# fabioiuri/DRecPy

Measured on AMD Instinct MI355X. Metric: training samples/sec (user-item pairs), higher is better.
Workload: dtype f32; 1 GPU; CDAE hidden_factors=128 sampled-output sparse-Adagrad on synth-10m-shaped synthetic (10000000 users x 1000000 items, 199573906 positives), corruption 0.2, neg_ratio 5; batch_per_gpu=65536, global_batch=65536, touch_list=prepared ahead on a side stream, batches=fresh device-sampled batch every step (sampler running ahead on the side stream)

## Files before the change

drecpy_amd/_lib.py:

```python
import ctypes as C
import os

_HERE = os.path.dirname(os.path.abspath(__file__))
LIB_PATH = os.path.join(_HERE, 'libdrx.so')

LOSS_BCE, LOSS_MSE = 0, 1
TARGETS_REFERENCE, TARGETS_PER_ROW = 0, 1
OPT_ADAM, OPT_ADAGRAD, OPT_ROWWISE_ADAGRAD = 0, 1, 2
DENSE_AUX_CLEAN = 0x100
KEY_NONE = 0xFFFFFFFF
SHARD_SELF_BYPASS = 1
BATCH_SHARE_USERS = 1


class DrxError(RuntimeError):
    pass


DRX_REC_SIGMOID_BIAS, DRX_REC_BIAS, DRX_REC_CLIP = 0, 1, 2

KNN_METRICS = {'cosine': 0, 'adjusted_cosine': 1, 'cosine_cf': 2, 'jaccard': 3, 'msd': 4, 'pearson': 5}
KNN_USER, KNN_ITEM = 0, 1
KNN_AGGREGATIONS = {'mean': 0, 'weighted_mean': 1}

# ... 6 lines not shown
class History(C.Structure):
    _fields_ = [('indptr', C.c_void_p), ('indices', C.c_void_p), ('t_rank', C.c_void_p), ('t_nnz', C.c_int64), ('t_users', C.c_void_p),
                ('t_pos', C.c_void_p), ('t_items', C.c_void_p)]


class Batch(C.Structure):
    _fields_ = [('B', C.c_int32), ('uid', C.c_void_p), ('iid', C.c_void_p), ('y', C.c_void_p),
                ('keep_off', C.c_void_p), ('keep', C.c_void_p), ('mask_seed', C.c_uint64), ('q', C.c_float),
                ('n_touch_slots', C.c_int32), ('flags', C.c_uint32)]


class HotHead(C.Structure):
    _fields_ = [('H', C.c_int32), ('slot', C.c_void_p), ('item', C.c_void_p)]


class ListGroups(C.Structure):
    _fields_ = [('indptr', C.c_void_p), ('seq_ids', C.c_void_p), ('held_indptr', C.c_void_p), ('held', C.c_void_p),
                ('group_value', C.c_void_p), ('eligible', C.c_void_p), ('n_groups', C.c_int32), ('n_eligible', C.c_int32),
                ('n_ids', C.c_int32)]


class Shard(C.Structure):
    _fields_ = [('world', C.c_int32), ('rank', C.c_int32), ('n_items', C.c_int32), ('items_per_rank', C.c_int32),
                ('n_users_local', C.c_int32), ('flags', C.c_uint32), ('chunks', C.c_int32)]


MAX_CHUNKS = 16


class ShardExchange(C.Structure):
    _fields_ = [('send_counts', C.c_void_p), ('recv_counts', C.c_void_p), ('uniq', C.c_void_p), ('req', C.c_void_p), ('table', C.c_void_p),
                ('table_bytes', C.c_size_t), ('rows_cache', C.c_void_p), ('rows_send', C.c_void_p), ('grad_send', C.c_void_p),
                ('grad_recv', C.c_void_p), ('rows_ticket', C.c_int64 * MAX_CHUNKS), ('grad_ticket', C.c_int64 * MAX_CHUNKS)]


MAX_SEGMENTS = 24


class AdamSegments(C.Structure):
    _fields_ = [('n', C.c_int32), ('start', C.c_int32 * MAX_SEGMENTS), ('len', C.c_int32 * MAX_SEGMENTS), ('alpha', C.c_float * MAX_SEGMENTS),
                ('l2_coef', C.c_float * MAX_SEGMENTS)]


class CaserDims(C.Structure):
    _fields_ = [(n, C.c_int32) for n in ('L', 'T', 'Tp', 'd', 'ld', 'ld2', 'n_v', 'n_h', 'n_small', 'off_kv', 'off_bv')] + \
               [('off_kh', C.c_int32 * 8), ('off_bh', C.c_int32 * 8), ('off_wd', C.c_int32), ('off_bd', C.c_int32), ('act_h', C.c_int32),
                ('act_mlp', C.c_int32)]


class CaserArgs(C.Structure):
    _fields_ = [(n, C.c_void_p) for n in ('item_emb', 'user_emb', 'W1', 'b1', 'sw', 'uid', 'before', 'after', 'keep')] + \
               [('rate', C.c_float), ('B', C.c_int32)] + \
               [(n, C.c_void_p) for n in ('dE', 'dW1', 'db1', 'dPu', 'gsw_part', 'loss_part', 'cat_out')] + [('mask_seed', C.c_uint64)]


class CsrAdamTable(C.Structure):
    _fields_ = [(n, C.c_void_p) for n in ('row_ptr', 'order', 'src', 'scale')] + [(n, C.c_int32) for n in ('group', 'ld', 'n_rows')] + \
               [(n, C.c_void_p) for n in ('p', 'm', 'v', 'p_s', 'm_s', 'v_s')] + [(n, C.c_float) for n in ('alpha', 'alpha_s', 'l2_coef')]


class OptRule(C.Structure):
    _fields_ = [('kind', C.c_int32), ('lr', C.c_float), ('mu', C.c_float), ('mu2', C.c_float), ('eps', C.c_float)]


class NcfDims(C.Structure):
    _fields_ = [(n, C.c_int32) for n in ('n_users', 'n_items', 'kg', 'km', 'ldg', 'ldm', 'n_layers')] + \
               [('f', C.c_int32 * 4), ('off_w', C.c_int32 * 4), ('off_b', C.c_int32 * 4), ('off_h', C.c_int32), ('off_b0', C.c_int32),
                ('n_small', C.c_int32)]


class GruDims(C.Structure):
    _fields_ = [(n, C.c_int32) for n in ('n_items', 'k', 'h', 'ldk', 'ldh', 'off_wx', 'off_wh', 'off_bx', 'off_bhn', 'n_small')]


class VaeDims(C.Structure):
    _fields_ = [(n, C.c_int32) for n in ('n_items', 'h', 'ldh', 'latent', 'variational', 'e', 'off_we', 'off_wd', 'off_vec', 'n_small')]


class SasDims(C.Structure):
    _fields_ = [(n, C.c_int32) for n in ('n_items', 'h', 'ldh', 'L', 'blocks', 'off_pos', 'off_blk', 'off_vec', 'off_lnf', 'n_small')]


class CsrList(C.Structure):
    _fields_ = [('keys', C.c_void_p), ('T', C.c_int32), ('n_rows', C.c_int32), ('row_ptr', C.c_void_p), ('order', C.c_void_p)]


class DmfDims(C.Structure):
    _fields_ = [('n_layers', C.c_int32 * 2), ('f', (C.c_int32 * 4) * 2), ('ld0', C.c_int32 * 2),
                ('off_k', (C.c_int32 * 4) * 2), ('off_b', (C.c_int32 * 4) * 2), ('n_small', C.c_int32),
                ('l2_norm_vectors', C.c_int32), ('off_scale', C.c_int32)]


class DmfArgs(C.Structure):
    _fields_ = [(n, C.c_void_p) for n in ('K0u', 'K0i', 'sw', 'u_indptr', 'u_indices', 'u_values', 'i_indptr', 'i_indices',
                                          'i_values', 'uid', 'iid', 'y')] + [('target_mode', C.c_int32), ('y_mean', C.c_float)] + \
               [(n, C.c_void_p) for n in ('off_u', 'off_i')] + [('B', C.c_int32)] + \
               [(n, C.c_void_p) for n in ('dz0u', 'dz0i', 'tkeys_u', 'tsrc_u', 'tcoef_u', 'tkeys_i', 'tsrc_i', 'tcoef_i',
                                          'gsw_part', 'loss_part', 'pred_out', 'rep_u_out', 'rep_i_out', 'work', 'inv_u', 'inv_i',
                                          'gptr_u', 'gptr_i', 'grows_u', 'grows_i')] + [('n_du', C.c_int32), ('n_di', C.c_int32)] + \
               [(n, C.c_void_p) for n in ('map_u', 'map_i', 'rho_u', 'rho_i')] + [('stamp', C.c_uint32)] + \
               [(n, C.c_void_p) for n in ('nd_dev', 'y_mean_dev', 'work_order')] + [('n_work', C.c_int32), ('seg_len', C.c_int32)] + \
               [(n, C.c_void_p) for n in ('zseg', 'zpart', 'n_work_dev')]


class DmfK0Update(C.Structure):
    _fields_ = [(n, C.c_void_p) for n in ('K0u', 'm_u', 'v_u', 'K0i', 'm_i', 'v_i')] + [('n_items', C.c_int32), ('n_users', C.c_int32)] + \
               [(n, C.c_float) for n in ('alpha_u', 'alpha_i', 'l2_coef', 'beta1', 'beta2', 'eps')] + [('row_order', C.c_void_p), ('n_long', C.c_int32), ('opt_kind', C.c_int32)]


class Optim(C.Structure):
    _fields_ = [('kind', C.c_int32), ('lr', C.c_float), ('reg_rate', C.c_float), ('beta1', C.c_float),
                ('beta2', C.c_float), ('eps', C.c_float), ('alpha', C.c_float * 5),
                ('s1', C.c_void_p * 5), ('s2', C.c_void_p * 5)]


_lib = None

SIGNATURES = {
    'drx_version': (C.c_int, []),
    'drx_strerror': (C.c_char_p, [C.c_int]),
    'drx_hash_u32': (C.c_uint32, [C.c_uint64, C.c_uint32, C.c_uint32]),
    'drx_event_create': (C.c_void_p, []),
    'drx_event_destroy': (None, [C.c_void_p]),
    'drx_event_record': (C.c_int, [C.c_void_p, C.c_void_p]),
    'drx_stream_wait_event': (C.c_int, [C.c_void_p, C.c_void_p]),
    'drx_event_synchronize': (C.c_int, [C.c_void_p]),
    'drx_stream_create_cu_slice': (C.c_void_p, [C.c_int32]),
    'drx_stream_destroy': (None, [C.c_void_p]),
    'drx_cdae_forward': (C.c_int, [C.POINTER(CdaeParams), C.POINTER(History), C.POINTER(Batch), C.c_void_p,
                                   C.c_void_p, C.c_void_p]),
    'drx_cdae_scratch_bytes': (C.c_size_t, [C.POINTER(CdaeParams), C.c_int32, C.c_int32, C.c_int32]),
    'drx_cdae_step_dense': (C.c_int, [C.POINTER(CdaeParams), C.POINTER(Optim), C.POINTER(History), C.POINTER(Batch),
                                      C.c_int32, C.c_int32, C.c_void_p, C.c_size_t, C.c_void_p, C.c_void_p]),
    'drx_cdae_step_sparse': (C.c_int, [C.POINTER(CdaeParams), C.POINTER(Optim), C.POINTER(History), C.POINTER(Batch),
                                       C.c_int32, C.c_void_p, C.c_size_t, C.c_void_p, C.c_void_p]),
    'drx_cdae_step_sparse_timed': (C.c_int, [C.POINTER(CdaeParams), C.POINTER(Optim), C.POINTER(History),
                                             C.POINTER(Batch), C.c_int32, C.c_void_p, C.c_size_t, C.c_void_p,
                                             C.POINTER(C.c_void_p), C.c_void_p]),
    'drx_cdae_prep_bytes': (C.c_size_t, [C.POINTER(CdaeParams), C.c_int32, C.c_int32]),
    'drx_cdae_sparse_prepare': (C.c_int, [C.POINTER(CdaeParams), C.POINTER(History), C.POINTER(Batch), C.c_void_p,
                                          C.c_size_t, C.c_void_p]),
    'drx_cdae_step_sparse_prepared': (C.c_int, [C.POINTER(CdaeParams), C.POINTER(Optim), C.POINTER(History),
                                                C.POINTER(Batch), C.c_int32, C.c_void_p, C.c_size_t, C.c_void_p,
                                                C.c_size_t, C.c_void_p, C.POINTER(C.c_void_p), C.c_void_p]),
    'drx_cdae_prep_bytes_hot': (C.c_size_t, [C.POINTER(CdaeParams), C.c_int32, C.c_int32, C.c_int32]),
    'drx_cdae_scratch_bytes_hot': (C.c_size_t, [C.POINTER(CdaeParams), C.c_int32, C.c_int32, C.c_int32]),
    'drx_cdae_sparse_prepare_hot': (C.c_int, [C.POINTER(CdaeParams), C.POINTER(History), C.POINTER(Batch), C.POINTER(HotHead),
                                              C.c_void_p, C.c_size_t, C.c_void_p]),
    'drx_debug_prep_counts': (C.c_int, [C.POINTER(CdaeParams), C.POINTER(History), C.POINTER(Batch), C.POINTER(HotHead), C.c_void_p,
                                        C.c_int32, C.c_int32, C.c_int32, C.c_void_p, C.c_size_t, C.c_void_p, C.c_void_p, C.c_void_p,
                                        C.c_void_p, C.c_void_p, C.POINTER(C.c_int32), C.c_void_p]),
    'drx_debug_prep_result': (C.c_int, [C.POINTER(CdaeParams), C.c_int32, C.c_int32, C.c_int32, C.c_void_p, C.c_size_t, C.c_void_p,
                                        C.c_void_p, C.c_void_p, C.c_void_p, C.c_void_p, C.c_void_p]),
    'drx_debug_cdae_reduce': (C.c_int, [C.POINTER(CdaeParams), C.POINTER(Optim), C.POINTER(History), C.POINTER(Batch), C.POINTER(HotHead),
                                        C.c_void_p, C.c_size_t, C.c_void_p, C.c_void_p, C.c_void_p, C.c_int32, C.c_void_p, C.c_size_t,
                                        C.c_void_p]),
    'drx_debug_span_plan': (C.c_int, [C.POINTER(CdaeParams), C.c_int32, C.c_int32, C.c_int32, C.c_void_p, C.c_size_t, C.c_void_p,
                                      C.c_void_p, C.c_void_p, C.c_void_p]),
    'drx_cdae_step_sparse_hot': (C.c_int, [C.POINTER(CdaeParams), C.POINTER(Optim), C.POINTER(History), C.POINTER(Batch),
                                           C.POINTER(HotHead), C.c_int32, C.c_void_p, C.c_size_t, C.c_void_p, C.c_size_t,
                                           C.c_void_p, C.POINTER(C.c_void_p), C.c_void_p]),
    'drx_cdae_hot_rows_for': (C.c_int32, [C.POINTER(CdaeParams), C.c_int32, C.c_int32, C.c_int32, C.c_int32]),
    'drx_cdae_prep_forget': (None, [C.c_void_p]),
    'drx_point_sample_scratch_bytes': (C.c_size_t, [C.c_int32]),
    'drx_list_sample_device': (C.c_int, [C.POINTER(ListGroups), C.c_int32, C.c_int32, C.c_int32, C.c_int32, C.c_uint64, C.c_void_p, C.c_void_p,
                                         C.c_void_p, C.c_void_p]),
    'drx_point_sample': (C.c_int, [C.POINTER(History), C.c_int32, C.c_int32, C.c_int32, C.c_int32, C.c_uint64,
                                   C.c_void_p, C.c_void_p, C.c_void_p, C.c_void_p, C.c_void_p, C.c_size_t, C.c_void_p, C.c_uint32,
                                   C.c_void_p]),
    'drx_point_sample_recorded': (C.c_int, [C.POINTER(History), C.POINTER(History), C.c_int32, C.c_int32, C.c_int32, C.c_int32, C.c_uint64,
                                   C.c_void_p, C.c_void_p, C.c_void_p, C.c_void_p, C.c_void_p, C.c_size_t, C.c_void_p, C.c_uint32,
                                   C.c_void_p]),
    'drx_point_sample_by_user_scratch_bytes': (C.c_size_t, [C.c_int32, C.c_int32]),
    'drx_point_sample_by_user': (C.c_int, [C.POINTER(History), C.POINTER(History), C.c_int32, C.c_int32, C.c_int32, C.c_int32, C.c_uint64,
                                           C.c_void_p, C.c_void_p, C.c_void_p, C.c_void_p, C.c_void_p, C.c_size_t, C.c_void_p, C.c_uint32,
                                           C.c_void_p]),
    'drx_point_sample_valued': (C.c_int, [C.POINTER(History), C.POINTER(History), C.c_void_p, C.c_float, C.c_float, C.c_int32, C.c_int32,
                                          C.c_int32, C.c_int32, C.c_uint64, C.c_void_p, C.c_void_p, C.c_void_p, C.c_void_p]),
    'drx_dmf_distinct_scratch_bytes': (C.c_size_t, [C.c_int32, C.c_int32, C.c_int32]),
    'drx_dmf_batch_distinct_device': (C.c_int, [C.c_void_p, C.c_void_p, C.c_void_p, C.c_int32, C.c_int32, C.c_int32] + [C.c_void_p] * 10 +
                                      [C.c_void_p, C.c_size_t, C.c_void_p]),
    'drx_shard_prep_bytes': (C.c_size_t, [C.POINTER(CdaeParams), C.POINTER(Shard), C.c_int32, C.c_int32]),
    'drx_shard_work_bytes': (C.c_size_t, [C.POINTER(Shard)]),
    'drx_shard_prep_layout': (C.c_int, [C.POINTER(CdaeParams), C.POINTER(Shard), C.c_int32, C.c_int32, C.POINTER(C.c_size_t)]),
    'drx_shard_prepare': (C.c_int, [C.POINTER(CdaeParams), C.POINTER(Shard), C.POINTER(History), C.POINTER(Batch), C.c_void_p,
                                    C.c_size_t, C.c_void_p, C.c_size_t, C.c_void_p]),
    'drx_shard_owner_table_bytes': (C.c_size_t, [C.POINTER(Shard), C.c_int32]),
    'drx_shard_chunks': (C.c_int32, [C.POINTER(Shard)]),
    'drx_shard_unit_shift': (C.c_int32, [C.POINTER(Shard)]),
    'drx_shard_owner_index': (C.c_int, [C.POINTER(Shard), C.c_void_p, C.c_int32, C.POINTER(C.c_int32), C.c_int32, C.c_int32, C.c_void_p,
                                        C.c_size_t, C.c_void_p]),
    'drx_shard_gather_rows': (C.c_int, [C.POINTER(CdaeParams), C.POINTER(Shard), C.c_void_p, C.c_int32, C.POINTER(C.c_int32),
                                        C.c_int32, C.c_void_p, C.c_void_p]),
    'drx_shard_step_scratch_bytes': (C.c_size_t, [C.POINTER(CdaeParams), C.c_int32, C.c_int32]),
    'drx_shard_step_local': (C.c_int, [C.POINTER(CdaeParams), C.POINTER(Optim), C.POINTER(Shard), C.POINTER(History), C.POINTER(Batch),
                                       C.c_void_p, C.c_size_t, C.c_void_p, C.c_void_p, C.c_int32, C.c_int32, C.c_void_p, C.c_size_t,
                                       C.POINTER(C.c_void_p), C.c_void_p]),
    'drx_shard_apply': (C.c_int, [C.POINTER(CdaeParams), C.POINTER(Optim), C.POINTER(Shard), C.c_int32, C.c_void_p, C.c_void_p,
                                  C.c_int32, C.POINTER(C.c_int32), C.c_int32, C.c_int32, C.c_void_p, C.POINTER(C.c_void_p), C.POINTER(C.c_int64),
                                  C.c_void_p, C.c_void_p]),
    'drx_shard_exchange_sizes': (C.c_int, [C.POINTER(CdaeParams), C.POINTER(Shard), C.c_void_p, C.c_void_p, C.POINTER(C.c_int64)]),
    'drx_shard_phase_layout': (C.c_int, [C.POINTER(CdaeParams), C.POINTER(Shard), C.c_void_p, C.c_void_p, C.c_int32, C.POINTER(C.c_int64)]),
    'drx_shard_phase_keys': (C.c_int, [C.POINTER(Shard), C.c_void_p, C.POINTER(ShardExchange), C.c_void_p]),
    'drx_shard_phase_rows': (C.c_int, [C.POINTER(CdaeParams), C.POINTER(Shard), C.c_void_p, C.POINTER(ShardExchange), C.c_int32, C.c_void_p]),
    'drx_shard_phase_local': (C.c_int, [C.POINTER(CdaeParams), C.POINTER(Optim), C.POINTER(Shard), C.POINTER(History), C.POINTER(Batch),
                                        C.c_void_p, C.POINTER(ShardExchange), C.c_void_p, C.c_size_t, C.c_int32, C.c_int32, C.c_void_p,
                                        C.c_size_t, C.POINTER(C.c_void_p), C.c_void_p]),
    'drx_shard_phase_tail': (C.c_int, [C.POINTER(CdaeParams), C.POINTER(Optim), C.POINTER(Shard), C.c_void_p, C.POINTER(ShardExchange),
                                       C.POINTER(ShardExchange), C.c_int32, C.c_void_p, C.c_void_p]),
    'drx_copy_f4': (C.c_int, [C.c_void_p, C.c_void_p, C.c_size_t, C.c_void_p]),
    'drx_copy_f4_variant': (C.c_int, [C.c_void_p, C.c_void_p, C.c_size_t, C.c_int32, C.c_void_p]),
    'drx_comm_unique_id': (C.c_int, [C.c_void_p]),
    'drx_comm_create': (C.c_int, [C.c_void_p, C.c_int32, C.c_int32, C.c_uint32, C.POINTER(C.c_void_p)]),
    'drx_comm_destroy': (C.c_int, [C.c_void_p]),
    'drx_comm_stream': (C.c_void_p, [C.c_void_p]),
    'drx_comm_alltoallv': (C.c_int64, [C.c_void_p, C.c_void_p, C.POINTER(C.c_int64), C.POINTER(C.c_int64), C.c_void_p, C.POINTER(C.c_int64),
                                       C.POINTER(C.c_int64), C.c_void_p]),
    'drx_comm_wait': (C.c_int, [C.c_void_p, C.c_int64, C.c_void_p]),
    'drx_comm_last_error': (C.c_char_p, []),
    'drx_adam_dense': (C.c_int, [C.c_void_p, C.c_void_p, C.c_void_p, C.c_void_p, C.c_int64, C.c_float, C.c_float, C.c_float,
                                 C.c_float, C.c_float, C.c_void_p]),
    'drx_scatter_scratch_bytes': (C.c_size_t, [C.c_int32, C.c_int32, C.c_int32]),
    'drx_scatter_rows': (C.c_int, [C.c_void_p, C.c_int32, C.c_void_p, C.c_void_p, C.c_void_p, C.c_void_p, C.c_int32,
                                   C.c_int32, C.c_void_p, C.c_void_p, C.c_void_p, C.c_size_t, C.c_void_p]),
    'drx_batch_offsets': (C.c_int, [C.c_void_p, C.c_void_p, C.c_int32, C.c_void_p, C.c_void_p, C.c_size_t, C.c_void_p]),
    'drx_sumsq': (C.c_int, [C.c_void_p, C.c_int64, C.c_void_p, C.c_int32, C.c_void_p]),
    'drx_rows_dot': (C.c_int, [C.c_void_p, C.c_int32, C.c_void_p, C.c_int32, C.c_int32, C.c_void_p, C.c_void_p,
                               C.c_void_p]),
    'drx_adam_segments': (C.c_int, [C.c_void_p, C.c_void_p, C.c_void_p, C.c_void_p, C.POINTER(AdamSegments), C.c_float,
                                    C.c_float, C.c_float, C.c_void_p]),
    'drx_caser_grid': (C.c_int, [C.POINTER(CaserDims), C.c_int32]),
    'drx_caser_fwd_bwd': (C.c_int, [C.POINTER(CaserDims), C.POINTER(CaserArgs), C.c_void_p, C.c_void_p]),
    'drx_caser_step_small': (C.c_int, [C.POINTER(CaserDims), C.POINTER(CaserArgs), C.c_void_p, C.c_void_p, C.c_void_p, C.c_void_p,
                                       C.POINTER(AdamSegments), C.c_float, C.c_float, C.c_float, C.c_void_p]),
    'drx_caser_hidden': (C.c_int, [C.POINTER(CaserDims), C.POINTER(CaserArgs), C.c_void_p]),
    'drx_rows_csr_adam_multi': (C.c_int, [C.POINTER(CsrAdamTable), C.c_int32, C.c_float, C.c_float, C.c_float, C.c_void_p]),
    'drx_dmf_grid': (C.c_int, [C.c_int32]),
    'drx_dmf_work_bytes': (C.c_size_t, [C.c_int32]),
    'drx_dmf_fwd_bwd': (C.c_int, [C.POINTER(DmfDims), C.POINTER(DmfArgs), C.c_void_p, C.c_void_p]),
    'drx_dmf_step_small': (C.c_int, [C.POINTER(DmfDims), C.POINTER(DmfArgs), C.c_void_p, C.c_void_p, C.c_void_p, C.c_void_p,
                                     C.POINTER(AdamSegments), C.c_float, C.c_float, C.c_float, C.c_void_p]),
    'drx_dmf_predict': (C.c_int, [C.POINTER(DmfDims), C.POINTER(DmfArgs), C.c_void_p]),
    'drx_first_occurrence': (C.c_int64, [C.c_void_p, C.c_int64, C.c_int64, C.c_void_p]),
    'drx_spin_until': (C.c_int, [C.c_void_p, C.c_int64, C.c_int32]),
    'drx_batch_csr': (C.c_int, [C.c_void_p, C.c_int32, C.c_int32, C.c_void_p, C.c_void_p]),
    'drx_batch_csr_device_bytes': (C.c_size_t, [C.POINTER(CsrList), C.c_int32]),
    'drx_batch_csr_device': (C.c_int, [C.POINTER(CsrList), C.c_int32, C.c_void_p, C.c_size_t, C.c_void_p]),
    'drx_rows_csr_adam': (C.c_int, [C.c_void_p, C.c_void_p, C.c_void_p, C.c_void_p, C.c_int32, C.c_int32, C.c_void_p, C.c_void_p, C.c_void_p,
                                    C.c_void_p, C.c_void_p, C.c_void_p, C.c_float, C.c_float, C.c_float, C.c_float, C.c_float, C.c_float,
                                    C.c_void_p]),
    'drx_rows_csr_adam_outer': (C.c_int, [C.c_void_p, C.c_void_p, C.c_void_p, C.c_void_p, C.c_int32, C.c_int32, C.c_int32, C.c_void_p,
                                          C.c_void_p, C.c_void_p, C.c_void_p, C.c_void_p, C.c_void_p, C.c_float, C.c_float, C.c_float,
                                          C.c_float, C.c_float, C.c_float, C.c_void_p]),
    'drx_opt_dense': (C.c_int, [C.c_void_p, C.c_void_p, C.c_void_p, C.c_void_p, C.c_int64, C.POINTER(OptRule), C.c_float, C.c_void_p]),
    'drx_opt_segments': (C.c_int, [C.c_void_p, C.c_void_p, C.c_void_p, C.c_void_p, C.POINTER(AdamSegments), C.POINTER(OptRule), C.c_void_p]),
    'drx_rows_csr_opt': (C.c_int, [C.c_void_p, C.c_void_p, C.c_void_p, C.c_void_p, C.c_int32, C.c_int32, C.c_void_p, C.c_void_p, C.c_void_p,
                                   C.c_void_p, C.c_void_p, C.c_void_p, C.c_float, C.c_float, C.c_float, C.POINTER(OptRule), C.c_void_p]),
    'drx_rows_csr_opt_outer': (C.c_int, [C.c_void_p, C.c_void_p, C.c_void_p, C.c_void_p, C.c_int32, C.c_int32, C.c_int32, C.c_void_p,
                                         C.c_void_p, C.c_void_p, C.c_void_p, C.c_void_p, C.c_void_p, C.c_float, C.c_float, C.c_float,
                                         C.POINTER(OptRule), C.c_void_p]),
    'drx_rows_csr_opt_multi': (C.c_int, [C.POINTER(CsrAdamTable), C.c_int32, C.POINTER(OptRule), C.c_void_p]),
    'drx_bpr_sample': (C.c_int, [C.POINTER(History), C.POINTER(History), C.c_void_p, C.c_int32, C.c_int32, C.c_int32, C.c_int32, C.c_uint64,
                                 C.c_void_p, C.c_void_p, C.c_void_p, C.c_void_p]),
    'drx_bpr_gather_rows': (C.c_int, [C.c_void_p, C.c_int32, C.c_void_p, C.c_int32, C.c_void_p, C.c_void_p]),
    'drx_bpr_step_scratch_bytes': (C.c_size_t, [C.c_int32, C.c_int32, C.c_int32, C.c_int32]),
    'drx_bpr_step': (C.c_int, [C.c_void_p] * 9 + [C.c_int32, C.c_int32, C.c_int32, C.c_void_p, C.c_void_p, C.c_void_p, C.c_int32,
                               C.POINTER(OptRule), C.POINTER(C.c_float), C.c_float, C.c_void_p, C.c_void_p, C.c_size_t, C.c_void_p]),
    'drx_als_gram_scratch_bytes': (C.c_size_t, [C.c_int32, C.c_int32]),
    'drx_als_gram': (C.c_int, [C.c_void_p, C.c_int32, C.c_int32, C.c_void_p, C.c_void_p, C.c_size_t, C.c_void_p]),
    'drx_als_solve_rows_scratch_bytes': (C.c_size_t, [C.c_int32, C.c_int32, C.c_int32]),
    'drx_als_solve_rows': (C.c_int, [C.c_void_p] * 7 + [C.c_int32, C.c_int32, C.c_int32, C.c_float, C.c_void_p, C.c_void_p, C.c_size_t,
                                     C.c_void_p]),
    'drx_als_loss_scratch_bytes': (C.c_size_t, [C.c_int32, C.c_int32]),
    'drx_als_loss': (C.c_int, [C.c_void_p] * 7 + [C.c_int32, C.c_int32, C.c_int32, C.c_float, C.c_void_p, C.c_void_p, C.c_size_t, C.c_void_p]),
    'drx_fpmc_step_scratch_bytes': (C.c_size_t, [C.c_int32] * 6),
    'drx_fpmc_step': (C.c_int, [C.c_void_p] * 12 + [C.c_int32, C.c_int32, C.c_int32, C.c_void_p, C.c_void_p, C.c_void_p, C.c_int32, C.c_int32,
                                C.c_int32, C.POINTER(OptRule), C.POINTER(C.c_float), C.c_float, C.c_void_p, C.c_void_p, C.c_size_t, C.c_void_p]),
    'drx_fpmc_query_rows': (C.c_int, [C.c_void_p, C.c_void_p, C.c_int32, C.c_void_p, C.c_int32, C.c_void_p, C.c_int32, C.c_void_p, C.c_void_p]),
    'drx_ncf_grid': (C.c_int, [C.c_int32]),
    'drx_ncf_step_scratch_bytes': (C.c_size_t, [C.POINTER(NcfDims), C.c_int32]),
    'drx_ncf_step': (C.c_int, [C.POINTER(NcfDims)] + [C.c_void_p] * 12 + [C.c_int32, C.POINTER(OptRule), C.POINTER(C.c_float), C.c_float,
                               C.c_void_p, C.c_void_p, C.c_size_t, C.c_void_p]),
    'drx_ncf_half_width': (C.c_int32, [C.POINTER(NcfDims)]),
    'drx_ncf_half_rows': (C.c_int, [C.POINTER(NcfDims), C.c_void_p, C.c_void_p, C.c_void_p, C.c_int32, C.c_int32, C.c_void_p, C.c_void_p]),
    'drx_ncf_score_rows': (C.c_int, [C.POINTER(NcfDims), C.c_void_p, C.c_void_p, C.c_void_p, C.c_int32, C.c_void_p, C.c_void_p]),
    'drx_ncf_pair_scores': (C.c_int, [C.POINTER(NcfDims), C.c_void_p, C.c_void_p, C.c_void_p, C.c_void_p, C.c_void_p, C.c_int32, C.c_void_p,
                                      C.c_void_p]),
    'drx_gru_grid': (C.c_int, [C.c_int32]),
    'drx_gru_step_scratch_bytes': (C.c_size_t, [C.POINTER(GruDims), C.c_int32, C.c_int32, C.c_int32]),
    'drx_gru_step': (C.c_int, [C.POINTER(GruDims)] + [C.c_void_p] * 14 + [C.c_int32, C.c_int32, C.c_int32, C.POINTER(OptRule),
                               C.POINTER(C.c_float), C.c_float, C.c_void_p, C.c_void_p, C.c_size_t, C.c_void_p]),
    'drx_gru_query_rows': (C.c_int, [C.c_void_p, C.c_void_p, C.POINTER(GruDims), C.c_void_p, C.c_int32, C.c_void_p, C.c_int32, C.c_void_p,
                                     C.c_void_p]),
    'drx_sas_grid': (C.c_int, [C.c_int32]),
    'drx_sas_step_scratch_bytes': (C.c_size_t, [C.POINTER(SasDims), C.c_int32, C.c_int32]),
    'drx_sas_step': (C.c_int, [C.POINTER(SasDims)] + [C.c_void_p] * 14 + [C.c_int32, C.c_int32, C.POINTER(OptRule), C.POINTER(C.c_float),
                               C.c_float, C.c_void_p, C.c_void_p, C.c_size_t, C.c_void_p]),
    'drx_sas_query_rows': (C.c_int, [C.c_void_p, C.c_void_p, C.POINTER(SasDims), C.c_void_p, C.c_void_p, C.c_int32, C.c_void_p,
                                     C.c_void_p]),
    'drx_vae_step_scratch_bytes': (C.c_size_t, [C.POINTER(VaeDims), C.c_int32, C.c_int32, C.c_int32]),
    'drx_vae_step': (C.c_int, [C.POINTER(VaeDims)] + [C.c_void_p] * 12 + [C.POINTER(History), C.c_void_p, C.c_void_p, C.c_int32, C.c_int32,
                               C.c_int32, C.c_void_p, C.c_void_p, C.c_float, C.c_float, C.POINTER(OptRule), C.POINTER(C.c_float), C.c_float,
                               C.c_void_p, C.c_void_p, C.c_size_t, C.c_void_p]),
    'drx_vae_noise': (C.c_int, [C.c_uint64, C.c_void_p, C.c_int32, C.c_int32, C.c_int32, C.c_float, C.c_void_p, C.c_void_p, C.c_void_p,
                                C.c_void_p]),
    'drx_vae_query_rows': (C.c_int, [C.c_void_p, C.c_void_p, C.POINTER(VaeDims), C.POINTER(History), C.c_void_p, C.c_int32, C.c_void_p,
# ... 172 lines not shown
```

drecpy_amd/csrc/drx_cdae.hip:

```cpp
#include "drx_common.hpp"
#include "drx_rows.hpp"
#include "drx_segreduce.hpp"
#include <cstring>
#include "drx_scan.hpp"
#include "drx_prep.hpp"
#include "drx_segstream.hpp"
#include "drx_cdae_host.hpp"
#include <type_traits>
#include <mutex>
#include <unordered_map>

#ifdef DRX_STAMPS
static unsigned long long *h_stamps = nullptr;
extern "C" int drx_debug_set_stamps(unsigned long long *buf, unsigned int) { h_stamps = buf; return 0; }
#endif

namespace drx {

struct SparseBufs {
  float *dz1;
  float *g2;
  float *dz2;
  float *lossb;
  float *phead, *ptail;
  float *phs, *pts;
  float *pblock, *pbs;
  float *bpart;
  const uint8_t *solo_v, *solo_o;
  unsigned long long *stamps;
  const int32_t *order;
  const int32_t *usamp, *worder, *n_items;
  const WorkItem *witem;
  int T, n_chunks, n_bpart;
};

template <int G, int J, int KIND = -1>
__device__ __forceinline__ void sparse_apply(const DrxCdaeParams &P, const DrxOptim &opt, int B, uint32_t key, int lane,
                                             const float4 (&g)[J], float gs) {
  const uint32_t N = (uint32_t)P.n_items;
  float *const tW = P.W, *const tO = P.W2T, *const tV = P.V;
  float *const a0 = opt.s1[0], *const a1 = opt.s1[1], *const a2 = opt.s1[2];
  float *const c0 = opt.s2[0], *const c1 = opt.s2[1], *const c2 = opt.s2[2];
  const int var = key < N ? 0 : (key < 2 * N ? 1 : 2);
  const size_t row = key - (uint32_t)var * N;
  float *const tab = var == 0 ? tW : (var == 1 ? tO : tV);
  float *const s1 = var == 0 ? a0 : (var == 1 ? a1 : a2);
  float *const s2 = var == 0 ? c0 : (var == 1 ? c1 : c2);
  OptScalars o = opt_for(opt, 0, B);
  o.inv_k = 1.0f / (float)P.k;
  float4 w[J];
  load_row<G, J>(tab, row, P.ld, lane, w);
  row_update<G, J, KIND>(o, tab, s1, s2, row, P.ld, lane, w, g);
  if (var == 1 && lane == 0) {
    const int kind = KIND >= 0 ? KIND : o.kind;
    float pb = P.b2[row], m = opt.s1[4][row], v = kind == DRX_OPT_ADAM ? opt.s2[4][row] : 0.f;
    o.rb = 0.f;
    opt_update1<KIND>(o, gs, pb, m, v);
    P.b2[row] = pb; opt.s1[4][row] = m;
    if (kind == DRX_OPT_ADAM) opt.s2[4][row] = v;
  }
}

template <int G, int J>
__device__ __forceinline__ float sampled_hidden(const DrxCdaeParams &P, const DrxBatch &bt, float scale, int b, int lane,
                                                const float4 (&acc)[J], float4 (&h)[J], float4 (&w2)[J]) {
  hidden_act<G, J>(P, bt.uid[b], scale, lane, acc, h);
  load_row<G, J>(P.W2T, (size_t)bt.iid[b], P.ld, lane, w2);
  float d = 0.f;
#pragma unroll
  for (int j = 0; j < J; ++j) d += f4_dot(w2[j], h[j]);
  return group_sum<G>(d);
}

template <int G, int J, int KIND = -1>
__device__ __forceinline__ void sampled_rest(const DrxCdaeParams &P, const DrxOptim &opt, const DrxHistory &H, const DrxBatch &bt,
                                             float scale, uint32_t qthr, int loss_kind, const SparseBufs &S, int b, int lane,
                                             float d, const float4 (&h)[J], const float4 (&w2)[J],
                                             float4 (*dz1_out)[J] = nullptr) {
  const int u = bt.uid[b], i = bt.iid[b];
  const float y = bt.y[b];
  const float p = sigmoidf_(d + P.b2[i]);
  const float invB = 1.0f / (float)bt.B;
  float lval, dp;
  if (loss_kind == DRX_LOSS_BCE) { lval = bce_elem(y, p); dp = bce_grad(y, p) * invB; }
  else { lval = (p - y) * (p - y); dp = 2.0f * (p - y) * invB; }
  const float dz2 = dp * p * (1.0f - p);
  float4 dz1[J], g2[J];
#pragma unroll
  for (int j = 0; j < J; ++j) {
    dz1[j].x = dz2 * w2[j].x * h[j].x * (1.0f - h[j].x); dz1[j].y = dz2 * w2[j].y * h[j].y * (1.0f - h[j].y);
    dz1[j].z = dz2 * w2[j].z * h[j].z * (1.0f - h[j].z); dz1[j].w = dz2 * w2[j].w * h[j].w * (1.0f - h[j].w);
    g2[j].x = dz2 * h[j].x; g2[j].y = dz2 * h[j].y; g2[j].z = dz2 * h[j].z; g2[j].w = dz2 * h[j].w;
  }
  store_row<G, J>(S.dz1, (size_t)b, P.ld, lane, dz1);
  if (lane == 0) S.lossb[b] = lval;
  const uint8_t *const pv = S.solo_v, *const po = S.solo_o;
  const bool solo_v = pv && pv[b], solo_o = po && po[b];
  if (solo_o) {
    sparse_apply<G, J, KIND>(P, opt, bt.B, (uint32_t)P.n_items + (uint32_t)i, lane, g2, dz2);
  } else {
    store_row<G, J>(S.g2, (size_t)b, P.ld, lane, g2);
    if (lane == 0) S.dz2[b] = dz2;
  }
  if (solo_v) sparse_apply<G, J, KIND>(P, opt, bt.B, 2u * (uint32_t)P.n_items + (uint32_t)u, lane, dz1, 0.f);
  if (dz1_out) {
#pragma unroll
    for (int j = 0; j < J; ++j) (*dz1_out)[j] = dz1[j];
  }
}

template <int G, int J, int KIND = -1>
__device__ __forceinline__ void sampled_finish(const DrxCdaeParams &P, const DrxOptim &opt, const DrxHistory &H, const DrxBatch &bt,
                                               float scale, uint32_t qthr, int loss_kind, const SparseBufs &S, int b, int lane,
                                               const float4 (&acc)[J]) {
  float4 h[J], w2[J];
#ifdef DRX_STAMPS
  if (acc[0].x == acc[0].x) DRX_STAMP(S.stamps, b, 5, lane);
#endif
  const float d = sampled_hidden<G, J>(P, bt, scale, b, lane, acc, h, w2);
#ifdef DRX_STAMPS
  if (d == d) DRX_STAMP(S.stamps, b, 6, lane);
#endif
  sampled_rest<G, J, KIND>(P, opt, H, bt, scale, qthr, loss_kind, S, b, lane, d, h, w2);
  DRX_STAMP(S.stamps, b, 7, lane);
}

template <int G, int J>
__global__ __launch_bounds__(kBlock) void k_kshard_fwd(DrxCdaeParams P, DrxHistory H, DrxBatch bt, float scale, uint32_t qthr,
                                                       float *__restrict__ h_out, float *__restrict__ dot_out,
                                                       const int32_t *__restrict__ order) {
  const int lane = threadIdx.x % G;
  const int slot = blockIdx.x * (kBlock / G) + threadIdx.x / G;
  if (slot >= bt.B) return;
  const int b = order ? order[slot] : slot;
  float4 acc[J], h[J], w2[J];
  DenseAux none{};
  gather_bag<G, J, 0>(P, H, bt, qthr, b, lane, acc, none, nullptr, nullptr, 0);
  const float d = sampled_hidden<G, J>(P, bt, scale, b, lane, acc, h, w2);
  store_row<G, J>(h_out, (size_t)b, P.ld, lane, h);
  if (lane == 0) dot_out[b] = d;
}

template <int G, int J>
__global__ __launch_bounds__(kBlock) void k_kshard_fwd_wg(DrxCdaeParams P, DrxHistory H, DrxBatch bt, float scale, uint32_t qthr,
                                                          float *__restrict__ h_out, float *__restrict__ dot_out) {
  extern __shared__ __align__(16) float lds[];
  constexpr int R = kBlock / G;
  const int lane = threadIdx.x % G, r = threadIdx.x / G;
  const int b = blockIdx.x;
  float4 acc[J], h[J], w2[J];
  DenseAux none{};
  gather_bag<G, J, 0>(P, H, bt, qthr, b, lane, acc, none, nullptr, nullptr, 0, r, R);
  store_row<G, J>(lds, (size_t)r, P.ld, lane, acc);
  __syncthreads();
  if (r != 0) return;
#pragma unroll
  for (int j = 0; j < J; ++j) acc[j] = f4_zero();
#pragma unroll 8
  for (int rr = 0; rr < R; ++rr) {
    float4 v[J];
    load_row<G, J>(lds, (size_t)rr, P.ld, lane, v);
#pragma unroll
    for (int j = 0; j < J; ++j) f4_add(acc[j], v[j]);
  }
  const float d = sampled_hidden<G, J>(P, bt, scale, b, lane, acc, h, w2);
  store_row<G, J>(h_out, (size_t)b, P.ld, lane, h);
  if (lane == 0) dot_out[b] = d;
}

template <int G, int J>
__global__ __launch_bounds__(kBlock) void k_kshard_rest(DrxCdaeParams P, DrxOptim opt, DrxHistory H, DrxBatch bt, float scale,
                                                        uint32_t qthr, int loss_kind, SparseBufs S,
                                                        const float *__restrict__ h_in, const float *__restrict__ dot_total) {
  const int lane = threadIdx.x % G;
  const int b = blockIdx.x * (kBlock / G) + threadIdx.x / G;
  if (b >= bt.B) return;
  float4 h[J], w2[J];
  load_row<G, J>(h_in, (size_t)b, P.ld, lane, h);
  load_row<G, J>(P.W2T, (size_t)bt.iid[b], P.ld, lane, w2);
  sampled_rest<G, J>(P, opt, H, bt, scale, qthr, loss_kind, S, b, lane, dot_total[b], h, w2);
}

template <int G, int J, int KIND = -1>
__global__ __launch_bounds__(kBlock) void k_sampled_fwd_bwd(DrxCdaeParams P, DrxOptim opt, DrxHistory H, DrxBatch bt, float scale,
                                                            uint32_t qthr, int loss_kind, SparseBufs S) {
  const int lane = threadIdx.x % G;
  const int slot = blockIdx.x * (kBlock / G) + threadIdx.x / G;
#ifdef DRX_STAMPS
  const unsigned long long t_in = wall_clock64();
#endif
  if (slot >= bt.B) return;
  const int32_t *const ord = S.order;
  const int b = ord ? ord[slot] : slot;
  float4 acc[J];
  DenseAux none{};
#ifdef DRX_STAMPS
  if (lane == 0 && S.stamps && (unsigned)b < 110000u) S.stamps[(size_t)b * 16] = t_in;
  if (bt.uid[b] >= 0) DRX_STAMP(S.stamps, b, 1, lane);
#endif
  gather_bag<G, J, 0>(P, H, bt, qthr, b, lane, acc, none, nullptr, nullptr, 0, 0, 1, S.stamps);
  sampled_finish<G, J, KIND>(P, opt, H, bt, scale, qthr, loss_kind, S, b, lane, acc);
}

template <int G, int J, int KIND = -1>
__global__ __launch_bounds__(kItemThreads, (4 * G * J <= 128 ? 5 : 1)) void k_items_fwd_bwd(DrxCdaeParams P, DrxOptim opt, DrxHistory H, DrxBatch bt, float scale,
                                                          uint32_t qthr, int loss_kind, SparseBufs S) {
  extern __shared__ __align__(16) float lds[];
  constexpr int R = kItemThreads / G, NWV = kItemThreads / 64, RT = kShareTriples;
  constexpr int NH = 4 * G * J / 64;
  static_assert(NH >= 1 && NH <= 8 && RT == 16, "rows of 64 .. 512 floats; the 16 x 16 x 4 matrix instruction");
  constexpr int NF = NH <= 2 ? 16 : (NH == 4 ? 8 : 4);
  constexpr int TPG = (RT + R - 1) / R;
  if ((int)blockIdx.x >= S.n_items[0]) return;
  const int w = S.worder[blockIdx.x];
  const WorkItem wi = S.witem[w];
  const int p0 = wi.p0, n = wi.n, u = wi.user;
  const int64_t s = wi.hist_start, e = s + wi.deg;
  const int lane = threadIdx.x % G, r = threadIdx.x / G;
  int *lb = (int *)(lds + (size_t)NWV * RT * P.ld);
  if ((int)threadIdx.x < RT) lb[threadIdx.x] = (int)threadIdx.x < n ? S.usamp[p0 + threadIdx.x] : 0;
  float4 vrow[J];
  load_row<G, J>(P.V, (size_t)u, P.ld, lane, vrow);
  const int n_waves = (int)min((int64_t)NWV, (e - s + NF - 1) / NF);
  {
    typedef float f4v __attribute__((ext_vector_type(4)));
    const int wl = threadIdx.x & 63, wv = threadIdx.x >> 6;
    const int kr = wl >> 4, nc = wl & 15;
    f4v acc[NH][4];
#pragma unroll
    for (int h = 0; h < NH; ++h)
#pragma unroll
      for (int j = 0; j < 4; ++j) acc[h][j] = f4v{0.f, 0.f, 0.f, 0.f};
    const int64_t c0 = s + (int64_t)wv * NF;
    int ridx[NF / 4];
#pragma unroll
    for (int g = 0; g < NF / 4; ++g) ridx[g] = c0 + 4 * g + kr < e ? H.indices[c0 + 4 * g + kr] : 0;
    __syncthreads();
    const int bmine = lb[nc];
    for (int64_t c = c0; c < e; c += (int64_t)NWV * NF) {
      const int64_t cn = c + (int64_t)NWV * NF;
      int ridx_n[NF / 4];
#pragma unroll
      for (int g = 0; g < NF / 4; ++g) ridx_n[g] = cn + 4 * g + kr < e ? H.indices[cn + 4 * g + kr] : 0;
      float4 bv[NF / 4][NH];
#pragma unroll
      for (int g = 0; g < NF / 4; ++g)
#pragma unroll
        for (int h = 0; h < NH; ++h) {
          bv[g][h] = f4_zero();
          if (c + 4 * g + kr < e && 64 * h + 4 * nc < P.ld)
            bv[g][h] = *reinterpret_cast<const float4 *>(P.W + (size_t)ridx[g] * P.ld + 64 * h + 4 * nc);
        }
#pragma unroll
      for (int g = 0; g < NF / 4; ++g) {
        const int64_t row = c + 4 * g + kr;
        bool kf = false;
        if (nc < n && row < e) {
          const uint32_t jj = (uint32_t)(row - s);
          kf = bt.keep ? (bt.keep[bt.keep_off[bmine] + jj] != 0) : (hash_u32(bt.mask_seed, (uint32_t)bmine, jj) >= qthr);
        }
        const float a = kf ? 1.0f : 0.0f;
#pragma unroll
        for (int h = 0; h < NH; ++h) {
          acc[h][0] = __builtin_amdgcn_mfma_f32_16x16x4f32(a, bv[g][h].x, acc[h][0], 0, 0, 0);
          acc[h][1] = __builtin_amdgcn_mfma_f32_16x16x4f32(a, bv[g][h].y, acc[h][1], 0, 0, 0);
          acc[h][2] = __builtin_amdgcn_mfma_f32_16x16x4f32(a, bv[g][h].z, acc[h][2], 0, 0, 0);
          acc[h][3] = __builtin_amdgcn_mfma_f32_16x16x4f32(a, bv[g][h].w, acc[h][3], 0, 0, 0);
        }
      }
#pragma unroll
      for (int g = 0; g < NF / 4; ++g) ridx[g] = ridx_n[g];
    }
    if (wv < n_waves) {
#pragma unroll
      for (int i = 0; i < 4; ++i) {
        const int t = 4 * kr + i;
        if (t < n) {
#pragma unroll
          for (int h = 0; h < NH; ++h)
            if (64 * h + 4 * nc < P.ld)
              *reinterpret_cast<float4 *>(lds + (size_t)(wv * RT + t) * P.ld + 64 * h + 4 * nc) =
                  make_float4(acc[h][0][i], acc[h][1][i], acc[h][2][i], acc[h][3][i]);
        }
      }
    }
  }
  __syncthreads();
  float4 dsum[J];
#pragma unroll
  for (int j = 0; j < J; ++j) dsum[j] = f4_zero();
#pragma unroll
  for (int kt = 0; kt < TPG; ++kt) {
    const int t = r + kt * R;
    if (t < n) {
      const int b = lb[t];
      float4 acc[J], h[J], w2[J], dz1[J];
#pragma unroll
      for (int j = 0; j < J; ++j) acc[j] = f4_zero();
      for (int wv = 0; wv < n_waves; ++wv) {
        float4 x[J];
        load_row<G, J>(lds, (size_t)(wv * RT + t), P.ld, lane, x);
#pragma unroll
        for (int j = 0; j < J; ++j) f4_add(acc[j], x[j]);
      }
      float4 brow[J];
      load_row<G, J>(P.b, 0, P.ld, lane, brow);
      hidden_act_rows<G, J>(P, scale, lane, acc, vrow, brow, h);
      load_row<G, J>(P.W2T, (size_t)bt.iid[b], P.ld, lane, w2);
      float d = 0.f;
#pragma unroll
      for (int j = 0; j < J; ++j) d += f4_dot(w2[j], h[j]);
      d = group_sum<G>(d);
      sampled_rest<G, J, KIND>(P, opt, H, bt, scale, qthr, loss_kind, S, b, lane, d, h, w2, &dz1);
#pragma unroll
      for (int j = 0; j < J; ++j) f4_add(dsum[j], dz1[j]);
    }
  }
  __syncthreads();
  if (r < n) store_row<G, J>(lds, (size_t)r, P.ld, lane, dsum);
  __syncthreads();
  if (r == 0) {
    float4 t[J];
#pragma unroll
    for (int j = 0; j < J; ++j) t[j] = f4_zero();
    for (int rr = 0; rr < min(n, R); ++rr) {
      float4 x[J];
      load_row<G, J>(lds, (size_t)rr, P.ld, lane, x);
#pragma unroll
      for (int j = 0; j < J; ++j) f4_add(t[j], x[j]);
    }
    store_row<G, J>(S.dz1, (size_t)bt.B + w, P.ld, lane, t);
  }
}

template <int G, int J>
__global__ __launch_bounds__(kBlock) void k_sampled_fwd_bwd_wg(DrxCdaeParams P, DrxOptim opt, DrxHistory H, DrxBatch bt, float scale,
                                                               uint32_t qthr, int loss_kind, SparseBufs S) {
  extern __shared__ __align__(16) float lds[];
  constexpr int R = kBlock / G;
  const int lane = threadIdx.x % G, r = threadIdx.x / G;
  const int b = blockIdx.x;
  float4 acc[J];
  DenseAux none{};
  gather_bag<G, J, 0>(P, H, bt, qthr, b, lane, acc, none, nullptr, nullptr, 0, r, R);
// ... 153 lines not shown
    const uint32_t mlane = (uint32_t)c * (uint32_t)A.Bw, xlane = (uint32_t)(8 * kq * LD + c);
    hot_f32x4 acc[4];
#pragma unroll
    for (int t = 0; t < 4; ++t) acc[t] = hot_f32x4{0.f, 0.f, 0.f, 0.f};
    uint32_t seen = 0u;
    float bsum = 0.f;
    for (int b0 = b_begin; b0 < b_end; b0 += 32) {
      float x[8];
      uint32_t w[4];
      {
        const float *const rows = slice + (size_t)(b0 - b_begin) * LD;
        const uint32_t *const words = mgrp + (b0 >> 5);
        const int left = A.B - b0 - 8 * kq;
        if (left >= 8) {
#pragma unroll
          for (int j = 0; j < 8; ++j) x[j] = rows[xlane + (uint32_t)(j * LD)];
        } else {
#pragma unroll
          for (int j = 0; j < 8; ++j) x[j] = j < left ? rows[xlane + (uint32_t)(j * LD)] : 0.f;
        }
#pragma unroll
        for (int t = 0; t < 4; ++t) w[t] = (words + (size_t)(16 * min(t, nt - 1)) * A.Bw)[mlane] & (t < nt ? ~0u : 0u);
      }
      hot_u32x4 bh, bm, bl;
#pragma unroll
      for (int i = 0; i < 4; ++i) {
        uint32_t hv[2], mv[2], lv[2];
#pragma unroll
        for (int e = 0; e < 2; ++e) {
          const float v = x[2 * i + e];
          bsum += v;
          hv[e] = __float_as_uint(v) & 0xFFFF0000u;
          const float r1 = v - __uint_as_float(hv[e]);
          mv[e] = __float_as_uint(r1) & 0xFFFF0000u;
          lv[e] = __float_as_uint(r1 - __uint_as_float(mv[e])) & 0xFFFF0000u;
        }
        bh[i] = (hv[0] >> 16) | hv[1];
        bm[i] = (mv[0] >> 16) | mv[1];
        bl[i] = (lv[0] >> 16) | lv[1];
      }
#pragma unroll
      for (int t = 0; t < 4; ++t) {
        seen |= (w[t] != 0u ? 1u : 0u) << t;
        const uint32_t bits = (w[t] >> (8 * kq)) & 0xFFu;
        hot_u32x4 a;
#pragma unroll
        for (int i = 0; i < 4; ++i) a[i] = ((bits >> (2 * i)) & 1u) * 0x3F80u | ((bits >> (2 * i + 1)) & 1u) * 0x3F800000u;
        const hot_bf16x8 av = __builtin_bit_cast(hot_bf16x8, a);
        acc[t] = __builtin_amdgcn_mfma_f32_16x16x32_bf16(av, __builtin_bit_cast(hot_bf16x8, bh), acc[t], 0, 0, 0);
        acc[t] = __builtin_amdgcn_mfma_f32_16x16x32_bf16(av, __builtin_bit_cast(hot_bf16x8, bm), acc[t], 0, 0, 0);
        acc[t] = __builtin_amdgcn_mfma_f32_16x16x32_bf16(av, __builtin_bit_cast(hot_bf16x8, bl), acc[t], 0, 0, 0);
      }
    }
    float *const out = A.part + ((size_t)s * A.H + rg * kHotGroup) * LD + cs * 16 + c;
#pragma unroll
    for (int t = 0; t < 4; ++t)
      if (t < nt) {
#pragma unroll
        for (int i = 0; i < 4; ++i) out[(size_t)(16 * t + 4 * kq + i) * LD] = acc[t][i];
      }
    if (cs == 0) {
      uint32_t rows[4];
#pragma unroll
      for (int t = 0; t < 4; ++t) rows[t] = (uint32_t)__ballot((seen >> t) & 1u) & 0xFFFFu;
      if (lane == 0) {
        uint32_t *const any = A.any + (size_t)s * (A.H / 32) + rg * (kHotGroup / 32);
        any[0] = rows[0] | (rows[1] << 16);
        if (nt > 2) any[1] = rows[2] | (rows[3] << 16);
      }
    }
    if (rg == 0) {
      const float g1 = __shfl(bsum, c + 16, 64), g2 = __shfl(bsum, c + 32, 64), g3 = __shfl(bsum, c + 48, 64);
      if (kq == 0) A.bpart[(size_t)s * LD + cs * 16 + c] = ((bsum + g1) + g2) + g3;
      if (cs == 0 && A.lossb) {
        float l = 0.f;
        for (int b = b_begin + lane; b < b_end; b += 64) l += A.lossb[b];
#pragma unroll
        for (int o = 32; o > 0; o >>= 1) l += __shfl_xor(l, o, 64);
        if (lane == 0) A.bpart[(size_t)A.S * LD + s] = l;
      }
    }
  }
};

template <int LD, class Policy>
struct HotFinishExtra {
  HotArgs A;
  Policy pol;
  __device__ __forceinline__ void operator()(float *lds) const {
    constexpr int NT = kFixBlock, NQ = NT / LD;
    static_assert(NQ >= 1 && NT % LD == 0, "a row per workgroup");
    const int h = (int)blockIdx.x - A.first;
    if (h >= A.H) return;
    const uint32_t bit = 1u << (h & 31);
    bool touched = false;
    for (int s = (int)threadIdx.x; s < A.S; s += NT) touched |= (A.any[(size_t)s * (A.H / 32) + (h >> 5)] & bit) != 0u;
    if (!__syncthreads_or(touched)) return;
    const int c = (int)threadIdx.x % LD, q = (int)threadIdx.x / LD;
    const int per = (A.S + NQ - 1) / NQ, s0 = q * per, s1 = min(A.S, s0 + per);
    float sum = 0.f;
#pragma unroll 8
    for (int s = s0; s < s1; ++s) sum += A.part[((size_t)s * A.H + h) * LD + c];
    lds[q * LD + c] = sum;
    __syncthreads();
    if (q == 0) {
      float t = lds[c];
#pragma unroll
      for (int k = 1; k < NQ; ++k) t += lds[k * LD + c];
      const StreamArrays SA = pol.stream_arrays();
      const size_t off = (size_t)A.item[h] * LD + c;
      float pv = SA.table[0][off], av = SA.slot[0][off];
      pol.stream_update(fmaf(pol.stream_decay(), pv, A.scale * t), pv, av);
      SA.table[0][off] = pv;
      SA.slot[0][off] = av;
    }
  }
};

template <class E1, class E2>
struct ExtraPair {
  E1 e1;
  int n1;
  E2 e2;
  __device__ __forceinline__ void operator()(float *lds) const {
    if ((int)blockIdx.x < n1) e1(lds);
    else e2(lds);
  }
};

static SparseBufs sparse_layout(Carver &cv, const DrxCdaeParams &P, int B, int n_touch_slots) {
  SparseBufs S{};
  S.T = n_touch_slots + 2 * B;
  const int chunk = seg_chunk(long_segments(S.T, P));
  S.n_chunks = (S.T + chunk - 1) / chunk;
  S.n_bpart = 1024;
  S.dz1 = cv.take<float>((size_t)2 * B * P.ld);
  S.g2 = cv.take<float>((size_t)B * P.ld);
  S.dz2 = cv.take<float>(B);
  S.lossb = cv.take<float>(B);
  S.phead = cv.take<float>((size_t)S.n_chunks * P.ld);
  S.ptail = cv.take<float>((size_t)S.n_chunks * P.ld);
  S.phs = cv.take<float>(S.n_chunks);
  S.pts = cv.take<float>(S.n_chunks);
  {
    const int cpb = kSegBlock / pick_geom(P.ld).G;
    const int n_blocks = (S.n_chunks + cpb - 1) / cpb;
    S.pblock = cv.take<float>((size_t)n_blocks * P.ld);
    S.pbs = cv.take<float>(n_blocks);
  }
  S.bpart = cv.take<float>((size_t)S.n_bpart * (P.ld + 1));
  return S;
}

static std::mutex g_hot_mu;
static std::unordered_map<const void *, int> g_hot_of;
static void hot_record(const void *prepared, int H) {
  std::lock_guard<std::mutex> lk(g_hot_mu);
  if (H > 0) g_hot_of[prepared] = H;
  else g_hot_of.erase(prepared);
}
static int hot_recorded(const void *prepared) {
  std::lock_guard<std::mutex> lk(g_hot_mu);
  const auto it = g_hot_of.find(prepared);
  return it == g_hot_of.end() ? 0 : it->second;
}

struct HotBufs { float *part; uint32_t *any; float *bpart; };
static HotBufs hot_layout(Carver &cv, const DrxCdaeParams &P, int B, int H) {
  HotBufs HB{nullptr, nullptr, nullptr};
  if (H <= 0) return HB;
  HB.part = cv.take<float>((size_t)hot_slices(B) * H * P.ld);
  HB.any = cv.take<uint32_t>((size_t)hot_slices(B) * (H / 32));
  HB.bpart = cv.take<float>((size_t)hot_slices(B) * (P.ld + 1));
  return HB;
}

template <int G, int J>
static void launch_forward(ForwardForm form, const DrxCdaeParams &P, const DrxOptim &opt, const DrxHistory &hist, const DrxBatch &bt,
                           float scale, uint32_t qthr, int32_t loss_kind, const SparseBufs &S, const float *ks_h, const float *ks_dot,
                           hipStream_t st) {
  constexpr int gpb = kBlock / G;
  const dim3 groups((bt.B + gpb - 1) / gpb);
  const bool adagrad = opt.kind == DRX_OPT_ADAGRAD;
  switch (form) {
  case ForwardForm::ColumnShard:
    hipLaunchKernelGGL((k_kshard_rest<G, J>), groups, dim3(kBlock), 0, st, P, opt, hist, bt, scale, qthr, loss_kind, S, ks_h, ks_dot);
    break;
  case ForwardForm::SharedUsers:
    if constexpr (G >= 16 && J <= 2) {
      const long long wmax = (long long)(P.n_users < bt.B ? P.n_users : bt.B) + bt.B / share_item_triples(P.ld) + 1;
      hipLaunchKernelGGL((adagrad ? k_items_fwd_bwd<G, J, DRX_OPT_ADAGRAD> : k_items_fwd_bwd<G, J>), dim3((unsigned)(wmax < bt.B ? wmax : bt.B)),
                         dim3(kItemThreads), share_item_lds_bytes(P.ld), st, P, opt, hist, bt, scale, qthr, loss_kind, S);
    }
    break;
  case ForwardForm::PerWorkgroup:
    hipLaunchKernelGGL((k_sampled_fwd_bwd_wg<G, J>), dim3(bt.B), dim3(kBlock), (size_t)gpb * P.ld * 4, st, P, opt, hist, bt, scale, qthr,
                       loss_kind, S);
    break;
  case ForwardForm::PerGroup:
    hipLaunchKernelGGL((adagrad ? k_sampled_fwd_bwd<G, J, DRX_OPT_ADAGRAD> : k_sampled_fwd_bwd<G, J>), groups, dim3(kBlock), 0, st, P, opt, hist,
                       bt, scale, qthr, loss_kind, S);
    break;
  }
}

template <int G, int J, class Policy>
static int reduce_and_finish(ReduceForm form, const DrxCdaeParams &P, const DrxOptim &opt, const SparseBufs &S, const SegBufs &SB,
                             const PlanBufs &PB, const SpanPlan &plan, const BiasArgs &BA, const HotArgs &HA, void *const *events,
                             hipStream_t st) {
  const Policy pol{P, opt, BA.B, HA.scale, S.dz1, (long long)(S.g2 - S.dz1), S.dz2};
  const BiasFinalExtra<G, J> bias{P, opt, BA};
  int rc = DRX_EINVAL;
  if (HA.H == 0) rc = launch_reduce<G, J>(form, SB, PB, plan, pol, BA, st);
  else if constexpr (kHotBuilt<G, J, Policy>) {
    constexpr int NT = kStreamThreads<G>;
    HotArgs part = HA;
    part.first = 0;
    const int n_hot = (HA.S * hot_groups(HA.H) * (G / 4) + NT / 64 - 1) / (NT / 64);
    rc = launch_reduce_streamed<G, J>(SB, PB, plan, pol, n_hot, HotPartialExtra<4 * G, NT>{part}, st);
  }
  if (rc) return rc;
  DRX_HIP(phase_event(events, 3, st));
  rc = DRX_EINVAL;
  if (HA.H == 0) rc = launch_spans<G, J>(SB, PB, plan, pol, 1, bias, st);
  else if constexpr (kHotBuilt<G, J, Policy>) {
    HotArgs fin = HA;
    fin.first = kSpanBlocks + 1;
    using Finish = ExtraPair<BiasFinalExtra<G, J>, HotFinishExtra<4 * G, Policy>>;
    rc = launch_spans<G, J>(SB, PB, plan, pol, 1 + HA.H, Finish{bias, fin.first, {fin, pol}}, st);
  }
  if (rc) return rc;
  DRX_HIP(phase_event(events, 4, st));
  DRX_HIP(phase_event(events, 5, st));
  return DRX_OK;
}

}

using namespace drx;

extern "C" {

size_t drx_cdae_scratch_bytes(const DrxCdaeParams *p, int32_t B, int32_t n_touch_slots, int32_t dense_mode) {
  if (!p || B < 1 || n_touch_slots < 0) return 0;
  Carver c(nullptr, 0);
  if (dense_mode) {
    c.off = dense_layout_bytes(*p, B);
  } else {
    (void)sparse_layout(c, *p, B, n_touch_slots);
    (void)prep_layout(c, *p, B, n_touch_slots);
  }
  return align_up(c.off, 256) + 256;
}

struct GivenGradients { const float *dz1, *g2, *dz2; int32_t form; };

static int step_sparse_impl(const DrxCdaeParams *p, const DrxOptim *opt, const DrxHistory *hist, const DrxBatch *bt,
                            int32_t loss_kind, const void *prepared, size_t prepared_bytes, void *scratch, size_t scratch_bytes,
                            float *loss_out, void *const *events, void *stream, const float *ks_h = nullptr,
                            const float *ks_dot = nullptr, const DrxHotHead *hot = nullptr, const GivenGradients *given = nullptr) {
  int rc = check_params(p);
  if (rc) return rc;
  rc = check_batch(hist, bt);
  if (rc || !opt || !scratch || !bt->iid || (!bt->y && !given) || !bt->keep_off) return DRX_EINVAL;
  if (opt->kind != DRX_OPT_ADAM && opt->kind != DRX_OPT_ADAGRAD && opt->kind != DRX_OPT_ROWWISE_ADAGRAD) return DRX_EINVAL;
  for (int i = 0; i < 5; ++i)
    if (!opt->s1[i] || (opt->kind == DRX_OPT_ADAM && !opt->s2[i])) return DRX_EINVAL;
  if ((uint64_t)2 * p->n_items + p->n_users + 1 >= 0xFFFFFFFFull) return DRX_EINVAL;
  hipStream_t st = (hipStream_t)stream;
  const int H = hot ? hot->H : 0;
  if (prepared && hot_recorded(prepared) != H) return DRX_EINVAL;
  Carver cv(scratch, scratch_bytes);
  SparseBufs S = sparse_layout(cv, *p, bt->B, bt->n_touch_slots);
  const HotBufs HB = hot_layout(cv, *p, bt->B, H);
  PrepBufs R{};
  if (prepared) {
    Carver cp(const_cast<void *>(prepared), prepared_bytes);
    R = prep_layout(cp, *p, bt->B, bt->n_touch_slots, H);
    if (!cp.ok()) return DRX_ESCRATCH;
  } else {
    R = prep_layout(cv, *p, bt->B, bt->n_touch_slots, H);
  }
  if (!cv.ok()) return DRX_ESCRATCH;
  const float scale = 1.0f / (1.0f - bt->q);
  const uint32_t qthr = q_threshold(bt->q);
  const int rows_per_block = (bt->B + S.n_bpart - 1) / S.n_bpart;
  const int n_bpart = (bt->B + rows_per_block - 1) / rows_per_block;
  S.solo_v = prepared ? R.solo_v : nullptr;
  S.solo_o = prepared ? R.solo_o : nullptr;
  S.order = prepared ? R.order : nullptr;
  SegBufs SB{R.keys_s, R.vals_s, S.phead, S.ptail, S.phs, S.pts, nullptr, nullptr, nullptr, nullptr, S.T, S.n_chunks, p->ld, nullptr};
#ifdef DRX_STAMPS
  S.stamps = SB.stamps = h_stamps;
#endif
  PlanBufs PB{S.pblock, S.pbs};
  if (prepared && ks_h && share_users(p, hist, bt, R)) return DRX_EINVAL;
  const bool share = prepared && !ks_h && share_users(p, hist, bt, R);
  S.usamp = share ? R.usamp : nullptr;
  S.witem = share ? R.witem : nullptr;
  S.worder = share ? R.worder : nullptr;
  S.n_items = share ? R.n_du : nullptr;
  ReduceForm form = reduce_form(opt->kind, bt->B, S.T, *p);
  const ForwardForm fwd = forward_form(ks_h != nullptr, share, bt->B, bt->n_touch_slots);
  if (H > 0 && !hot_head_fits(form, p->ld, share, ks_h != nullptr)) return DRX_EINVAL;
  if (given) {
    if (share || (given->form == 1 && (H > 0 || form == ReduceForm::PlannedLong))) return DRX_EINVAL;
    if (given->form == 1) form = ReduceForm::PlannedShort;
  }
  const HotArgs HA{S.dz1, R.hmask, HB.part, HB.any, hot ? hot->item : nullptr, scale, bt->B, H, R.Bw, hot_slices(bt->B), 0, HB.bpart,
                   loss_out ? S.lossb : nullptr};
  const BiasArgs BA = H > 0 ? BiasArgs{S.dz1, HB.bpart, S.lossb, loss_out, bt->B, hot_slices(bt->B), kHotSlice}
                            : BiasArgs{S.dz1, S.bpart, S.lossb, loss_out, bt->B, n_bpart, rows_per_block};
  DRX_HIP(phase_event(events, 0, st));
  if (given) {
    const size_t row_bytes = (size_t)bt->B * p->ld * sizeof(float);
    DRX_HIP(hipMemcpyAsync(S.dz1, given->dz1, row_bytes, hipMemcpyDeviceToDevice, st));
    DRX_HIP(hipMemcpyAsync(S.g2, given->g2, row_bytes, hipMemcpyDeviceToDevice, st));
    DRX_HIP(hipMemcpyAsync(S.dz2, given->dz2, (size_t)bt->B * sizeof(float), hipMemcpyDeviceToDevice, st));
    DRX_HIP(hipMemsetAsync(S.lossb, 0, (size_t)bt->B * sizeof(float), st));
  } else {
    (void)dispatch_geom(p->ld, [&](auto g) -> int {
      launch_forward<decltype(g)::G, decltype(g)::J>(fwd, *p, *opt, *hist, *bt, scale, qthr, loss_kind, S, ks_h, ks_dot, st);
      return DRX_OK;
    });
  }
  DRX_HIP(phase_event(events, 1, st));
  if (!prepared) {
    rc = prepare_impl(p, hist, bt, R, st, false, TouchPresence{nullptr, WireGeo{1, 0, 1}}, hot ? hot->slot : nullptr,
                      hot ? hot->item : nullptr);
    if (rc) return rc;
  }
  DRX_HIP(phase_event(events, 2, st));
  rc = dispatch_geom(p->ld, [&](auto g) -> int {
    constexpr int G = decltype(g)::G, J = decltype(g)::J;
    return opt->kind == DRX_OPT_ADAGRAD
        ? reduce_and_finish<G, J, DirectPolicyAdagrad>(form, *p, *opt, S, SB, PB, R.plan, BA, HA, events, st)
        : reduce_and_finish<G, J, DirectPolicy>(form, *p, *opt, S, SB, PB, R.plan, BA, HA, events, st);
  });
  if (rc) return rc;
  DRX_LAUNCH_CHECK();
  return DRX_OK;
}

size_t drx_cdae_prep_bytes(const DrxCdaeParams *p, int32_t B, int32_t n_touch_slots) {
  if (!p || B < 1 || n_touch_slots < 0) return 0;
  Carver c(nullptr, 0);
  (void)prep_layout(c, *p, B, n_touch_slots);
  return align_up(c.off, 256) + 256;
}

int drx_cdae_sparse_prepare(const DrxCdaeParams *p, const DrxHistory *hist, const DrxBatch *bt, void *prepared,
                            size_t prepared_bytes, void *stream) {
  int rc = check_params(p);
  if (rc) return rc;
  rc = check_batch(hist, bt);
  if (rc || !prepared || !bt->iid || !bt->keep_off) return DRX_EINVAL;
  Carver cp(prepared, prepared_bytes);
  PrepBufs R = prep_layout(cp, *p, bt->B, bt->n_touch_slots);
  if (!cp.ok()) return DRX_ESCRATCH;
  hot_record(prepared, 0);
  rc = prepare_impl(p, hist, bt, R, (hipStream_t)stream, true);
  if (rc) return rc;
  if (p->ld <= 16) order_by_degree(bt, R, (hipStream_t)stream, true);
  DRX_LAUNCH_CHECK();
  return DRX_OK;
}

size_t drx_cdae_prep_result_bytes(const DrxCdaeParams *p, int32_t B, int32_t n_touch_slots) {
  if (!p || B < 1 || n_touch_slots < 0) return 0;
  Carver c(nullptr, 0);
  return prep_layout(c, *p, B, n_touch_slots).result_bytes;
}

int drx_cdae_step_sparse_prepared(const DrxCdaeParams *p, const DrxOptim *opt, const DrxHistory *hist, const DrxBatch *bt,
                                  int32_t loss_kind, const void *prepared, size_t prepared_bytes, void *scratch,
                                  size_t scratch_bytes, float *loss_out, void *const *events, void *stream) {
  if (!prepared) return DRX_EINVAL;
  return step_sparse_impl(p, opt, hist, bt, loss_kind, prepared, prepared_bytes, scratch, scratch_bytes, loss_out, events, stream);
}

int drx_cdae_kshard_forward(const DrxCdaeParams *p, const DrxHistory *hist, const DrxBatch *bt, float *h_out, float *dot_partial,
                            void *stream) {
  return drx_cdae_kshard_forward_prepared(p, hist, bt, nullptr, 0, h_out, dot_partial, stream);
}

int drx_cdae_kshard_forward_prepared(const DrxCdaeParams *p, const DrxHistory *hist, const DrxBatch *bt, const void *prepared,
                                     size_t prepared_bytes, float *h_out, float *dot_partial, void *stream) {
  int rc = check_params(p);
  if (rc) return rc;
  rc = check_batch(hist, bt);
  if (rc || !bt->iid || !bt->keep_off || !h_out || !dot_partial) return DRX_EINVAL;
  const int32_t *order = nullptr;
  if (prepared) {
    Carver cp(const_cast<void *>(prepared), prepared_bytes);
    const PrepBufs R = prep_layout(cp, *p, bt->B, bt->n_touch_slots);
    if (!cp.ok()) return DRX_ESCRATCH;
    order = R.order;
  }
  hipStream_t st = (hipStream_t)stream;
  const float scale = 1.0f / (1.0f - bt->q);
  const uint32_t qthr = q_threshold(bt->q);
  const bool per_wg = forward_per_workgroup(bt->B, bt->n_touch_slots);
  return dispatch_geom(p->ld, [&](auto g) -> int {
    constexpr int G = decltype(g)::G, J = decltype(g)::J;
    constexpr int gpb = kBlock / G;
    if (per_wg)
      hipLaunchKernelGGL((k_kshard_fwd_wg<G, J>), dim3(bt->B), dim3(kBlock), (size_t)gpb * p->ld * 4, st, *p, *hist, *bt, scale, qthr,
                         h_out, dot_partial);
    else
      hipLaunchKernelGGL((k_kshard_fwd<G, J>), dim3((bt->B + gpb - 1) / gpb), dim3(kBlock), 0, st, *p, *hist, *bt, scale, qthr, h_out,
                         dot_partial, order);
    DRX_LAUNCH_CHECK();
    return DRX_OK;
  });
}

int drx_cdae_kshard_step(const DrxCdaeParams *p, const DrxOptim *opt, const DrxHistory *hist, const DrxBatch *bt, int32_t loss_kind,
                         const float *h, const float *dot_total, const void *prepared, size_t prepared_bytes, void *scratch,
                         size_t scratch_bytes, float *loss_out, void *const *events, void *stream) {
  if (!h || !dot_total) return DRX_EINVAL;
  if (opt && opt->kind == DRX_OPT_ROWWISE_ADAGRAD) return DRX_EINVAL;
  return step_sparse_impl(p, opt, hist, bt, loss_kind, prepared, prepared_bytes, scratch, scratch_bytes, loss_out, events, stream,
                          h, dot_total);
}

int drx_cdae_step_sparse(const DrxCdaeParams *p, const DrxOptim *opt, const DrxHistory *hist, const DrxBatch *bt,
                         int32_t loss_kind, void *scratch, size_t scratch_bytes, float *loss_out, void *stream) {
  return step_sparse_impl(p, opt, hist, bt, loss_kind, nullptr, 0, scratch, scratch_bytes, loss_out, nullptr, stream);
}

int drx_cdae_step_sparse_timed(const DrxCdaeParams *p, const DrxOptim *opt, const DrxHistory *hist, const DrxBatch *bt,
                               int32_t loss_kind, void *scratch, size_t scratch_bytes, float *loss_out, void *const *events,
                               void *stream) {
  if (!events) return DRX_EINVAL;
  return step_sparse_impl(p, opt, hist, bt, loss_kind, nullptr, 0, scratch, scratch_bytes, loss_out, events, stream);
}

static int hot_rows(const DrxCdaeParams *p, int32_t H) {
  if (!p || H < 0 || H > DRX_MAX_HOT || H % 32 || H > p->n_items) return -1;
  return H;
}

static bool hot_ok(const DrxCdaeParams *p, const DrxHotHead *hot) {
  return hot && hot_rows(p, hot->H) >= 0 && (hot->H == 0 || (hot->slot && hot->item && p->ld <= 4 * kHotMaxG));
}

size_t drx_cdae_prep_bytes_hot(const DrxCdaeParams *p, int32_t B, int32_t n_touch_slots, int32_t H) {
  if (!p || B < 1 || n_touch_slots < 0 || hot_rows(p, H) < 0) return 0;
  Carver c(nullptr, 0);
  (void)prep_layout(c, *p, B, n_touch_slots, H);
  return align_up(c.off, 256) + 256;
}

size_t drx_cdae_scratch_bytes_hot(const DrxCdaeParams *p, int32_t B, int32_t n_touch_slots, int32_t H) {
  if (!p || B < 1 || n_touch_slots < 0 || hot_rows(p, H) < 0) return 0;
  Carver c(nullptr, 0);
  (void)sparse_layout(c, *p, B, n_touch_slots);
  (void)hot_layout(c, *p, B, H);
  (void)prep_layout(c, *p, B, n_touch_slots, H);
  return align_up(c.off, 256) + 256;
}

int drx_cdae_sparse_prepare_hot(const DrxCdaeParams *p, const DrxHistory *hist, const DrxBatch *bt, const DrxHotHead *hot,
                                void *prepared, size_t prepared_bytes, void *stream) {
  int rc = check_params(p);
  if (rc) return rc;
  rc = check_batch(hist, bt);
  if (rc || !prepared || !bt->iid || !bt->keep_off || !hot_ok(p, hot)) return DRX_EINVAL;
  Carver cp(prepared, prepared_bytes);
  PrepBufs R = prep_layout(cp, *p, bt->B, bt->n_touch_slots, hot->H);
  if (!cp.ok()) return DRX_ESCRATCH;
  hot_record(prepared, 0);
  rc = prepare_impl(p, hist, bt, R, (hipStream_t)stream, true, TouchPresence{nullptr, WireGeo{1, 0, 1}}, hot->slot, hot->item);
  if (rc) return rc;
  hot_record(prepared, hot->H);
  if (p->ld <= 16) order_by_degree(bt, R, (hipStream_t)stream, true);
  DRX_LAUNCH_CHECK();
  return DRX_OK;
}

int drx_debug_prep_counts(const DrxCdaeParams *p, const DrxHistory *hist, const DrxBatch *bt, const DrxHotHead *hot, uint8_t *present,
                          int32_t ipr, int32_t cshift, int32_t world, void *prepared, size_t prepared_bytes, uint32_t *hist_out,
                          uint32_t *buckets_out, uint32_t *keys_out, uint32_t *vals_out, uint32_t *mask_out, int32_t *info_out,
                          void *stream) {
  int rc = check_params(p);
  if (rc) return rc;
  rc = check_batch(hist, bt);
  if (rc || !prepared || !bt->iid || !bt->keep_off || !hist_out || !buckets_out || !keys_out || !vals_out || !info_out) return DRX_EINVAL;
  if ((uint64_t)2 * p->n_items + p->n_users + 1 >= 0xFFFFFFFFull) return DRX_EINVAL;
  if (hot && !hot_ok(p, hot)) return DRX_EINVAL;
  if (present && (ipr < 1 || cshift < 0 || cshift > 30 || world < 1)) return DRX_EINVAL;
  const int H = hot ? hot->H : 0;
  if (H > 0 && !mask_out) return DRX_EINVAL;
  Carver cp(prepared, prepared_bytes);
  const PrepBufs R = prep_layout(cp, *p, bt->B, bt->n_touch_slots, H);
  if (!cp.ok()) return DRX_ESCRATCH;
  if (H > 0 && !hot_list_fits(R.T, *p, present != nullptr)) return DRX_EINVAL;
  hipStream_t st = (hipStream_t)stream;
  hot_record(prepared, 0);
  launch_touches(p, hist, bt, R, st, TouchPresence{present, WireGeo{present ? ipr : 1, present ? cshift : 0, present ? world : 1}},
                 H > 0 ? hot->slot : nullptr, H > 0 ? hot->item : nullptr);
  const SortRider rider{bt->keep_off, bt->B, R.order_work, R.partials, R.partial_rows};
  const uint32_t *h = nullptr;
  rc = sort_first_counts(R.sort_temp, R.sort_bytes, R.keys, (size_t)R.T, R.bits, true, st, rider, &h);
  if (rc) return rc;
  const int dbits = sort_first_digit_bits(R.bits);
  DRX_HIP(hipMemcpyAsync(hist_out, h, sizeof(uint32_t) << dbits, hipMemcpyDeviceToDevice, st));
  DRX_HIP(hipMemcpyAsync(buckets_out, R.order_work, 256 * sizeof(uint32_t), hipMemcpyDeviceToDevice, st));
  DRX_HIP(hipMemcpyAsync(keys_out, R.keys, (size_t)R.T * sizeof(uint32_t), hipMemcpyDeviceToDevice, st));
  DRX_HIP(hipMemcpyAsync(vals_out, R.vals, (size_t)R.T * sizeof(uint32_t), hipMemcpyDeviceToDevice, st));
  if (H > 0) DRX_HIP(hipMemcpyAsync(mask_out, R.hmask, (size_t)H * R.Bw * sizeof(uint32_t), hipMemcpyDeviceToDevice, st));
  info_out[0] = dbits;
  info_out[1] = R.partials ? R.partial_rows : 0;
  info_out[2] = R.T;
  info_out[3] = DRX_PREP_ROUNDS ? touch_grid(bt->B) : (bt->B + 15) / 16;
  DRX_LAUNCH_CHECK();
  return DRX_OK;
}

int drx_debug_prep_result(const DrxCdaeParams *p, int32_t B, int32_t n_touch_slots, int32_t H, const void *prepared, size_t prepared_bytes,
                          uint32_t *keys_s_out, uint32_t *vals_s_out, uint8_t *solo_v_out, uint8_t *solo_o_out, int32_t *order_out,
                          void *stream) {
  int rc = check_params(p);
  if (rc) return rc;
  if (B < 1 || n_touch_slots < 0 || hot_rows(p, H) < 0 || !prepared || !keys_s_out || !vals_s_out || !solo_v_out || !solo_o_out || !order_out)
    return DRX_EINVAL;
  Carver cp(const_cast<void *>(prepared), prepared_bytes);
  const PrepBufs R = prep_layout(cp, *p, B, n_touch_slots, H);
  if (!cp.ok()) return DRX_ESCRATCH;
  hipStream_t st = (hipStream_t)stream;
  DRX_HIP(hipMemcpyAsync(keys_s_out, R.keys_s, (size_t)R.T * sizeof(uint32_t), hipMemcpyDeviceToDevice, st));
  DRX_HIP(hipMemcpyAsync(vals_s_out, R.vals_s, (size_t)R.T * sizeof(uint32_t), hipMemcpyDeviceToDevice, st));
  DRX_HIP(hipMemcpyAsync(solo_v_out, R.solo_v, (size_t)B, hipMemcpyDeviceToDevice, st));
  DRX_HIP(hipMemcpyAsync(solo_o_out, R.solo_o, (size_t)B, hipMemcpyDeviceToDevice, st));
  DRX_HIP(hipMemcpyAsync(order_out, R.order, (size_t)B * sizeof(int32_t), hipMemcpyDeviceToDevice, st));
  return DRX_OK;
}

int drx_debug_cdae_reduce(const DrxCdaeParams *p, const DrxOptim *opt, const DrxHistory *hist, const DrxBatch *bt, const DrxHotHead *hot,
                          const void *prepared, size_t prepared_bytes, const float *dz1_in, const float *g2_in, const float *dz2_in,
                          int32_t form, void *scratch, size_t scratch_bytes, void *stream) {
  if (!dz1_in || !g2_in || !dz2_in || (form != 0 && form != 1) || (hot && !hot_ok(p, hot))) return DRX_EINVAL;
  const GivenGradients given{dz1_in, g2_in, dz2_in, form};
  return step_sparse_impl(p, opt, hist, bt, DRX_LOSS_BCE, prepared, prepared_bytes, scratch, scratch_bytes, nullptr, nullptr, stream,
                          nullptr, nullptr, hot && hot->H > 0 ? hot : nullptr, &given);
}

int drx_debug_span_plan(const DrxCdaeParams *p, int32_t B, int32_t n_touch_slots, int32_t H, const void *prepared, size_t prepared_bytes,
                        uint8_t *ext_out, uint32_t *desc_out, uint32_t *cnt_out, void *stream) {
  int rc = check_params(p);
  if (rc) return rc;
  if (B < 1 || n_touch_slots < 0 || hot_rows(p, H) < 0 || !prepared || !ext_out || !desc_out || !cnt_out) return DRX_EINVAL;
  Carver cp(const_cast<void *>(prepared), prepared_bytes);
  const PrepBufs R = prep_layout(cp, *p, B, n_touch_slots, H);
  if (!cp.ok()) return DRX_ESCRATCH;
  hipStream_t st = (hipStream_t)stream;
  DRX_HIP(hipMemcpyAsync(ext_out, R.plan.ext, (size_t)R.n_chunks, hipMemcpyDeviceToDevice, st));
  DRX_HIP(hipMemcpyAsync(desc_out, R.plan.desc, (size_t)R.n_chunks * sizeof(uint2), hipMemcpyDeviceToDevice, st));
  DRX_HIP(hipMemcpyAsync(cnt_out, R.plan.cnt, 2 * sizeof(uint32_t), hipMemcpyDeviceToDevice, st));
  return DRX_OK;
}

int drx_cdae_step_sparse_hot(const DrxCdaeParams *p, const DrxOptim *opt, const DrxHistory *hist, const DrxBatch *bt,
                             const DrxHotHead *hot, int32_t loss_kind, const void *prepared, size_t prepared_bytes, void *scratch,
                             size_t scratch_bytes, float *loss_out, void *const *events, void *stream) {
  if (!hot_ok(p, hot)) return DRX_EINVAL;
  return step_sparse_impl(p, opt, hist, bt, loss_kind, prepared, prepared_bytes, scratch, scratch_bytes, loss_out, events, stream,
                          nullptr, nullptr, hot);
}

int32_t drx_cdae_hot_rows_for(const DrxCdaeParams *p, int32_t opt_kind, int32_t B, int32_t n_touch_slots, int32_t H) {
  if (B < 1 || n_touch_slots < 0 || hot_rows(p, H) <= 0) return 0;
  return hot_head_fits(reduce_form(opt_kind, B, n_touch_slots + 2 * B, *p), p->ld, false, false) ? H : 0;
}

void drx_cdae_prep_forget(const void *prepared) {
  if (prepared) hot_record(prepared, 0);
}

}
```

drecpy_amd/csrc/drx_prep.hpp:

```cpp
#pragma once
#include <algorithm>
#include "drx_common.hpp"
#include "drx_rows.hpp"
#include "drx_segreduce.hpp"
#include "drx_scan.hpp"

namespace drx {

struct WireGeo {
  int ipr, cshift, world;
  __host__ __device__ __forceinline__ uint32_t wire(int item, int is_out) const {
    const int o = item / ipr;
    const uint32_t l = 2u * (uint32_t)(item - o * ipr) + (uint32_t)(is_out ? 1 : 0);
    return (((l >> cshift) * (uint32_t)world + (uint32_t)o) << cshift) | (l & ((1u << cshift) - 1u));
  }
  __host__ __device__ __forceinline__ uint32_t local(uint32_t w) const {
    return (((w >> cshift) / (uint32_t)world) << cshift) | (w & ((1u << cshift) - 1u));
  }
  __host__ __device__ __forceinline__ uint32_t unit(uint32_t w) const { return w >> cshift; }
};

struct TouchPresence {
  uint8_t *present;
  WireGeo G;
  __device__ __forceinline__ uint32_t wire(int item, int is_out) const { return G.wire(item, is_out); }
};

#ifndef DRX_HOT_LDS_LOOKUP
#define DRX_HOT_LDS_LOOKUP 1
#endif
struct HotMark {
  const int16_t *slot;
  uint32_t *mask;
  int H, Bw;
  const int32_t *item;
  int tbits;
};
static inline int hot_table_bits(int H) {
  int b = 0;
  while ((1 << b) < 4 * H) ++b;
  return b;
}
static inline size_t hot_table_lds_bytes(int H) { return H > 0 && DRX_HOT_LDS_LOOKUP ? ((size_t)6 << hot_table_bits(H)) : 0; }
__device__ __forceinline__ uint32_t hot_table_home(int item, int tbits) { return ((uint32_t)item * 2654435761u) >> (32 - tbits); }

static __global__ __launch_bounds__(kBlock) void k_sparse_touches(int n_items, DrxHistory H, DrxBatch bt, uint32_t qthr, uint32_t *keys,
                                                           uint32_t *vals, int T, uint8_t *solo, uint32_t *zero_a,
                                                           int n_zero_a, uint32_t *zero_b, int n_zero_b, uint32_t *zero_c, int n_zero_c,
                                                           TouchPresence pres, HotMark hot) {
  constexpr int G = 16;
  const int lane = threadIdx.x % G;
  const int b = blockIdx.x * (kBlock / G) + threadIdx.x / G;
  for (int w = blockIdx.x * kBlock + threadIdx.x; w < n_zero_a; w += gridDim.x * kBlock) zero_a[w] = 0u;
  for (int w = blockIdx.x * kBlock + threadIdx.x; w < n_zero_b; w += gridDim.x * kBlock) zero_b[w] = 0u;
  for (int w = blockIdx.x * kBlock + threadIdx.x; w < n_zero_c; w += gridDim.x * kBlock) zero_c[w] = 0u;
  __shared__ uint32_t hm[DRX_MAX_HOT];
  extern __shared__ __align__(16) int hot_table[];
  const uint32_t tmask = (1u << hot.tbits) - 1u;
  uint16_t *const hot_slot_of = reinterpret_cast<uint16_t *>(hot_table + tmask + 1);
  if (hot.slot) {
    for (int i = threadIdx.x; i < hot.H; i += kBlock) hm[i] = 0u;
    if (DRX_HOT_LDS_LOOKUP) {
      for (int i = threadIdx.x; i <= (int)tmask; i += kBlock) hot_table[i] = -1;
      __syncthreads();
      for (int i = threadIdx.x; i < hot.H; i += kBlock) {
        const int it = hot.item[i];
        uint32_t at = hot_table_home(it, hot.tbits);
        while (atomicCAS(&hot_table[at], -1, it) != -1) at = (at + 1u) & tmask;
        hot_slot_of[at] = (uint16_t)i;
      }
    }
    __syncthreads();
  }
  if (b < bt.B) {
  if (solo && lane == 0) { solo[b] = 0; solo[bt.B + b] = 0; }
  if (b == bt.B - 1)
    for (int j = bt.keep_off[bt.B] + 2 * bt.B + lane; j < T; j += G) { keys[j] = DRX_KEY_NONE; vals[j] = 0; }
  const int u = bt.uid[b];
  const int64_t s = H.indptr[u], e = H.indptr[u + 1];
  const int base = bt.keep_off[b] + 2 * b;
  const uint8_t *kp = bt.keep ? bt.keep + bt.keep_off[b] : nullptr;
  for (int64_t j = s + lane; j < e; j += G) {
    const uint32_t jj = (uint32_t)(j - s);
    const bool kf = kp ? (kp[jj] != 0) : (hash_u32(bt.mask_seed, (uint32_t)b, jj) >= qthr);
    const int item = H.indices[j];
    int hs = -1;
    if (hot.slot && kf) {
      if (DRX_HOT_LDS_LOOKUP) {
        for (uint32_t at = hot_table_home(item, hot.tbits);; at = (at + 1u) & tmask) {
          const int k = hot_table[at];
          if (k == item) hs = (int)hot_slot_of[at];
          if (k == item || k == -1) break;
        }
      } else hs = (int)hot.slot[item];
    }
    keys[base + jj] = kf && hs < 0 ? (uint32_t)item : DRX_KEY_NONE;
    vals[base + jj] = (uint32_t)b;
    if (hs >= 0) atomicOr(&hm[hs], 1u << (b & 15));
    if (pres.present && kf) pres.present[pres.wire(item, 0)] = 1;
  }
  if (lane == 0) {
    const int deg = (int)(e - s);
    keys[base + deg] = (uint32_t)(n_items + bt.iid[b]);       vals[base + deg] = (uint32_t)b;
    if (pres.present) pres.present[pres.wire(bt.iid[b], 1)] = 1;
    keys[base + deg + 1] = (uint32_t)(2 * n_items) + (uint32_t)u;       vals[base + deg + 1] = (uint32_t)b;
  }
  }
  if (hot.slot) {
    __syncthreads();
    uint16_t *const m16 = reinterpret_cast<uint16_t *>(hot.mask);
    const size_t row = 2 * (size_t)hot.Bw;
    const bool tail = blockIdx.x + 1 == gridDim.x && blockIdx.x + 1 < row;
    for (int i = threadIdx.x; i < hot.H; i += kBlock) {
      m16[(size_t)i * row + blockIdx.x] = (uint16_t)hm[i];
      if (tail) m16[(size_t)i * row + blockIdx.x + 1] = 0;
    }
  }
}

#ifndef DRX_PREP_ROUNDS
#define DRX_PREP_ROUNDS 1
#endif
#ifndef DRX_TOUCH_GRID
#define DRX_TOUCH_GRID 1024
#endif
static inline int touch_grid(int B) {
  const int rounds = (B + kBlock / 16 - 1) / (kBlock / 16);
  return rounds < DRX_TOUCH_GRID ? rounds : DRX_TOUCH_GRID;
}

static __global__ __launch_bounds__(kBlock) void k_sparse_touches_rounds(int n_items, DrxHistory H, DrxBatch bt, uint32_t qthr, uint32_t *keys,
                                                                  uint32_t *vals, int T, uint8_t *solo, uint32_t *zero_a,
                                                                  int n_zero_a, uint32_t *zero_b, int n_zero_b, uint32_t *zero_c,
                                                                  int n_zero_c, TouchPresence pres, HotMark hot, uint32_t *part) {
  constexpr int G = 16, SPR = kBlock / G;
  const int lane = threadIdx.x % G, grp = threadIdx.x / G;
  const int B = bt.B, n_rounds = (B + SPR - 1) / SPR, stride = (int)gridDim.x;
  for (int w = blockIdx.x * kBlock + threadIdx.x; w < n_zero_a; w += gridDim.x * kBlock) zero_a[w] = 0u;
  for (int w = blockIdx.x * kBlock + threadIdx.x; w < n_zero_b; w += gridDim.x * kBlock) zero_b[w] = 0u;
  for (int w = blockIdx.x * kBlock + threadIdx.x; w < n_zero_c; w += gridDim.x * kBlock) zero_c[w] = 0u;
  __shared__ uint32_t hm[DRX_MAX_HOT];
  __shared__ uint32_t dh[2048];
  __shared__ uint32_t bh[256];
  extern __shared__ __align__(16) int hot_table[];
  const uint32_t tmask = (1u << hot.tbits) - 1u;
  uint16_t *const hot_slot_of = reinterpret_cast<uint16_t *>(hot_table + tmask + 1);
  if (part) {
    for (int i = threadIdx.x; i < 2048; i += kBlock) dh[i] = 0u;
    for (int i = threadIdx.x; i < 256; i += kBlock) bh[i] = 0u;
  }
  if (hot.slot) {
    for (int i = threadIdx.x; i < hot.H; i += kBlock) hm[i] = 0u;
    if (DRX_HOT_LDS_LOOKUP) {
      for (int i = threadIdx.x; i <= (int)tmask; i += kBlock) hot_table[i] = -1;
      __syncthreads();
      for (int i = threadIdx.x; i < hot.H; i += kBlock) {
        const int it = hot.item[i];
        uint32_t at = hot_table_home(it, hot.tbits);
        while (atomicCAS(&hot_table[at], -1, it) != -1) at = (at + 1u) & tmask;
        hot_slot_of[at] = (uint16_t)i;
      }
    }
  }
  __syncthreads();
  const uint32_t rep = threadIdx.x & 7u;
  constexpr int kPre = 2;
  struct Stage { int u, ko0, ko1, iid; int64_t s, e; };
  const int S = stride * SPR;
  int r = (int)blockIdx.x;
  int b = r * SPR + grp;
  Stage c{0, 0, 0, 0, 0, 0}, n1 = c;
  int it[kPre], u2 = 0;
  if (b < B) { c.u = bt.uid[b]; c.ko0 = bt.keep_off[b]; c.ko1 = bt.keep_off[b + 1]; c.iid = bt.iid[b]; c.s = H.indptr[c.u]; c.e = H.indptr[c.u + 1]; }
  if (b + S < B) {
    n1.u = bt.uid[b + S]; n1.ko0 = bt.keep_off[b + S]; n1.ko1 = bt.keep_off[b + S + 1]; n1.iid = bt.iid[b + S];
    n1.s = H.indptr[n1.u]; n1.e = H.indptr[n1.u + 1];
  }
  if (b + 2 * S < B) u2 = bt.uid[b + 2 * S];
#pragma unroll
  for (int k = 0; k < kPre; ++k) it[k] = c.s + lane + k * G < c.e ? H.indices[c.s + lane + k * G] : 0;
  for (; r < n_rounds; r += stride, b += S) {
    int itn[kPre], u3 = 0;
    Stage n2{u2, 0, 0, 0, 0, 0};
#pragma unroll
    for (int k = 0; k < kPre; ++k) itn[k] = n1.s + lane + k * G < n1.e ? H.indices[n1.s + lane + k * G] : 0;
    if (b + 2 * S < B) {
      n2.ko0 = bt.keep_off[b + 2 * S]; n2.ko1 = bt.keep_off[b + 2 * S + 1]; n2.iid = bt.iid[b + 2 * S];
      n2.s = H.indptr[u2]; n2.e = H.indptr[u2 + 1];
    }
    if (b + 3 * S < B) u3 = bt.uid[b + 3 * S];
    if (b < B) {
      const int u = c.u, ko0 = c.ko0, ko1 = c.ko1;
      const int64_t s = c.s, e = c.e;
      if (solo && lane == 0) { solo[b] = 0; solo[B + b] = 0; }
      if (b == B - 1)
        for (int j = ko1 + 2 * B + lane; j < T; j += G) { keys[j] = DRX_KEY_NONE; vals[j] = 0; }
      const int base = ko0 + 2 * b;
      const uint8_t *kp = bt.keep ? bt.keep + ko0 : nullptr;
      auto touch = [&](uint32_t jj, int item) {
        const bool kf = kp ? (kp[jj] != 0) : (hash_u32(bt.mask_seed, (uint32_t)b, jj) >= qthr);
        int hs = -1;
        if (hot.slot && kf) {
          if (DRX_HOT_LDS_LOOKUP) {
            for (uint32_t at = hot_table_home(item, hot.tbits);; at = (at + 1u) & tmask) {
              const int k = hot_table[at];
              if (k == item) hs = (int)hot_slot_of[at];
              if (k == item || k == -1) break;
            }
          } else hs = (int)hot.slot[item];
        }
        const bool listed = kf && hs < 0;
        keys[base + jj] = listed ? (uint32_t)item : DRX_KEY_NONE;
        vals[base + jj] = (uint32_t)b;
        if (part && listed) atomicAdd(&dh[(((uint32_t)item & 255u) << 3) + rep], 1u);
        if (hs >= 0) atomicOr(&hm[hs], 1u << (b & 15));
        if (pres.present && kf) pres.present[pres.wire(item, 0)] = 1;
      };
#pragma unroll
      for (int k = 0; k < kPre; ++k)
        if (s + lane + k * G < e) touch((uint32_t)(lane + k * G), it[k]);
      for (int64_t j = s + lane + kPre * G; j < e; j += G) touch((uint32_t)(j - s), H.indices[j]);
      if (lane == 0) {
        const int deg = (int)(e - s);
        const uint32_t k_out = (uint32_t)(n_items + c.iid), k_usr = (uint32_t)(2 * n_items) + (uint32_t)u;
        keys[base + deg] = k_out;       vals[base + deg] = (uint32_t)b;
        if (pres.present) pres.present[pres.wire(c.iid, 1)] = 1;
        keys[base + deg + 1] = k_usr;       vals[base + deg + 1] = (uint32_t)b;
        if (part) {
          atomicAdd(&dh[((k_out & 255u) << 3) + rep], 1u);
          atomicAdd(&dh[((k_usr & 255u) << 3) + rep], 1u);
          const int d = (ko1 - ko0) >> 2;
          atomicAdd(&bh[255 - (d > 255 ? 255 : d)], 1u);
        }
      }
    }
    if (hot.slot) {
      __syncthreads();
      uint16_t *const m16 = reinterpret_cast<uint16_t *>(hot.mask);
      const size_t row = 2 * (size_t)hot.Bw;
      const bool tail = r + 1 == n_rounds && (size_t)r + 1 < row;
      for (int i = threadIdx.x; i < hot.H; i += kBlock) {
        m16[(size_t)i * row + r] = (uint16_t)hm[i];
        if (tail) m16[(size_t)i * row + r + 1] = 0;
        hm[i] = 0u;
      }
      __syncthreads();
    }
    c = n1; n1 = n2; u2 = u3;
#pragma unroll
    for (int k = 0; k < kPre; ++k) it[k] = itn[k];
  }
  if (part) {
    __syncthreads();
    uint32_t *const mine = part + (size_t)blockIdx.x * kPartialWords;
    for (int d = threadIdx.x; d < 256; d += kBlock) {
      uint32_t c = 0;
#pragma unroll
      for (int q = 0; q < 8; ++q) c += dh[(d << 3) + q];
      mine[d] = c;
      mine[256 + d] = bh[d];
    }
  }
}

static __global__ __launch_bounds__(1024) void k_degree_counts(const int32_t *__restrict__ keep_off, int B, unsigned int *__restrict__ work) {
  __shared__ unsigned int cnt[256];
  degree_counts_body<1024>(keep_off, B, work, (int)blockIdx.x, cnt);
}

template <int NT>
__device__ __forceinline__ void degree_scatter_body(const int32_t *__restrict__ keep_off, int B, unsigned int *__restrict__ work,
                                                    int32_t *__restrict__ order, int block_id, unsigned int *lds ) {
  unsigned int *start = lds, *cnt = lds + 256, *base = lds + 512;
  for (int i = threadIdx.x; i < 256; i += NT) cnt[i] = 0;
  if (threadIdx.x < 64) {
    unsigned int c[4], sum = 0;
#pragma unroll
    for (int q = 0; q < 4; ++q) { c[q] = work[threadIdx.x * 4 + q]; sum += c[q]; }
    unsigned int inc = sum;
#pragma unroll
    for (int o = 1; o < 64; o <<= 1) { const unsigned int t = __shfl_up(inc, o); if ((int)threadIdx.x >= o) inc += t; }
    unsigned int run = inc - sum;
#pragma unroll
    for (int q = 0; q < 4; ++q) { start[threadIdx.x * 4 + q] = run; run += c[q]; }
  }
  __syncthreads();
  const int b = block_id * NT + (int)threadIdx.x, lane = threadIdx.x & 63;
  const bool valid = b < B;
  const int d = valid ? degree_bucket(keep_off, b) : 0;
  const unsigned long long m = same_bucket_lanes(valid, d);
  const int leader = valid ? __ffsll((long long)m) - 1 : lane;
  unsigned int at = 0;
  if (valid && lane == leader) at = atomicAdd(&cnt[d], (unsigned int)__popcll(m));
  at = __shfl(at, leader);
  __syncthreads();
  for (int i = threadIdx.x; i < 256; i += NT) base[i] = cnt[i] ? atomicAdd(&work[256 + i], cnt[i]) : 0u;
  __syncthreads();
  if (valid) order[start[d] + base[d] + at + __popcll(m & ((1ull << lane) - 1ull))] = b;
}

static __global__ __launch_bounds__(1024) void k_degree_scatter(const int32_t *__restrict__ keep_off, int B, unsigned int *__restrict__ work,
                                                         int32_t *__restrict__ order) {
  __shared__ unsigned int lds[768];
  degree_scatter_body<1024>(keep_off, B, work, order, (int)blockIdx.x, lds);
}

static __global__ void k_mark_solo(uint32_t *keys_s, const uint32_t *__restrict__ vals_s, int T, uint32_t n_items, int B, uint8_t *solo_v,
                            uint8_t *solo_o) {
  for (int j = blockIdx.x * blockDim.x + threadIdx.x; j < T; j += gridDim.x * blockDim.x) {
    const uint32_t k = keys_s[j];
    if (k == DRX_KEY_NONE || k < n_items) continue;
    const uint32_t prev = j > 0 ? keys_s[j - 1] : DRX_KEY_NONE, next = j + 1 < T ? keys_s[j + 1] : DRX_KEY_NONE;
    if (k == prev || k == next) continue;
    const uint32_t b = vals_s[j];
    if (k < 2 * n_items) solo_o[b] = 1;
    else solo_v[b] = 1;
    keys_s[j] = DRX_KEY_NONE;
  }
}

static __global__ __launch_bounds__(256) void k_plan_and_mark(uint32_t *keys_s, const uint32_t *__restrict__ vals_s, int T, int n_chunks, int cpb,
                                                       SpanPlan P, uint32_t n_items, int B, uint8_t *solo_v, uint8_t *solo_o,
                                                       int order_blocks, const int32_t *keep_off, unsigned int *order_work,
                                                       int32_t *order) {
  const int plan_blocks = (int)gridDim.x - order_blocks;
  if ((int)blockIdx.x >= plan_blocks) {
    __shared__ unsigned int lds[768];
    degree_scatter_body<256>(keep_off, B, order_work, order, (int)blockIdx.x - plan_blocks, lds);
    return;
  }
  const int tid = blockIdx.x * blockDim.x + threadIdx.x;
  const int real = P.xrank ? (int)P.cnt[20] : 0;
  if (tid < n_chunks && (real == 0 || (long long)tid * P.chunk < (long long)real)) plan_chunk(keys_s, T, n_chunks, cpb, P, tid);
  const int nb = (n_chunks + cpb - 1) / cpb;
  if (P.xrank && (tid & ~63) < nb) place_block(keys_s, vals_s, T, cpb, B, P, tid, tid < nb);
  const int j_lo = real != 0 ? max(0, real - 2 * B) : 0, j_hi = real != 0 ? min(T, real) : T;
  for (int j = j_lo + tid; j < j_hi; j += plan_blocks * blockDim.x) {
    const uint32_t k = keys_s[j];
    if (k == DRX_KEY_NONE || k < n_items) continue;
    const uint32_t prev = j > 0 ? keys_s[j - 1] : DRX_KEY_NONE, next = j + 1 < T ? keys_s[j + 1] : DRX_KEY_NONE;
    if (k == prev || k == next) continue;
    const uint32_t b = vals_s[j];
    if (k < 2 * n_items) solo_o[b] = 1;
    else solo_v[b] = 1;
    keys_s[j] = DRX_KEY_NONE;
  }
}

struct BiasArgs {
  const float *dz1;
  float *part;
  const float *lossb;
  float *loss_out;
  int B, n_part, rows_per_block;
};

template <int G, int J, int NT>
__device__ __forceinline__ void bias_partial_body(int ld, const BiasArgs &A, int block_id, float *lds , float *red) {
  constexpr int R = (NT < kSegBlock ? NT : kSegBlock) / G;
  const int lane = threadIdx.x % G, r = threadIdx.x / G;
  const int b0 = block_id * A.rows_per_block, b1 = r < R ? min(A.B, b0 + A.rows_per_block) : 0;
  float4 acc[J];
#pragma unroll
  for (int j = 0; j < J; ++j) acc[j] = f4_zero();
  constexpr int NB = J == 1 ? 8 : 2;
  for (int b = b0 + r; b < b1; b += NB * R) {
    float4 v[NB][J];
#pragma unroll
    for (int q = 0; q < NB; ++q) {
#pragma unroll
      for (int j = 0; j < J; ++j) v[q][j] = f4_zero();
      if (b + q * R < b1) load_row<G, J>(A.dz1, (size_t)(b + q * R), ld, lane, v[q]);
    }
#pragma unroll
    for (int q = 0; q < NB; ++q)
#pragma unroll
      for (int j = 0; j < J; ++j) f4_add(acc[j], v[q][j]);
  }
  if (r < R) store_row<G, J>(lds, (size_t)r, ld, lane, acc);
  __syncthreads();
  if (r == 0) {
    float4 t[J];
#pragma unroll
    for (int j = 0; j < J; ++j) t[j] = f4_zero();
#pragma unroll 8
    for (int rr = 0; rr < R; ++rr) {
      float4 v[J];
      load_row<G, J>(lds, (size_t)rr, ld, lane, v);
#pragma unroll
      for (int j = 0; j < J; ++j) f4_add(t[j], v[j]);
    }
    store_row<G, J>(A.part, (size_t)block_id, ld, lane, t);
  }
  if (A.loss_out) {
    const int b1 = min(A.B, b0 + A.rows_per_block);
    float a = 0.f;
    for (int b = b0 + (int)threadIdx.x; b < b1; b += NT) a += A.lossb[b];
    const float tl = block_sum(a, red);
    if (threadIdx.x == 0) A.part[(size_t)A.n_part * ld + block_id] = tl;
  }
}

template <int G, int J, int NT = kSegBlock>
struct BiasPartialExtra {
  int ld;
  BiasArgs A;
  __device__ __forceinline__ void operator()(float *lds) const {
    __shared__ float red[NT / 64 > 0 ? NT / 64 : 1];
    bias_partial_body<G, J, NT>(ld, A, (int)blockIdx.x, lds, red);
  }
};

constexpr int kLongBlocks = 256, kShortBlocks = 1024;

struct __attribute__((aligned(32))) WorkItem { int32_t p0, n, user, deg; long long hist_start, pad_; };

struct PrepBufs {
  uint32_t *keys_s, *vals_s, *keys, *vals;
  void *sort_temp;
  size_t sort_bytes;
  uint8_t *solo_v, *solo_o;
  SpanPlan plan;
  int32_t *order;
  int32_t *usamp;
  int32_t *pitem;
  WorkItem *witem;
  int32_t *worder;
  int32_t *n_du;
  unsigned int *order_work;
  int n_chunks;
  size_t result_bytes;
  int T, bits;
  uint32_t *hmask;
  int H, Bw;
  uint32_t *partials;
  int partial_rows;
};

static inline bool long_segments(int T, const DrxCdaeParams &P) { return (int64_t)T > 8 * ((int64_t)2 * P.n_items + P.n_users); }

#ifndef DRX_STREAM_DEPTH
#define DRX_STREAM_DEPTH 4
#endif
constexpr int kStreamDepth = DRX_STREAM_DEPTH;
constexpr int kStreamIndexBits = 28;
constexpr int kHotMaxG = 32;

enum class ReduceForm { Streamed, PlannedLong, PlannedShort };

template <class Policy> struct PolicyKind;
template <template <int> class PolicyT, int KIND> struct PolicyKind<PolicyT<KIND>> { static constexpr int value = KIND; };
template <int G, int J, class Policy>
constexpr bool kStreamBuilt = kStreamDepth > 0 && J == 1 && G >= 16 && PolicyKind<Policy>::value == DRX_OPT_ADAGRAD;
template <int G, int J, class Policy>
constexpr bool kHotBuilt = kStreamBuilt<G, J, Policy> && G <= kHotMaxG;

static inline ReduceForm reduce_form(int opt_kind, int B, int T, const DrxCdaeParams &K) {
  if (long_segments(T, K)) return ReduceForm::PlannedLong;
  const Geom gm = pick_geom(K.ld);
  const bool streamed = kStreamDepth > 0 && gm.J == 1 && gm.G >= 16 && K.ld == 4 * gm.G && opt_kind == DRX_OPT_ADAGRAD &&
                        B < (1 << kStreamIndexBits) && K.n_items < (1 << kStreamIndexBits) && K.n_users < (1 << kStreamIndexBits);
  return streamed ? ReduceForm::Streamed : ReduceForm::PlannedShort;
}

static inline bool hot_list_fits(int T, const DrxCdaeParams &K, bool presence) { return !presence && !long_segments(T, K); }
static inline bool hot_head_fits(ReduceForm form, int ld, bool share, bool kshard) {
  return form == ReduceForm::Streamed && pick_geom(ld).G <= kHotMaxG && !share && !kshard;
}

static inline bool forward_per_workgroup(int B, int n_touch_slots) {
  const long long mean_hist = n_touch_slots / (long long)B;
  return mean_hist > 64 || (B <= 8192 && mean_hist > 16);
}
enum class ForwardForm { ColumnShard, SharedUsers, PerWorkgroup, PerGroup };
static inline ForwardForm forward_form(bool kshard, bool share, int B, int n_touch_slots) {
  if (kshard) return ForwardForm::ColumnShard;
  if (share) return ForwardForm::SharedUsers;
  return forward_per_workgroup(B, n_touch_slots) ? ForwardForm::PerWorkgroup : ForwardForm::PerGroup;
}

static inline hipError_t phase_event(void *const *events, int i, hipStream_t st) {
  return events ? hipEventRecord((hipEvent_t)events[i], st) : hipSuccess;
}

static PrepBufs prep_layout(Carver &cv, const DrxCdaeParams &P, int B, int n_touch_slots, int H = 0) {
  PrepBufs R{};
  R.T = n_touch_slots + 2 * B;
  R.bits = bits_for((uint64_t)2 * P.n_items + P.n_users + 1);
  R.keys_s = cv.take<uint32_t>(R.T);
  R.vals_s = cv.take<uint32_t>(R.T);
  R.solo_v = cv.take<uint8_t>((size_t)2 * B);
  R.solo_o = R.solo_v ? R.solo_v + B : nullptr;
  R.plan.chunk = seg_chunk(long_segments(R.T, P));
  R.n_chunks = (R.T + R.plan.chunk - 1) / R.plan.chunk;
  R.plan.desc = cv.take<uint2>(R.n_chunks);
  R.plan.cnt = cv.take<uint32_t>(128);
  R.plan.ext = cv.take<uint8_t>(R.n_chunks);
  {
    R.plan.xstride = (R.n_chunks + 1) / 2;
    const bool placed = long_segments(R.T, P);
    const bool placed_any = placed || DRX_STREAM_PLACED != 0;
    R.plan.xrank = placed_any ? cv.take<uint32_t>((size_t)R.plan.xstride) : nullptr;
    R.plan.xperm = placed_any ? cv.take<uint32_t>((size_t)R.plan.xstride) : nullptr;
    R.usamp = placed ? cv.take<int32_t>(B) : nullptr;
    R.pitem = placed ? cv.take<int32_t>(B) : nullptr;
    R.witem = placed ? cv.take<WorkItem>((size_t)B) : nullptr;
    R.worder = placed ? cv.take<int32_t>(B) : nullptr;
    R.n_du = placed ? cv.take<int32_t>(128) : nullptr;
  }
  R.order = cv.take<int32_t>(B);
  R.result_bytes = align_up(cv.off, 256);
  R.keys = cv.take<uint32_t>(R.T);
  R.vals = cv.take<uint32_t>(R.T);
  R.sort_bytes = sort_pairs_temp_bytes(R.T, R.bits);
  R.sort_temp = cv.take<char>(R.sort_bytes);
  R.order_work = cv.take<unsigned int>(512);
  R.H = H;
  R.Bw = (B + 31) / 32;
  R.hmask = H > 0 ? cv.take<uint32_t>((size_t)H * R.Bw) : nullptr;
  R.partial_rows = DRX_PREP_ROUNDS && sort_first_digit_bits(R.bits) == 8 ? touch_grid(B) : 0;
  R.partials = R.partial_rows > 0 ? cv.take<uint32_t>((size_t)R.partial_rows * kPartialWords) : nullptr;
  return R;
}

static int plan_zero_words(const PrepBufs &R) { return (int)(((const char *)R.plan.ext + R.n_chunks - (const char *)R.plan.cnt + 3) / 4); }

static int plan_spans(const DrxCdaeParams *p, const DrxBatch *bt, const PrepBufs &R0, hipStream_t st, bool cleared) {
  const PrepBufs &R = R0;
  if (!cleared) DRX_HIP(hipMemsetAsync(R.plan.cnt, 0, (size_t)plan_zero_words(R) * 4, st));
  hipLaunchKernelGGL(k_plan_spans<0>, dim3((R.n_chunks + 255) / 256), dim3(256), 0, st, R.keys_s, R.vals_s, R.T, R.n_chunks,
                     kSegBlock / pick_geom(p->ld).G, bt->B, R.plan);
  if (R.plan.xrank) hipLaunchKernelGGL(k_place_blocks, dim3(256), dim3(256), 0, st, R.plan, R.n_chunks);
  return DRX_OK;
}

static void order_by_degree(const DrxBatch *bt, const PrepBufs &R, hipStream_t st, bool cleared) {
  if (!cleared) (void)hipMemsetAsync(R.order_work, 0, 512 * sizeof(unsigned int), st);
  const int blocks = (bt->B + 1023) / 1024;
  hipLaunchKernelGGL(k_degree_counts, dim3(blocks), dim3(1024), 0, st, bt->keep_off, bt->B, R.order_work);
  hipLaunchKernelGGL(k_degree_scatter, dim3(blocks), dim3(1024), 0, st, bt->keep_off, bt->B, R.order_work, R.order);
}

constexpr int kTpFallback = 0x7fff0001;

static __global__ __launch_bounds__(256) void k_tp_begin(DrxBatch bt, int n_users, uint32_t *__restrict__ k2, uint32_t *__restrict__ v2,
                                                         int32_t *__restrict__ se, int n_se, uint8_t *solo, uint32_t *zero_a, int n_zero_a,
                                                         uint32_t *zero_b, int n_zero_b) {
  const int tid = blockIdx.x * blockDim.x + threadIdx.x, nt = gridDim.x * blockDim.x;
  for (int j = tid; j < 2 * bt.B; j += nt) {
    k2[j] = j < bt.B ? (uint32_t)bt.uid[j] : (uint32_t)n_users + (uint32_t)bt.iid[j - bt.B];
    v2[j] = (uint32_t)j;
  }
  for (int j = tid; j < n_se; j += nt) se[j] = 0;
  for (int j = tid; j < 2 * bt.B; j += nt) solo[j] = 0;
  for (int j = tid; j < n_zero_a; j += nt) zero_a[j] = 0u;
  for (int j = tid; j < n_zero_b; j += nt) zero_b[j] = 0u;
}

static __global__ __launch_bounds__(256) void k_tp_runs(const uint32_t *__restrict__ ks, int n, int32_t *__restrict__ start, int32_t *__restrict__ end) {
  for (int p = blockIdx.x * blockDim.x + threadIdx.x; p < n; p += gridDim.x * blockDim.x) {
    const uint32_t k = ks[p];
    if (p == 0 || ks[p - 1] != k) start[k] = p;
    if (p == n - 1 || ks[p + 1] != k) end[k] = p + 1;
  }
}

#ifndef DRX_ITEM_THREADS
#define DRX_ITEM_THREADS 256
#endif
constexpr int kShareTriples = 16;
static inline int share_item_triples(int) { return kShareTriples; }
constexpr int kItemThreads = DRX_ITEM_THREADS;
static inline size_t share_item_lds_bytes(int ld) { return ((size_t)(kItemThreads / 64) * kShareTriples * ld + kShareTriples) * 4; }
static inline bool share_geometry_ok(int ld) {
  const Geom g = pick_geom(ld);
  return g.G >= 16 && g.J <= 2 && share_item_lds_bytes(ld) <= 64 * 1024;
}

static __global__ __launch_bounds__(256) void k_tp_item_flags(const uint32_t *__restrict__ ks, int B, int rt, const int32_t *__restrict__ start,
                                                              int32_t *__restrict__ pitem, int32_t *n_du) {
  const int p = blockIdx.x * blockDim.x + threadIdx.x;
  if (blockIdx.x == 0 && threadIdx.x < 128) n_du[threadIdx.x] = 0;
  if (p < B) pitem[p] = ((p - start[ks[p]]) % rt == 0) ? 1 : 0;
}
__device__ __forceinline__ int tp_bucket_of(const int64_t *__restrict__ indptr, uint32_t u) {
  const long long d = (long long)(indptr[u + 1] - indptr[u]);
  return __clz((int)min(d, 0x7FFFFFFFll) | 1);
}
static __global__ __launch_bounds__(256) void k_tp_item_finish(const uint32_t *__restrict__ ks, const uint32_t *__restrict__ vs, int B, int rt,
                                                               const int32_t *__restrict__ start, const int32_t *__restrict__ end,
                                                               const int64_t *__restrict__ indptr, int32_t *__restrict__ usamp,
                                                               int32_t *__restrict__ pitem, WorkItem *__restrict__ witem, int32_t *n_du,
                                                               uint32_t *plan_cnt) {
  __shared__ int lcnt[32];
  if (threadIdx.x < 32) lcnt[threadIdx.x] = 0;
  __syncthreads();
  const int p = blockIdx.x * blockDim.x + threadIdx.x;
  if (p < B) {
    const int item = pitem[p] - 1;
    pitem[p] = item;
    usamp[p] = (int32_t)vs[p];
    const uint32_t u = ks[p];
    if ((p - start[u]) % rt == 0) {
      const long long hs = indptr[u], he = indptr[u + 1];
      witem[item] = WorkItem{p, min(rt, end[u] - p), (int32_t)u, (int32_t)min(he - hs, 0x7FFFFFFFll), hs, 0};
      atomicAdd(&lcnt[tp_bucket_of(indptr, u)], 1);
    }
    if (p == B - 1) { n_du[0] = item + 1; plan_cnt[21] = (uint32_t)(item + 1); }
  }
  __syncthreads();
  if (threadIdx.x < 32 && lcnt[threadIdx.x]) atomicAdd(&n_du[32 + threadIdx.x], lcnt[threadIdx.x]);
}
static __global__ __launch_bounds__(256) void k_tp_item_order(const uint32_t *__restrict__ ks, int B, int rt, const int32_t *__restrict__ start,
                                                              const int64_t *__restrict__ indptr, const int32_t *__restrict__ pitem,
                                                              int32_t *__restrict__ worder, int32_t *n_du) {
  __shared__ int lcnt[32], lbase[32];
  if (threadIdx.x < 32) lcnt[threadIdx.x] = 0;
  __syncthreads();
  const int p = blockIdx.x * blockDim.x + threadIdx.x;
  const bool head = p < B && (p - start[ks[p]]) % rt == 0;
  int b = 0, local = 0;
  if (head) { b = tp_bucket_of(indptr, ks[p]); local = atomicAdd(&lcnt[b], 1); }
  __syncthreads();
  if (threadIdx.x < 32) {
    const int t = threadIdx.x;
    int base = 0;
    for (int x = 0; x < t; ++x) base += n_du[32 + x];
    lbase[t] = lcnt[t] ? base + atomicAdd(&n_du[64 + t], lcnt[t]) : 0;
  }
  __syncthreads();
  if (head) worder[lbase[b] + local] = pitem[p];
}

template <bool SHARE>
static __global__ __launch_bounds__(256) void k_tp_count(DrxHistory H, DrxBatch bt, uint32_t qthr, int n_users, const int32_t *__restrict__ start,
                                                         const int32_t *__restrict__ end, const uint32_t *__restrict__ vs,
                                                         int *__restrict__ cnt, unsigned long long *__restrict__ km, int rt) {
  const int lane = threadIdx.x & 63, wv = threadIdx.x >> 6, nwv = blockDim.x >> 6;
  for (int u = blockIdx.x; u < n_users; u += gridDim.x) {
    const int s0 = start[u], c = end[u] - s0;
    const int64_t hs = H.indptr[u];
    const int deg = (int)(H.indptr[u + 1] - hs);
    if (c <= 0) {
      for (int j = wv * 64 + lane; j < deg; j += nwv * 64) cnt[H.t_rank[hs + j]] = 0;
      continue;
    }
    for (int j = wv * 64 + lane; j < deg; j += nwv * 64) {
      const int e = H.t_rank[hs + j];
      unsigned long long bits = 0ull;
      int kept = 0;
      for (int q0 = 0; q0 < c; q0 += rt) {
        const int nq = min(c - q0, rt);
        uint32_t m = 0;
        for (int q = 0; q < nq; ++q) {
          const uint32_t b = vs[s0 + q0 + q];
          m |= ((bt.keep ? (bt.keep[bt.keep_off[b] + j] != 0) : (hash_u32(bt.mask_seed, b, (uint32_t)j) >= qthr)) ? 1u : 0u) << q;
        }
        if (q0 < 64) bits |= (unsigned long long)m << q0;
        const int k = __popc(m);
        kept += (SHARE && nq > 1 && 1 + (nq - k) < k) ? 1 + (nq - k) : k;
      }
      cnt[e] = kept;
      km[e] = bits;
    }
  }
}

template <bool SHARE>
static __global__ __launch_bounds__(256) void k_tp_write(DrxHistory H, DrxBatch bt, uint32_t qthr, const int32_t *__restrict__ start,
                                                         const int32_t *__restrict__ end, const uint32_t *__restrict__ vs,
                                                         const int *__restrict__ cnt, const unsigned long long *__restrict__ km,
                                                         uint32_t *__restrict__ keys_s, uint32_t *__restrict__ vals_s,
                                                         const int32_t *__restrict__ pitem, int rt, int32_t *__restrict__ row_end) {
  const int64_t nnz = H.t_nnz;
  for (int64_t e = (int64_t)blockIdx.x * blockDim.x + threadIdx.x; e < nnz; e += (int64_t)gridDim.x * blockDim.x) {
    const int u = H.t_users[e];
    const int s0 = start[u], c = end[u] - s0;
    const uint32_t n = (uint32_t)H.t_items[e];
    const bool last_of_item = e + 1 == nnz || (uint32_t)H.t_items[e + 1] != n;
    if (last_of_item && e + 1 < nnz) row_end[n] = cnt[e + 1];
    if (c <= 0) {
      if (last_of_item && e + 1 == nnz) row_end[n] = cnt[e];
      continue;
    }
    const unsigned long long bits = km[e];
    int at = cnt[e];
    for (int q0 = 0; q0 < c; q0 += rt) {
      const int nq = min(c - q0, rt);
      uint32_t m;
      if (q0 + nq <= 64) m = (uint32_t)(bits >> q0) & (nq >= 32 ? 0xFFFFFFFFu : ((1u << nq) - 1u));
      else {
        const int j = H.t_pos[e];
        m = 0;
        for (int q = 0; q < nq; ++q) {
          const uint32_t b = vs[s0 + q0 + q];
          m |= ((bt.keep ? (bt.keep[bt.keep_off[b] + j] != 0) : (hash_u32(bt.mask_seed, b, (uint32_t)j) >= qthr)) ? 1u : 0u) << q;
        }
      }
      const int k = __popc(m);
      const bool shared = SHARE && nq > 1 && 1 + (nq - k) < k;
      if (shared) { keys_s[at] = n; vals_s[at] = (uint32_t)bt.B + (uint32_t)pitem[s0 + q0]; ++at; }
      uint32_t em = shared ? (~m & (nq >= 32 ? 0xFFFFFFFFu : ((1u << nq) - 1u))) : m;
      while (em) {
        const int q = __ffs((int)em) - 1;
        em &= em - 1u;
        const uint32_t b = vs[s0 + q0 + q];
        keys_s[at] = n; vals_s[at] = shared ? (b | 0x80000000u) : b; ++at;
      }
    }
    if (last_of_item && e + 1 == nnz) row_end[n] = at;
  }
}

static __global__ __launch_bounds__(256) void k_tp_tail(const uint32_t *__restrict__ ks, const uint32_t *__restrict__ vs, int B, int n_users,
                                                        int n_items, const int *__restrict__ off_last, const int *__restrict__ cnt_last, int T,
                                                        uint32_t *__restrict__ keys_s, uint32_t *__restrict__ vals_s, uint32_t *plan_cnt) {
  const int Tw = off_last[0] + cnt_last[0];
  if (blockIdx.x == 0 && threadIdx.x == 0) plan_cnt[20] = (uint32_t)(Tw + 2 * B);
  const int n_tail = min(T - Tw, 2 * B + (kSegBlock / 4 + 1) * kChunkLong);
  for (int p = blockIdx.x * blockDim.x + threadIdx.x; p < n_tail; p += gridDim.x * blockDim.x) {
    uint32_t k = DRX_KEY_NONE, v = 0;
    if (p < B) { k = (uint32_t)n_items + (ks[B + p] - (uint32_t)n_users); v = vs[B + p] - (uint32_t)B; }
    else if (p < 2 * B) { k = 2u * (uint32_t)n_items + ks[p - B]; v = vs[p - B]; }
    keys_s[Tw + p] = k; vals_s[Tw + p] = v;
  }
}

static int plan_zero_words(const PrepBufs &R);
static void order_by_degree(const DrxBatch *bt, const PrepBufs &R, hipStream_t st, bool cleared);

static bool transposed_applies(const DrxCdaeParams *p, const DrxHistory *hist, const DrxBatch *bt, const PrepBufs &R) {
  if (!hist->t_rank || !hist->t_users || !hist->t_pos || !hist->t_items || !long_segments(R.T, *p)) return false;
  const int B = bt->B, U = p->n_users, N = p->n_items;
  const int64_t nnz = hist->t_nnz;
  if (nnz < 1 || nnz > (int64_t)R.T || nnz >= (1ll << 30) || (int64_t)U + N >= 0x7FFFFFFFll) return false;
  Carver cw(nullptr, R.sort_bytes);
  for (int i = 0; i < 4; ++i) (void)cw.take<uint32_t>((size_t)2 * B);
  (void)cw.take<int32_t>((size_t)U + N); (void)cw.take<int32_t>((size_t)U + N);
  (void)cw.take<char>(sort_pairs_temp_bytes((size_t)2 * B, bits_for((uint64_t)U + (uint64_t)N + 1)));
  (void)cw.take<char>(scan_i32_temp_bytes((size_t)nnz));
  (void)cw.take<char>(scan_i32_temp_bytes((size_t)B));
  (void)cw.take<unsigned long long>((size_t)nnz);
  (void)cw.take<int32_t>((size_t)N);
  return cw.ok();
}
static bool share_users(const DrxCdaeParams *p, const DrxHistory *hist, const DrxBatch *bt, const PrepBufs &R) {
  return (bt->flags & DRX_BATCH_SHARE_USERS) != 0 && R.pitem != nullptr && share_geometry_ok(p->ld) &&
         transposed_applies(p, hist, bt, R);
}

static int prepare_transposed(const DrxCdaeParams *p, const DrxHistory *hist, const DrxBatch *bt, const PrepBufs &R, hipStream_t st,
                              bool allow_share, const int32_t **row_end_out) {
  const int B = bt->B, U = p->n_users, N = p->n_items;
  if (!transposed_applies(p, hist, bt, R)) return kTpFallback;
  const bool share = allow_share && share_users(p, hist, bt, R);
  const int64_t nnz = hist->t_nnz;
  if (nnz < 1 || nnz > (int64_t)R.T || nnz >= (1ll << 30) || (int64_t)U + N >= 0x7FFFFFFFll) return kTpFallback;
  int *cnt = (int *)R.keys;
  Carver cw(R.sort_temp, R.sort_bytes);
  const int bits2 = bits_for((uint64_t)U + (uint64_t)N + 1);
  uint32_t *k2 = cw.take<uint32_t>((size_t)2 * B), *v2 = cw.take<uint32_t>((size_t)2 * B);
  uint32_t *ks = cw.take<uint32_t>((size_t)2 * B), *vs = cw.take<uint32_t>((size_t)2 * B);
  int32_t *start = cw.take<int32_t>((size_t)U + N), *end = start + ((size_t)U + N);
  (void)cw.take<int32_t>((size_t)U + N);
  const size_t sb = sort_pairs_temp_bytes((size_t)2 * B, bits2);
  void *stemp = cw.take<char>(sb);
  const size_t scb = scan_i32_temp_bytes((size_t)nnz);
  void *sctemp = cw.take<char>(scb);
  const size_t scb2 = scan_i32_temp_bytes((size_t)B);
  void *sctemp2 = cw.take<char>(scb2);
  unsigned long long *km = cw.take<unsigned long long>((size_t)nnz);
  int32_t *row_end = cw.take<int32_t>((size_t)N);
  if (!cw.ok()) return kTpFallback;
  *row_end_out = row_end;
  const uint32_t qthr = q_threshold(bt->q);
  hipLaunchKernelGGL(k_tp_begin, dim3(512), dim3(256), 0, st, *bt, U, k2, v2, start, 2 * (U + N), R.solo_v, R.plan.cnt, plan_zero_words(R),
                     R.order_work, 512);
  int rc = sort_pairs(stemp, sb, k2, ks, v2, vs, (size_t)2 * B, bits2, st);
  if (rc) return rc;
  hipLaunchKernelGGL(k_tp_runs, dim3((2 * B + 255) / 256 < 1024 ? (2 * B + 255) / 256 : 1024), dim3(256), 0, st, ks, 2 * B, start, end);
  const int egrid = U < (1 << 20) ? U : (1 << 20);
  const int wgrid = (int)((nnz + 255) / 256 < 16384 ? (nnz + 255) / 256 : 16384);
  const int rt = share_item_triples(p->ld);
  if (share) {
    const int ig = (B + 255) / 256;
    hipLaunchKernelGGL(k_tp_item_flags, dim3(ig), dim3(256), 0, st, ks, B, rt, start, R.pitem, R.n_du);
    rc = scan_i32(sctemp2, scb2, R.pitem, R.pitem, (size_t)B, true, st);
    if (rc) return rc;
    hipLaunchKernelGGL(k_tp_item_finish, dim3(ig), dim3(256), 0, st, ks, vs, B, rt, start, end, hist->indptr, R.usamp, R.pitem, R.witem,
                       R.n_du, R.plan.cnt);
    hipLaunchKernelGGL(k_tp_item_order, dim3(ig), dim3(256), 0, st, ks, B, rt, start, hist->indptr, R.pitem, R.worder, R.n_du);
    hipLaunchKernelGGL((k_tp_count<true>), dim3(egrid), dim3(256), 0, st, *hist, *bt, qthr, U, start, end, vs, cnt, km, rt);
  } else
    hipLaunchKernelGGL((k_tp_count<false>), dim3(egrid), dim3(256), 0, st, *hist, *bt, qthr, U, start, end, vs, cnt, km, rt);
  int *cnt_last = (int *)R.vals;
  DRX_HIP(hipMemcpyAsync(cnt_last, cnt + (nnz - 1), sizeof(int), hipMemcpyDeviceToDevice, st));
  rc = scan_i32(sctemp, scb, cnt, cnt, (size_t)nnz, false, st);
  if (rc) return rc;
  if (share)
    hipLaunchKernelGGL((k_tp_write<true>), dim3(wgrid), dim3(256), 0, st, *hist, *bt, qthr, start, end, vs, cnt, km, R.keys_s, R.vals_s, R.pitem, rt, row_end);
  else
    hipLaunchKernelGGL((k_tp_write<false>), dim3(wgrid), dim3(256), 0, st, *hist, *bt, qthr, start, end, vs, cnt, km, R.keys_s, R.vals_s, R.pitem, rt, row_end);
  hipLaunchKernelGGL(k_tp_tail, dim3(2048), dim3(256), 0, st, ks, vs, B, U, N, cnt + (nnz - 1), cnt_last, R.T, R.keys_s, R.vals_s, R.plan.cnt);
  return DRX_OK;
}

static void launch_touches(const DrxCdaeParams *p, const DrxHistory *hist, const DrxBatch *bt, const PrepBufs &R, hipStream_t st,
                           TouchPresence pres, const int16_t *hot_slot, const int32_t *hot_item) {
  const int gpb = kBlock / 16;
  (void)gpb;
  uint32_t *sort_zero = nullptr;
  size_t sort_zero_words = 0;
  sort_pairs_zero_region(R.sort_temp, (size_t)R.T, R.bits, &sort_zero, &sort_zero_words);
  const HotMark hm{R.H > 0 ? hot_slot : nullptr, R.hmask, R.H, R.Bw, hot_item, hot_table_bits(R.H)};
#if DRX_PREP_ROUNDS
  hipLaunchKernelGGL(k_sparse_touches_rounds, dim3(touch_grid(bt->B)), dim3(kBlock), hot_table_lds_bytes(R.H), st, p->n_items, *hist, *bt,
                     q_threshold(bt->q), R.keys, R.vals, R.T, R.solo_v, R.plan.cnt, plan_zero_words(R), R.order_work, 512,
                     sort_zero, (int)sort_zero_words, pres, hm, R.partials);
#else
  hipLaunchKernelGGL(k_sparse_touches, dim3((bt->B + gpb - 1) / gpb), dim3(kBlock), hot_table_lds_bytes(R.H), st, p->n_items, *hist, *bt,
                     q_threshold(bt->q), R.keys, R.vals, R.T, R.solo_v, R.plan.cnt, plan_zero_words(R), R.order_work, 512,
                     sort_zero, (int)sort_zero_words, pres, hm);
#endif
}

static int prepare_impl(const DrxCdaeParams *p, const DrxHistory *hist, const DrxBatch *bt, const PrepBufs &R, hipStream_t st,
                        bool with_marks = false, TouchPresence pres = TouchPresence{nullptr, WireGeo{1, 0, 1}},
                        const int16_t *hot_slot = nullptr, const int32_t *hot_item = nullptr) {
  if (R.H > 0 && (!hot_slot || !hot_item || !hot_list_fits(R.T, *p, pres.present != nullptr))) return DRX_EINVAL;
  if (hist->t_rank && hist->t_users && hist->t_pos && hist->t_items && !pres.present && long_segments(R.T, *p)) {
    const int32_t *row_end = nullptr;
    const int rc = prepare_transposed(p, hist, bt, R, st, with_marks, &row_end);
    if (rc == DRX_OK) {
      PrepBufs Rb = R;
      Rb.plan.row_end = row_end;
      Rb.plan.row_end_keys = (uint32_t)p->n_items;
      if (with_marks && p->ld > 16) {
        if (!share_users(p, hist, bt, R)) order_by_degree(bt, R, st, true);
        const int blocks = std::max(2048, (R.n_chunks + 255) / 256);
        hipLaunchKernelGGL(k_plan_and_mark, dim3(blocks), dim3(256), 0, st, R.keys_s, R.vals_s, R.T, R.n_chunks,
                           kSegBlock / pick_geom(p->ld).G, Rb.plan, (uint32_t)p->n_items, bt->B, R.solo_v, R.solo_o, 0, bt->keep_off,
                           R.order_work, R.order);
        if (R.plan.xrank) hipLaunchKernelGGL(k_place_blocks, dim3(256), dim3(256), 0, st, Rb.plan, R.n_chunks);
        return DRX_OK;
      }
      return plan_spans(p, bt, Rb, st, true);
    }
    if (rc != kTpFallback) return rc;
  }
  launch_touches(p, hist, bt, R, st, pres, hot_slot, hot_item);
  const bool fused_order = with_marks && p->ld > 16;
  const SortRider rider{fused_order ? bt->keep_off : nullptr, bt->B, R.order_work, R.partials, R.partial_rows};
  const int rc = sort_pairs_ex(R.sort_temp, R.sort_bytes, R.keys, R.keys_s, R.vals, R.vals_s, (size_t)R.T, R.bits, true, st, true, rider);
  if (rc) return rc;
  if (with_marks && p->ld > 16) {
    const int blocks = std::max(2048, (R.n_chunks + 255) / 256);
    const int order_blocks = (bt->B + 255) / 256;
    hipLaunchKernelGGL(k_plan_and_mark, dim3(blocks + order_blocks), dim3(256), 0, st, R.keys_s, R.vals_s, R.T, R.n_chunks,
                       kSegBlock / pick_geom(p->ld).G, R.plan, (uint32_t)p->n_items, bt->B, R.solo_v, R.solo_o,
                       order_blocks, bt->keep_off, R.order_work, R.order);
    if (R.plan.xrank) hipLaunchKernelGGL(k_place_blocks, dim3(256), dim3(256), 0, st, R.plan, R.n_chunks);
    return DRX_OK;
  }
  return plan_spans(p, bt, R, st, true);
}

static int mark_solo(const DrxCdaeParams *p, const DrxBatch *bt, const PrepBufs &R, hipStream_t st, bool cleared) {
  if (!cleared) {
    DRX_HIP(hipMemsetAsync(R.solo_v, 0, (size_t)bt->B * 2, st));
  }
  if (p->ld <= 16) return DRX_OK;
  hipLaunchKernelGGL(k_mark_solo, dim3(2048), dim3(256), 0, st, R.keys_s, R.vals_s, R.T, (uint32_t)p->n_items, bt->B, R.solo_v,
                     R.solo_o);
  return DRX_OK;
}


}
```

drecpy_amd/engine.py:

```python
import ctypes as C
import math

import os
import time
import weakref

import numpy as np
import torch

from . import _lib
from ._lib import Batch, CdaeParams, History, Optim, check, lib, ptr, stream_ptr
from .engine_rows import ADAM_B1, ADAM_B2, ADAM_EPS, RowsRecommender, _round_up, pack_mask_bits

VAR_ORDER = ('W', 'W2T', 'V', 'b', 'b2')
ADAGRAD_INIT, ADAGRAD_EPS = 0.1, 1e-7


def _forget_prepared(addr):
    try:
        lib().drx_cdae_prep_forget(addr)
    except Exception:
        pass


# ... 252 lines not shown
            st['host'][k] = torch.empty(int(total * 1.25) + 4096, dtype=torch.uint8, pin_memory=True)
            st['ev'][k] = torch.cuda.Event()
            st['busy'][k] = False
            st['views'][k] = None
        if st['busy'][k]:
            st['ev'][k].synchronize()
            st['busy'][k] = False
        v = st['views'][k]
        if v is None or v[0] != (B, int(keep_capacity)):
            hv = st['host'][k].numpy()
            extra = (np.empty(B, np.int32), np.empty(B, np.float64), np.empty(B, np.uint8))
            uid_v, ko_v, kp_v = hv[:4 * B].view(np.int32), hv[off_ko:off_ko + 4 * (B + 1)].view(np.int32), hv[off_kp:off_kp + max(int(keep_capacity), 1)]
            ptrs = (uid_v.ctypes.data, extra[0].ctypes.data, extra[1].ctypes.data, extra[2].ctypes.data, ko_v.ctypes.data, kp_v.ctypes.data,
                    len(kp_v))
            v = st['views'][k] = ((B, int(keep_capacity)), (k, off_ko, off_kp), uid_v, ko_v, kp_v, extra, ptrs)
        return v[1], v[2], v[3], v[4]

    def stage_extra(self, slot):
        return self._slots['views'][slot[0]][5]

    def stage_pointers(self, slot):
        return self._slots['views'][slot[0]][6]

    def batch_in_slot(self, slot, B, n_keep, q):
        k, off_ko, off_kp = slot
        base = self._slots['host'][k].data_ptr()
        return Batch(B, base, None, None, base + off_ko, base + off_kp, 0, float(q), int(n_keep))

    def stage_release(self, slot):
        st = self._slots
        st['ev'][slot[0]].record(torch.cuda.current_stream(self.device))
        st['busy'][slot[0]] = True

    def _batch_flags(self, n_touch_slots):
        return _lib.BATCH_SHARE_USERS if (self.share_users and getattr(self, '_hist_t', None) is not None) else 0

    def make_batch(self, uid, iid=None, y=None, keep_off=None, keep=None, q=0.0, mask_seed=0, n_touch_slots=None):
        if (keep_off is not None and n_touch_slots is not None and self.device.type == 'cuda'
                and not any(torch.is_tensor(a) for a in (uid, iid, y, keep_off, keep))):
            return self._make_batch_staged(uid, iid, y, keep_off, keep, q, mask_seed, n_touch_slots)
        uid = self._dev(uid, torch.int32)
        B = int(uid.numel())
        if keep_off is None:
            keep_off = _lib.batch_offsets(self.hist_indptr, uid)
        else:
            keep_off = self._dev(keep_off, torch.int32)
        if n_touch_slots is None:
            n_touch_slots = int(keep_off[-1].item())
        iid = self._dev(iid, torch.int32)
        y = self._dev(y, torch.float32)
        keep = self._dev(keep, torch.uint8)
        if keep is not None and keep.numel() == 0:
            keep = torch.zeros(1, dtype=torch.uint8, device=self.device)
        bt = Batch(B, ptr(uid), ptr(iid), ptr(y), ptr(keep_off), ptr(keep), int(mask_seed) & (2 ** 64 - 1), float(q),
                   int(n_touch_slots), self._batch_flags(n_touch_slots))
        return bt, (uid, iid, y, keep_off, keep)

    def _ensure_scratch(self, B, n_touch_slots, dense=False, hot=0):
        if dense:
            return self._ensure_dense_scratch(B)
        need = lib().drx_cdae_scratch_bytes_hot(C.byref(self._params), B, n_touch_slots, hot) if hot else \
            lib().drx_cdae_scratch_bytes(C.byref(self._params), B, n_touch_slots, 0)
        if self._scratch is None or self._scratch.numel() < need:
            self._scratch = None
            self._scratch = torch.empty(int(need * 1.1) + 1024, dtype=torch.uint8, device=self.device)
        return self._scratch

    def _ensure_dense_scratch(self, B):
        pool = self.__dict__.setdefault('_dense_pool', {})
        ent = pool.get(B)
        if ent is None:
            if len(pool) >= 4:
                pool.pop(next(iter(pool)))
            need = lib().drx_cdae_scratch_bytes(C.byref(self._params), B, 0, 1)
            ent = pool[B] = [torch.zeros(int(need) + 1024, dtype=torch.uint8, device=self.device), True]
        elif not ent[1]:
            ent[0].zero_()
            ent[1] = True
        self._dense_scratch, self._dense_scratch_B, self._dense_clean = ent[0], B, True
        self._dense_ent = ent
        return ent[0]

    def dense_fault(self):
        for ent in self.__dict__.get('_dense_pool', {}).values():
            ent[1] = False

    def forward(self, uid, keep_off=None, keep=None, q=0.0, mask_seed=0, want_pred=True):
        bt, alive = self.make_batch(uid, keep_off=keep_off, keep=keep, q=q, mask_seed=mask_seed, n_touch_slots=0)
        h = torch.empty(bt.B, self.ld, dtype=torch.float32, device=self.device)
        pred = torch.empty(bt.B, self.n_items, dtype=torch.float32, device=self.device) if want_pred else None
        check(lib().drx_cdae_forward(C.byref(self._params), C.byref(self._hist), C.byref(bt), ptr(h), ptr(pred),
                                     stream_ptr(self.device)), 'drx_cdae_forward')
        return h[:, :self.k], pred

    def step_dense(self, step, bt, loss='bce', targets='reference', want_loss=False):
        o = self._optim(self._dense_alphas(step))
        sc = self._ensure_dense_scratch(bt.B)
        self._dense_clean = self._dense_ent[1] = False
        check(lib().drx_cdae_step_dense(
            C.byref(self._params), C.byref(o), C.byref(self._hist), C.byref(bt),
            _lib.LOSS_BCE if loss == 'bce' else _lib.LOSS_MSE,
            (_lib.TARGETS_REFERENCE if targets == 'reference' else _lib.TARGETS_PER_ROW) | _lib.DENSE_AUX_CLEAN,
            ptr(sc), sc.numel(), ptr(self._loss) if want_loss else None, stream_ptr(self.device)),
            'drx_cdae_step_dense')
        self._dense_clean = self._dense_ent[1] = True
        return self._loss if want_loss else None

    _FIT_SLOTS = 16

    def fit_dense(self, drawahead, cursor, B, q, keep_capacity, first_step, n_steps, loss='bce', targets='reference'):
        L = lib()
        need = int(L.drx_cdae_fit_slot_bytes(B, int(keep_capacity)))
        slots = getattr(self, '_fit_slots', None)
        if slots is None or slots[0] < need:
            slots = self._fit_slots = (need, torch.empty(need * self._FIT_SLOTS, dtype=torch.uint8, pin_memory=True),
                                       torch.empty(2 * need, dtype=torch.uint8, device=self.device))
        o = self._optim([0.0] * 5)
        sc = self._ensure_dense_scratch(B)
        alphas = self._alpha_table(first_step, n_steps)
        self._dense_clean = self._dense_ent[1] = False
        check(L.drx_cdae_fit_dense(
            C.byref(self._params), C.byref(o), C.byref(self._hist), drawahead, cursor.ctypes.data, B, float(q), int(keep_capacity),
            _lib.LOSS_BCE if loss == 'bce' else _lib.LOSS_MSE, _lib.TARGETS_REFERENCE if targets == 'reference' else _lib.TARGETS_PER_ROW,
            n_steps, alphas.ctypes.data, slots[1].data_ptr(), slots[0], self._FIT_SLOTS, ptr(slots[2]), slots[2].numel(), ptr(sc),
            sc.numel(), stream_ptr(self.device)),
            'drx_cdae_fit_dense')
        self._dense_clean = self._dense_ent[1] = True

    def _retire(self, t):
        t.record_stream(torch.cuda.default_stream(self.device))
        t.record_stream(torch.cuda.current_stream(self.device))

    def prep_buffer(self, bt, out=None, hot=0):
        need = lib().drx_cdae_prep_bytes_hot(C.byref(self._params), bt.B, bt.n_touch_slots, hot) if hot else \
            lib().drx_cdae_prep_bytes(C.byref(self._params), bt.B, bt.n_touch_slots)
        if out is None or out.numel() < need:
            out = None
            out = torch.empty(int(need * 1.03) + 4096, dtype=torch.uint8, device=self.device)
        return out

    def prep_result_bytes(self, bt):
        return int(lib().drx_cdae_prep_result_bytes(C.byref(self._params), bt.B, bt.n_touch_slots))

    def prepare_sparse(self, bt, out=None, hot=False):
        H = self._hot_for(bt) if hot else 0
        out = self.prep_buffer(bt, out, H)
        if H:
            check(lib().drx_cdae_sparse_prepare_hot(C.byref(self._params), C.byref(self._hist), C.byref(bt), C.byref(self._hot_head(H)),
                                                    ptr(out), out.numel(), stream_ptr(self.device)), 'drx_cdae_sparse_prepare_hot')
        else:
            check(lib().drx_cdae_sparse_prepare(C.byref(self._params), C.byref(self._hist), C.byref(bt), ptr(out), out.numel(),
                                                stream_ptr(self.device)), 'drx_cdae_sparse_prepare')
        out._drx_hot = H
        if H and not getattr(out, '_drx_forget', None):
            out._drx_forget = weakref.finalize(out, _forget_prepared, out.data_ptr())
        return out

    def prepare_part(self, bt, part, parts, slot=None):
        P = C.byref(self._params)
        nb = int(lib().drx_cdae_prep_part_out_bytes(P, bt.B, bt.n_touch_slots, parts))
        if slot is None:
            out = torch.empty(nb, dtype=torch.uint8, device=self.device)
        else:
            bufs = self.__dict__.setdefault('_part_bufs', {})
            if slot not in bufs or bufs[slot].numel() < nb:
                if bufs.get(slot) is not None:
                    self._retire(bufs[slot])
                bufs[slot] = None
                bufs[slot] = torch.empty(int(nb * 1.05) + 4096, dtype=torch.uint8, device=self.device)
            out = bufs[slot][:nb]
        need = lib().drx_cdae_prep_part_bytes(P, bt.B, bt.n_touch_slots, parts)
        if getattr(self, '_pscratch', None) is None or self._pscratch.numel() < need:
            if getattr(self, '_pscratch', None) is not None:
                self._retire(self._pscratch)
            self._pscratch = None
            self._pscratch = torch.empty(int(need * 1.1) + 1024, dtype=torch.uint8, device=self.device)
        check(lib().drx_cdae_sparse_prepare_part(P, C.byref(self._hist), C.byref(bt), part, parts, ptr(out), out.numel(),
                                                 ptr(self._pscratch), self._pscratch.numel(), stream_ptr(self.device)),
              'drx_cdae_sparse_prepare_part')
        return out

    def prepare_assemble(self, bt, all_parts, parts, out=None, overflow=None):
        need = lib().drx_cdae_prep_bytes(C.byref(self._params), bt.B, bt.n_touch_slots)
        if out is None or out.numel() < need:
            out = torch.empty(int(need), dtype=torch.uint8, device=self.device)
        if overflow is None:
            overflow = torch.zeros(1, dtype=torch.int32, device=self.device)
        check(lib().drx_cdae_sparse_prepare_assemble(C.byref(self._params), C.byref(bt), ptr(all_parts), parts, ptr(out), out.numel(),
                                                     ptr(overflow), stream_ptr(self.device)), 'drx_cdae_sparse_prepare_assemble')
        return out, overflow

    def kshard_forward(self, bt, prepared=None):
        h = torch.empty(bt.B, self.ld, dtype=torch.float32, device=self.device)
        d = torch.empty(bt.B, dtype=torch.float32, device=self.device)
        check(lib().drx_cdae_kshard_forward_prepared(C.byref(self._params), C.byref(self._hist), C.byref(bt), ptr(prepared),
                                                     prepared.numel() if prepared is not None else 0, ptr(h), ptr(d),
                                                     stream_ptr(self.device)), 'drx_cdae_kshard_forward_prepared')
        return h, d

    def step_sparse(self, step, bt, loss='bce', want_loss=False, events=None, prepared=None, kshard=None, hot=False):
        a = self.adam_alpha(self.lr, step + 1, self.beta1, self.beta2)
        o = self._optim([a] * 5)
        H = int(getattr(prepared, '_drx_hot', 0)) if prepared is not None else (self._hot_for(bt) if hot else 0)
        sc = self._ensure_scratch(bt.B, bt.n_touch_slots, hot=H)
        lk = _lib.LOSS_BCE if loss == 'bce' else _lib.LOSS_MSE
        lo = ptr(self._loss) if want_loss else None
        arr = (C.c_void_p * len(events))(*[e.cuda_event for e in events]) if events is not None else None
        if H:
            if kshard is not None:
                raise _lib.DrxError('the column-sharded step takes no hot head')
            check(lib().drx_cdae_step_sparse_hot(C.byref(self._params), C.byref(o), C.byref(self._hist), C.byref(bt),
                                                 C.byref(self._hot_head(H)), lk, ptr(prepared) if prepared is not None else None,
                                                 prepared.numel() if prepared is not None else 0, ptr(sc), sc.numel(), lo, arr,
                                                 stream_ptr(self.device)), 'drx_cdae_step_sparse_hot')
            return self._loss if want_loss else None
        if kshard is not None:
            h, dot_total = kshard
            check(lib().drx_cdae_kshard_step(C.byref(self._params), C.byref(o), C.byref(self._hist), C.byref(bt), lk, ptr(h),
                                             ptr(dot_total), ptr(prepared) if prepared is not None else None,
                                             prepared.numel() if prepared is not None else 0, ptr(sc), sc.numel(), lo, arr,
                                             stream_ptr(self.device)), 'drx_cdae_kshard_step')
            return self._loss if want_loss else None
        if prepared is not None:
            check(lib().drx_cdae_step_sparse_prepared(C.byref(self._params), C.byref(o), C.byref(self._hist), C.byref(bt),
                                                      lk, ptr(prepared), prepared.numel(), ptr(sc), sc.numel(), lo, arr,
                                                      stream_ptr(self.device)), 'drx_cdae_step_sparse_prepared')
        elif events is None:
            check(lib().drx_cdae_step_sparse(C.byref(self._params), C.byref(o), C.byref(self._hist), C.byref(bt), lk,
                                             ptr(sc), sc.numel(), lo, stream_ptr(self.device)), 'drx_cdae_step_sparse')
        else:
            check(lib().drx_cdae_step_sparse_timed(C.byref(self._params), C.byref(o), C.byref(self._hist), C.byref(bt),
                                                   lk, ptr(sc), sc.numel(), lo, arr, stream_ptr(self.device)),
                  'drx_cdae_step_sparse_timed')
        return self._loss if want_loss else None

    def sample_device(self, B, neg_ratio, seed, n_items=None, out=None, mailbox=None, tag=0):
        if out is None:
            out = (torch.empty(B, dtype=torch.int32, device=self.device), torch.empty(B, dtype=torch.int32, device=self.device),
                   torch.empty(B, dtype=torch.float32, device=self.device), torch.empty(B + 1, dtype=torch.int32, device=self.device))
        uid, iid, y, keep_off = out
        by_user = getattr(self, '_hist_t', None) is not None and self.sample_by_user
        need = lib().drx_point_sample_by_user_scratch_bytes(B, self.n_users) if by_user else lib().drx_point_sample_scratch_bytes(B)
        pool = self.__dict__.setdefault('_sscratch', {})
        key = torch.cuda.current_stream(self.device).cuda_stream
        if pool.get(key) is None or pool[key].numel() < need:
            pool[key] = torch.empty(need, dtype=torch.uint8, device=self.device)
        scratch = pool[key]
        rec = getattr(self, '_recorded', None)
        fn = lib().drx_point_sample_by_user if by_user else lib().drx_point_sample_recorded
        check(fn(C.byref(self._hist), C.byref(rec[0]) if rec is not None else None, self.n_users,
                 n_items or self.n_items, B, neg_ratio, int(seed) & (2 ** 64 - 1), ptr(uid), ptr(iid), ptr(y),
                 ptr(keep_off), ptr(scratch), scratch.numel(), ptr(mailbox), int(tag) & 0xFFFFFFFF,
                 stream_ptr(self.device)),
              'drx_point_sample_by_user' if by_user else 'drx_point_sample_recorded')
        return out

    RECOMMEND_FALLBACK_BYTES = 1 << 30
    RECOMMEND_MIN_FUSED_USERS = 1

    def _hidden_rows(self, uid):
        bt, alive = self.make_batch(uid, n_touch_slots=0)
        h = torch.empty(bt.B, self.ld, dtype=torch.float32, device=self.device)
        check(lib().drx_cdae_forward(C.byref(self._params), C.byref(self._hist), C.byref(bt), ptr(h), None, stream_ptr(self.device)),
              'drx_cdae_forward')
        return h

    EPILOGUE = _lib.DRX_REC_SIGMOID_BIAS
    _query_rows = _hidden_rows

    def rank_ld(self):
        return self.ld

    def _score_table(self, items=None):
        return self.W2T, self.b2

    def _recommend_fused(self, R, n):
        return R >= self.RECOMMEND_MIN_FUSED_USERS and self.recommend_is_fused(self.ld, n)

    def _recommend_by_matrix(self, uid, n, excl, out_idx, out_val):
        R = int(uid.numel())
        chunk = self.matrix_chunk_users(self.n_items, self.RECOMMEND_FALLBACK_BYTES)
        host_uid = uid.cpu().numpy()
        k = min(n, self.n_items)
        for lo in range(0, R, chunk):
            u = uid[lo:lo + chunk]
            r = int(u.numel())
            _, pred = self.forward(u)
            idx, val = self.topk(pred, k) if excl is None else self.masked_topk(pred, self._exclusion_mask(host_uid[lo:lo + r]), k)
            out_idx[lo:lo + r, :k] = idx
            out_val[lo:lo + r, :k] = val
            if k < n:
                out_idx[lo:lo + r, k:] = -1
                out_val[lo:lo + r, k:] = float('-inf')
        return out_idx, out_val


class DeviceBatchSource:

    AHEAD = 2

    def __init__(self, eng, batch_size, neg_ratio, q, sample_seed_of, mask_seed_of, n_items=None, slots=8, stream_slot=2):
        self.eng, self.B, self.neg_ratio, self.q = eng, int(batch_size), int(neg_ratio), float(q)
        self.sample_seed_of, self.mask_seed_of, self.n_items = sample_seed_of, mask_seed_of, n_items
        self.stream = run_ahead_stream(eng.device, int(stream_slot))
        self.stream.wait_stream(torch.cuda.current_stream(eng.device))
        self.n_slots = slots
        self.ring = [None] * slots
# ... 258 lines not shown
```

include/drx.h:

```cpp
#ifndef DRX_H_
#define DRX_H_

#include <stddef.h>
#include <stdint.h>

#ifdef __cplusplus
extern "C" {
#endif

#define DRX_VERSION 100

enum {
  DRX_OK = 0,
  DRX_EINVAL = -1,
  DRX_ESCRATCH = -2,
  DRX_ENOTIMPL = -3,
  DRX_ERETRY = -4,
  DRX_ECOMM = -5
};

#define DRX_MAX_K 1024
#define DRX_KEY_NONE 0xFFFFFFFFu

enum { DRX_LOSS_BCE = 0, DRX_LOSS_MSE = 1 };
enum { DRX_TARGETS_REFERENCE = 0, DRX_TARGETS_PER_ROW = 1 };
#define DRX_DENSE_AUX_CLEAN 0x100
enum { DRX_OPT_ADAM = 0, DRX_OPT_ADAGRAD = 1,
       DRX_OPT_ROWWISE_ADAGRAD = 2,
       DRX_OPT_SGD = 3,
       DRX_OPT_MOMENTUM = 4,
       DRX_OPT_NESTEROV = 5,
       DRX_OPT_RMSPROP = 6,
       DRX_OPT_RMSPROP_MOMENTUM = 7   };

typedef struct DrxOptRule {
  int32_t kind;
  float lr, mu, mu2, eps;
} DrxOptRule;

typedef struct DrxCdaeParams {
  int32_t n_users, n_items, k, ld;
  float *W;
  float *W2T;
  float *V;
  float *b;
  float *b2;
} DrxCdaeParams;

typedef struct DrxHistory {
  const int64_t *indptr;
  const int32_t *indices;
  const int32_t *t_rank;
  int64_t t_nnz;
  const int32_t *t_users;
  const int32_t *t_pos;
  const int32_t *t_items;
} DrxHistory;

typedef struct DrxBatch {
  int32_t B;
  const int32_t *uid;
  const int32_t *iid;
  const float   *y;
  const int32_t *keep_off;
  const uint8_t *keep;
  uint64_t mask_seed;
  float q;
  int32_t n_touch_slots;
  uint32_t flags;
} DrxBatch;
#define DRX_BATCH_SHARE_USERS 1u

typedef struct DrxOptim {
  int32_t kind;
  float lr, reg_rate;
  float beta1, beta2, eps;
  float alpha[5];
  float *s1[5];
  float *s2[5];
} DrxOptim;

int drx_version(void);
const char *drx_strerror(int code);

void *drx_event_create(void);
void drx_event_destroy(void *ev);
int drx_event_record(void *ev, void *stream);
int drx_stream_wait_event(void *stream, void *ev);
int drx_event_synchronize(void *ev);

void *drx_stream_create_cu_slice(int32_t cus_per_xcd);
void drx_stream_destroy(void *stream);

uint32_t drx_hash_u32(uint64_t seed, uint32_t a, uint32_t b);

int drx_cdae_forward(const DrxCdaeParams *p, const DrxHistory *hist, const DrxBatch *bt,
                     float *h, float *pred, void *stream);

size_t drx_cdae_scratch_bytes(const DrxCdaeParams *p, int32_t B, int32_t n_touch_slots, int32_t dense_mode);

int drx_cdae_step_dense(const DrxCdaeParams *p, const DrxOptim *opt, const DrxHistory *hist,
                        const DrxBatch *bt, int32_t loss_kind, int32_t targets_kind,
                        void *scratch, size_t scratch_bytes, float *loss_out, void *stream);

int drx_cdae_step_sparse(const DrxCdaeParams *p, const DrxOptim *opt, const DrxHistory *hist,
                         const DrxBatch *bt, int32_t loss_kind,
                         void *scratch, size_t scratch_bytes, float *loss_out, void *stream);

#define DRX_SPARSE_PHASES 5
int drx_cdae_step_sparse_timed(const DrxCdaeParams *p, const DrxOptim *opt, const DrxHistory *hist,
                               const DrxBatch *bt, int32_t loss_kind, void *scratch, size_t scratch_bytes,
                               float *loss_out, void *const *events, void *stream);

size_t drx_cdae_prep_bytes(const DrxCdaeParams *p, int32_t B, int32_t n_touch_slots);
int drx_cdae_sparse_prepare(const DrxCdaeParams *p, const DrxHistory *hist, const DrxBatch *bt, void *prepared,
                            size_t prepared_bytes, void *stream);
int drx_cdae_step_sparse_prepared(const DrxCdaeParams *p, const DrxOptim *opt, const DrxHistory *hist, const DrxBatch *bt,
                                  int32_t loss_kind, const void *prepared, size_t prepared_bytes, void *scratch,
                                  size_t scratch_bytes, float *loss_out, void *const *events, void *stream);

typedef struct DrxHotHead {
  int32_t H;
  const int16_t *slot;
  const int32_t *item;
} DrxHotHead;
#define DRX_MAX_HOT 1024
size_t drx_cdae_prep_bytes_hot(const DrxCdaeParams *p, int32_t B, int32_t n_touch_slots, int32_t H);
size_t drx_cdae_scratch_bytes_hot(const DrxCdaeParams *p, int32_t B, int32_t n_touch_slots, int32_t H);
int drx_cdae_sparse_prepare_hot(const DrxCdaeParams *p, const DrxHistory *hist, const DrxBatch *bt, const DrxHotHead *hot,
                                void *prepared, size_t prepared_bytes, void *stream);
int drx_cdae_step_sparse_hot(const DrxCdaeParams *p, const DrxOptim *opt, const DrxHistory *hist, const DrxBatch *bt,
                             const DrxHotHead *hot, int32_t loss_kind, const void *prepared, size_t prepared_bytes, void *scratch,
                             size_t scratch_bytes, float *loss_out, void *const *events, void *stream);
int32_t drx_cdae_hot_rows_for(const DrxCdaeParams *p, int32_t opt_kind, int32_t B, int32_t n_touch_slots, int32_t H);
void drx_cdae_prep_forget(const void *prepared);

int drx_debug_prep_counts(const DrxCdaeParams *p, const DrxHistory *hist, const DrxBatch *bt, const DrxHotHead *hot, uint8_t *present,
                          int32_t ipr, int32_t cshift, int32_t world, void *prepared, size_t prepared_bytes, uint32_t *hist_out,
                          uint32_t *buckets_out, uint32_t *keys_out, uint32_t *vals_out, uint32_t *mask_out, int32_t *info_out,
                          void *stream);

int drx_debug_prep_result(const DrxCdaeParams *p, int32_t B, int32_t n_touch_slots, int32_t H, const void *prepared, size_t prepared_bytes,
                          uint32_t *keys_s_out, uint32_t *vals_s_out, uint8_t *solo_v_out, uint8_t *solo_o_out, int32_t *order_out,
                          void *stream);

int drx_debug_cdae_reduce(const DrxCdaeParams *p, const DrxOptim *opt, const DrxHistory *hist, const DrxBatch *bt, const DrxHotHead *hot,
                          const void *prepared, size_t prepared_bytes, const float *dz1_in, const float *g2_in, const float *dz2_in,
                          int32_t form, void *scratch, size_t scratch_bytes, void *stream);

int drx_debug_span_plan(const DrxCdaeParams *p, int32_t B, int32_t n_touch_slots, int32_t H, const void *prepared, size_t prepared_bytes,
                        uint8_t *ext_out, uint32_t *desc_out, uint32_t *cnt_out, void *stream);

int drx_batch_offsets(const int64_t *indptr, const int32_t *ids, int32_t B, int32_t *off, void *scratch, size_t scratch_bytes, void *stream);

size_t drx_point_sample_scratch_bytes(int32_t B);
int drx_point_sample(const DrxHistory *hist, int32_t n_users, int32_t n_items, int32_t B, int32_t neg_ratio,
                     uint64_t seed, int32_t *uid, int32_t *iid, float *y, int32_t *keep_off,
                     void *scratch, size_t scratch_bytes, uint64_t *host_mailbox, uint32_t tag, void *stream);
int drx_point_sample_recorded(const DrxHistory *hist, const DrxHistory *recorded, int32_t n_users, int32_t n_items, int32_t B,
                              int32_t neg_ratio, uint64_t seed, int32_t *uid, int32_t *iid, float *y, int32_t *keep_off,
                              void *scratch, size_t scratch_bytes, uint64_t *host_mailbox, uint32_t tag, void *stream);

size_t drx_point_sample_by_user_scratch_bytes(int32_t B, int32_t n_users);
int drx_point_sample_by_user(const DrxHistory *hist, const DrxHistory *recorded, int32_t n_users, int32_t n_items, int32_t B,
                             int32_t neg_ratio, uint64_t seed, int32_t *uid, int32_t *iid, float *y, int32_t *keep_off, void *scratch,
                             size_t scratch_bytes, uint64_t *host_mailbox, uint32_t tag, void *stream);

int drx_point_sample_valued(const DrxHistory *hist, const DrxHistory *recorded, const float *pos_values, float vmin, float vrange,
                            int32_t n_users, int32_t n_items, int32_t B, int32_t neg_ratio, uint64_t seed, int32_t *uid, int32_t *iid,
                            float *y, void *stream);

typedef struct DrxListGroups {
  const int64_t *indptr;
  const int32_t *seq_ids;
  const int64_t *held_indptr;
  const int32_t *held;
  const int32_t *group_value;
  const int32_t *eligible;
  int32_t n_groups, n_eligible, n_ids;
} DrxListGroups;
int drx_list_sample_device(const DrxListGroups *g, int32_t B, int32_t n_inputs, int32_t n_targets, int32_t neg_ratio, uint64_t seed,
                           int32_t *group_out, int32_t *before, int32_t *after, void *stream);

int drx_cdae_kshard_forward(const DrxCdaeParams *p, const DrxHistory *hist, const DrxBatch *bt, float *h_out ,
                            float *dot_partial , void *stream);
int drx_cdae_kshard_forward_prepared(const DrxCdaeParams *p, const DrxHistory *hist, const DrxBatch *bt, const void *prepared,
                                     size_t prepared_bytes, float *h_out , float *dot_partial , void *stream);
int drx_cdae_kshard_step(const DrxCdaeParams *p, const DrxOptim *opt, const DrxHistory *hist, const DrxBatch *bt, int32_t loss_kind,
                         const float *h, const float *dot_total, const void *prepared, size_t prepared_bytes, void *scratch,
                         size_t scratch_bytes, float *loss_out, void *const *events, void *stream);

size_t drx_cdae_prep_result_bytes(const DrxCdaeParams *p, int32_t B, int32_t n_touch_slots);

size_t drx_cdae_prep_part_out_bytes(const DrxCdaeParams *p, int32_t B, int32_t n_touch_slots, int32_t parts);
int drx_cdae_prep_part_layout(const DrxCdaeParams *p, int32_t B, int32_t n_touch_slots, int32_t parts, size_t *out4);
size_t drx_cdae_prep_part_bytes(const DrxCdaeParams *p, int32_t B, int32_t n_touch_slots, int32_t parts);
int drx_cdae_sparse_prepare_part(const DrxCdaeParams *p, const DrxHistory *hist, const DrxBatch *bt, int32_t part, int32_t parts,
                                 void *part_out, size_t part_out_bytes, void *scratch, size_t scratch_bytes, void *stream);
int drx_cdae_sparse_prepare_assemble(const DrxCdaeParams *p, const DrxBatch *bt, const void *all_parts, int32_t parts, void *prepared,
                                     size_t prepared_bytes, int32_t *overflow_out, void *stream);

#define DRX_MAX_WORLD 64
#define DRX_MAX_MICRO 4
#define DRX_MAX_CHUNKS 16
typedef struct DrxShard {
  int32_t world, rank;
  int32_t n_items;
  int32_t items_per_rank;
  int32_t n_users_local;
  uint32_t flags;
  int32_t chunks;
} DrxShard;
int32_t drx_shard_chunks(const DrxShard *sh);
int32_t drx_shard_unit_shift(const DrxShard *sh);
#define DRX_SHARD_SELF_BYPASS 1u

size_t drx_shard_prep_bytes(const DrxCdaeParams *p, const DrxShard *sh, int32_t B, int32_t n_touch_slots);
size_t drx_shard_work_bytes(const DrxShard *sh);
int drx_shard_prep_layout(const DrxCdaeParams *p, const DrxShard *sh, int32_t B, int32_t n_touch_slots, size_t *out4);
int drx_shard_prepare(const DrxCdaeParams *p, const DrxShard *sh, const DrxHistory *hist, const DrxBatch *bt, void *prepared,
                      size_t prepared_bytes, void *work, size_t work_bytes, void *stream);
size_t drx_shard_owner_table_bytes(const DrxShard *sh, int32_t n_segments);
int drx_shard_owner_index(const DrxShard *sh, const uint32_t *recv_keys, int32_t n, const int32_t *recv_counts, int32_t n_segments,
                          int32_t chunk, void *table, size_t table_bytes, void *stream);
int drx_shard_gather_rows(const DrxCdaeParams *p, const DrxShard *sh, const uint32_t *recv_keys, int32_t n, const int32_t *recv_counts,
                          int32_t n_segments, float *out, void *stream);
size_t drx_shard_step_scratch_bytes(const DrxCdaeParams *p, int32_t B, int32_t n_touch_slots);
int drx_shard_step_local(const DrxCdaeParams *p, const DrxOptim *opt, const DrxShard *sh, const DrxHistory *hist, const DrxBatch *bt,
                         const void *prepared, size_t prepared_bytes, const float *rows_cache, float *grad_send, int32_t b_norm,
                         int32_t loss_kind, void *scratch, size_t scratch_bytes, void *const *events, void *stream);
int drx_shard_apply(const DrxCdaeParams *p, const DrxOptim *opt, const DrxShard *sh, int32_t b_norm, const uint32_t *recv_keys,
                    const float *grad_recv, int32_t n, const int32_t *recv_counts, int32_t n_segments, int32_t chunk, const void *table,
                    const float *const *own_grad, const int64_t *own_off, float *loss_out, void *stream);

#define DRX_COMM_ID_BYTES 128
#define DRX_COMM_THREAD 1u
typedef struct DrxComm DrxComm;
int drx_comm_unique_id(void *id128);
int drx_comm_create(const void *id128, int32_t world, int32_t rank, uint32_t flags, DrxComm **out);
int drx_comm_destroy(DrxComm *c);
void *drx_comm_stream(DrxComm *c);
int64_t drx_comm_alltoallv(DrxComm *c, const void *send, const int64_t *send_off, const int64_t *send_bytes, void *recv,
                           const int64_t *recv_off, const int64_t *recv_bytes, void *after_stream);
int drx_comm_wait(DrxComm *c, int64_t ticket, void *stream);
const char *drx_comm_last_error(void);

typedef struct DrxShardExchange {
  const int64_t *send_counts;
  const int64_t *recv_counts;
  const uint32_t *uniq;
  uint32_t *req;
  void *table;
  size_t table_bytes;
  float *rows_cache;
  float *rows_send;
  float *grad_send;
  float *grad_recv;
  int64_t rows_ticket[DRX_MAX_CHUNKS];
  int64_t grad_ticket[DRX_MAX_CHUNKS];
} DrxShardExchange;
int drx_shard_exchange_sizes(const DrxCdaeParams *p, const DrxShard *sh, const int64_t *send_counts, const int64_t *recv_counts,
                             int64_t *sizes4);
int drx_shard_phase_layout(const DrxCdaeParams *p, const DrxShard *sh, const int64_t *send_counts, const int64_t *recv_counts, int32_t chunk,
                           int64_t *out);
int drx_shard_phase_keys(const DrxShard *sh, DrxComm *comm, DrxShardExchange *x, void *stream);
int drx_shard_phase_rows(const DrxCdaeParams *p, const DrxShard *sh, DrxComm *comm, DrxShardExchange *x, int32_t chunk, void *stream);
int drx_shard_phase_local(const DrxCdaeParams *p, const DrxOptim *opt, const DrxShard *sh, const DrxHistory *hist, const DrxBatch *bt,
                          DrxComm *comm, DrxShardExchange *x, const void *prepared, size_t prepared_bytes, int32_t b_norm,
                          int32_t loss_kind, void *scratch, size_t scratch_bytes, void *const *events, void *stream);
int drx_shard_phase_tail(const DrxCdaeParams *p, const DrxOptim *opt, const DrxShard *sh, DrxComm *comm, DrxShardExchange *x,
                         DrxShardExchange *next, int32_t b_norm, float *loss_out, void *stream);

int drx_copy_f4(void *dst, const void *src, size_t n_bytes, void *stream);
int drx_copy_f4_variant(void *dst, const void *src, size_t n_bytes, int32_t variant, void *stream);

int drx_adam_dense(float *p, float *m, float *v, const float *g, int64_t n, float alpha, float l2_coef, float beta1, float beta2,
                   float eps, void *stream);
size_t drx_scatter_scratch_bytes(int32_t ld, int32_t n_touches, int32_t n_rows);
int drx_rows_csr_adam(const int32_t *row_ptr, const int32_t *order, const float *src, const float *src_s, int32_t ld, int32_t n_rows,
                      float *p, float *m, float *v, float *p_s, float *m_s, float *v_s, float alpha, float alpha_s, float l2_coef,
                      float beta1, float beta2, float eps, void *stream);
int drx_rows_csr_adam_outer(const int32_t *row_ptr, const int32_t *order, const float *scale, const float *src, int32_t group, int32_t ld,
                            int32_t n_rows, float *p, float *m, float *v, float *p_s, float *m_s, float *v_s, float alpha, float alpha_s,
                            float l2_coef, float beta1, float beta2, float eps, void *stream);
#define DRX_MAX_CSR_TABLES 4
typedef struct DrxCsrAdamTable {
  const int32_t *row_ptr, *order;
  const float *src, *scale;
  int32_t group, ld, n_rows;
  float *p, *m, *v, *p_s, *m_s, *v_s;
  float alpha, alpha_s, l2_coef;
} DrxCsrAdamTable;
int drx_rows_csr_adam_multi(const DrxCsrAdamTable *tables, int32_t n_tables, float beta1, float beta2, float eps, void *stream);
int drx_opt_dense(float *p, float *s1, float *s2, const float *g, int64_t n, const DrxOptRule *rule, float l2_coef, void *stream);
int drx_rows_csr_opt(const int32_t *row_ptr, const int32_t *order, const float *src, const float *src_s, int32_t ld, int32_t n_rows,
                     float *p, float *s1, float *s2, float *p_s, float *s1_s, float *s2_s, float alpha, float alpha_s, float l2_coef,
                     const DrxOptRule *rule, void *stream);
// ... 366 lines not shown
```

Baseline: 223.0 million samples/s.

## Prepare per-slot gather lists and records for the forward kernel on the side stream

```diff
diff --git a/drecpy_amd/_lib.py b/drecpy_amd/_lib.py
--- a/drecpy_amd/_lib.py
+++ b/drecpy_amd/_lib.py
@@ -182,6 +182,8 @@
                                         C.c_void_p, C.c_void_p, C.POINTER(C.c_int32), C.c_void_p]),
     'drx_debug_prep_result': (C.c_int, [C.POINTER(CdaeParams), C.c_int32, C.c_int32, C.c_int32, C.c_void_p, C.c_size_t, C.c_void_p,
                                         C.c_void_p, C.c_void_p, C.c_void_p, C.c_void_p, C.c_void_p]),
+    'drx_debug_prep_gather': (C.c_int, [C.POINTER(CdaeParams), C.c_int32, C.c_int32, C.c_int32, C.c_void_p, C.c_size_t, C.c_void_p,
+                                        C.c_void_p, C.c_void_p, C.c_void_p]),
     'drx_debug_cdae_reduce': (C.c_int, [C.POINTER(CdaeParams), C.POINTER(Optim), C.POINTER(History), C.POINTER(Batch), C.POINTER(HotHead),
                                         C.c_void_p, C.c_size_t, C.c_void_p, C.c_void_p, C.c_void_p, C.c_int32, C.c_void_p, C.c_size_t,
                                         C.c_void_p]),
diff --git a/drecpy_amd/csrc/drx_cdae.hip b/drecpy_amd/csrc/drx_cdae.hip
--- a/drecpy_amd/csrc/drx_cdae.hip
+++ b/drecpy_amd/csrc/drx_cdae.hip
@@ -31,6 +31,8 @@
   const int32_t *order;
   const int32_t *usamp, *worder, *n_items;
   const WorkItem *witem;
+  const int4 *rec;
+  const int32_t *gl;
   int T, n_chunks, n_bpart;
 };
 
@@ -62,23 +64,26 @@
 }
 
 template <int G, int J>
+__device__ __forceinline__ float sampled_hidden(const DrxCdaeParams &P, int u, int i, float scale, int lane,
+                                                const float4 (&acc)[J], float4 (&h)[J], float4 (&w2)[J]) {
+  hidden_act<G, J>(P, u, scale, lane, acc, h);
+  load_row<G, J>(P.W2T, (size_t)i, P.ld, lane, w2);
+  float d = 0.f;
+#pragma unroll
+  for (int j = 0; j < J; ++j) d += f4_dot(w2[j], h[j]);
+  return group_sum<G>(d);
+}
+template <int G, int J>
 __device__ __forceinline__ float sampled_hidden(const DrxCdaeParams &P, const DrxBatch &bt, float scale, int b, int lane,
                                                 const float4 (&acc)[J], float4 (&h)[J], float4 (&w2)[J]) {
-  hidden_act<G, J>(P, bt.uid[b], scale, lane, acc, h);
-  load_row<G, J>(P.W2T, (size_t)bt.iid[b], P.ld, lane, w2);
-  float d = 0.f;
-#pragma unroll
-  for (int j = 0; j < J; ++j) d += f4_dot(w2[j], h[j]);
-  return group_sum<G>(d);
+  return sampled_hidden<G, J>(P, bt.uid[b], bt.iid[b], scale, lane, acc, h, w2);
 }
 
 template <int G, int J, int KIND = -1>
 __device__ __forceinline__ void sampled_rest(const DrxCdaeParams &P, const DrxOptim &opt, const DrxHistory &H, const DrxBatch &bt,
-                                             float scale, uint32_t qthr, int loss_kind, const SparseBufs &S, int b, int lane,
-                                             float d, const float4 (&h)[J], const float4 (&w2)[J],
+                                             float scale, uint32_t qthr, int loss_kind, const SparseBufs &S, int b, int u, int i, float y,
+                                             int lane, float d, const float4 (&h)[J], const float4 (&w2)[J],
                                              float4 (*dz1_out)[J] = nullptr) {
-  const int u = bt.uid[b], i = bt.iid[b];
-  const float y = bt.y[b];
   const float p = sigmoidf_(d + P.b2[i]);
   const float invB = 1.0f / (float)bt.B;
   float lval, dp;
@@ -108,21 +113,34 @@
     for (int j = 0; j < J; ++j) (*dz1_out)[j] = dz1[j];
   }
 }
-
+template <int G, int J, int KIND = -1>
+__device__ __forceinline__ void sampled_rest(const DrxCdaeParams &P, const DrxOptim &opt, const DrxHistory &H, const DrxBatch &bt,
+                                             float scale, uint32_t qthr, int loss_kind, const SparseBufs &S, int b, int lane,
+                                             float d, const float4 (&h)[J], const float4 (&w2)[J],
+                                             float4 (*dz1_out)[J] = nullptr) {
+  sampled_rest<G, J, KIND>(P, opt, H, bt, scale, qthr, loss_kind, S, b, bt.uid[b], bt.iid[b], bt.y[b], lane, d, h, w2, dz1_out);
+}
+
+template <int G, int J, int KIND = -1>
+__device__ __forceinline__ void sampled_finish(const DrxCdaeParams &P, const DrxOptim &opt, const DrxHistory &H, const DrxBatch &bt,
+                                               float scale, uint32_t qthr, int loss_kind, const SparseBufs &S, int b, int u, int i, float y,
+                                               int lane, const float4 (&acc)[J]) {
+  float4 h[J], w2[J];
+#ifdef DRX_STAMPS
+  if (acc[0].x == acc[0].x) DRX_STAMP(S.stamps, b, 5, lane);
+#endif
+  const float d = sampled_hidden<G, J>(P, u, i, scale, lane, acc, h, w2);
+#ifdef DRX_STAMPS
+  if (d == d) DRX_STAMP(S.stamps, b, 6, lane);
+#endif
+  sampled_rest<G, J, KIND>(P, opt, H, bt, scale, qthr, loss_kind, S, b, u, i, y, lane, d, h, w2);
+  DRX_STAMP(S.stamps, b, 7, lane);
+}
 template <int G, int J, int KIND = -1>
 __device__ __forceinline__ void sampled_finish(const DrxCdaeParams &P, const DrxOptim &opt, const DrxHistory &H, const DrxBatch &bt,
                                                float scale, uint32_t qthr, int loss_kind, const SparseBufs &S, int b, int lane,
                                                const float4 (&acc)[J]) {
-  float4 h[J], w2[J];
-#ifdef DRX_STAMPS
-  if (acc[0].x == acc[0].x) DRX_STAMP(S.stamps, b, 5, lane);
-#endif
-  const float d = sampled_hidden<G, J>(P, bt, scale, b, lane, acc, h, w2);
-#ifdef DRX_STAMPS
-  if (d == d) DRX_STAMP(S.stamps, b, 6, lane);
-#endif
-  sampled_rest<G, J, KIND>(P, opt, H, bt, scale, qthr, loss_kind, S, b, lane, d, h, w2);
-  DRX_STAMP(S.stamps, b, 7, lane);
+  sampled_finish<G, J, KIND>(P, opt, H, bt, scale, qthr, loss_kind, S, b, bt.uid[b], bt.iid[b], bt.y[b], lane, acc);
 }
 
 template <int G, int J>
@@ -181,15 +199,74 @@
   sampled_rest<G, J>(P, opt, H, bt, scale, qthr, loss_kind, S, b, lane, dot_total[b], h, w2);
 }
 
-template <int G, int J, int KIND = -1>
-__global__ __launch_bounds__(kBlock) void k_sampled_fwd_bwd(DrxCdaeParams P, DrxOptim opt, DrxHistory H, DrxBatch bt, float scale,
-                                                            uint32_t qthr, int loss_kind, SparseBufs S) {
+#ifndef DRX_FWD_PREPARED_GATHER
+#define DRX_FWD_PREPARED_GATHER 1
+#endif
+#ifndef DRX_FWD_THREADS
+#define DRX_FWD_THREADS 256
+#endif
+constexpr int kFwdThreads = DRX_FWD_THREADS;
+template <int G, int J> constexpr bool kPreparedGatherBuilt = DRX_FWD_PREPARED_GATHER != 0 && J == 1 && (G == 16 || G == 32);
+
+template <int G, int J>
+__device__ __forceinline__ void gather_prepared(const DrxCdaeParams &P, const int32_t *__restrict__ gl, int ko, int n, int b, int lane,
+                                                float4 (&acc)[J], unsigned long long *stamps) {
+  (void)stamps; (void)b;
+#pragma unroll
+  for (int j = 0; j < J; ++j) acc[j] = f4_zero();
+  constexpr int NF = J == 1 ? DRX_GATHER_ROWS : 4;
+#ifdef DRX_STAMPS
+  bool first_rows = true;
+#endif
+  for (int c = 0; c < n; c += G) {
+    const int here = n - c < G ? n - c : G;
+    const int id = lane < here ? gl[ko + c + lane] : 0;
+#ifdef DRX_STAMPS
+    if (first_rows && id >= 0) DRX_STAMP(stamps, b, 3, lane);
+#endif
+    for (int t = 0; t < here; t += NF) {
+      float4 r[NF][J];
+#pragma unroll
+      for (int q = 0; q < NF; ++q) {
+        const bool on = t + q < here;
+        const int iq = __shfl(id, (t + q) % G, G);
+#pragma unroll
+        for (int jx = 0; jx < J; ++jx) r[q][jx] = f4_zero();
+        if (on) load_row<G, J>(P.W, (size_t)iq, P.ld, lane, r[q]);
+      }
+#pragma unroll
+      for (int q = 0; q < NF; ++q)
+#pragma unroll
+        for (int jx = 0; jx < J; ++jx) f4_add(acc[jx], r[q][jx]);
+#ifdef DRX_STAMPS
+      if (first_rows && acc[0].x == acc[0].x) { DRX_STAMP(stamps, b, 4, lane); first_rows = false; }
+#endif
+    }
+  }
+}
+
+template <int G, int J, int KIND = -1, int NT = kFwdThreads, bool PG = false>
+__global__ __launch_bounds__(NT) void k_sampled_fwd_bwd(DrxCdaeParams P, DrxOptim opt, DrxHistory H, DrxBatch bt, float scale,
+                                                        uint32_t qthr, int loss_kind, SparseBufs S) {
   const int lane = threadIdx.x % G;
-  const int slot = blockIdx.x * (kBlock / G) + threadIdx.x / G;
+  const int slot = blockIdx.x * (NT / G) + threadIdx.x / G;
 #ifdef DRX_STAMPS
   const unsigned long long t_in = wall_clock64();
 #endif
   if (slot >= bt.B) return;
+  if constexpr (PG) {
+    const int4 *const rp = S.rec + 2 * (size_t)slot;
+    const int4 r0 = rp[0], r1 = rp[1];
+    const int b = r0.x;
+    float4 acc[J];
+#ifdef DRX_STAMPS
+    if (lane == 0 && S.stamps && (unsigned)b < 110000u) S.stamps[(size_t)b * 16] = t_in;
+    if (r1.y >= 0) { DRX_STAMP(S.stamps, b, 1, lane); DRX_STAMP(S.stamps, b, 2, lane); }
+#endif
+    gather_prepared<G, J>(P, S.gl, r1.x, r1.y, b, lane, acc, S.stamps);
+    sampled_finish<G, J, KIND>(P, opt, H, bt, scale, qthr, loss_kind, S, b, r0.y, r0.z, __int_as_float(r0.w), lane, acc);
+    return;
+  }
   const int32_t *const ord = S.order;
   const int b = ord ? ord[slot] : slot;
   float4 acc[J];
@@ -649,17 +726,23 @@
   return S;
 }
 
+struct PrepRecord { int H; bool gather; int B, n_touch_slots; };
 static std::mutex g_hot_mu;
-static std::unordered_map<const void *, int> g_hot_of;
-static void hot_record(const void *prepared, int H) {
+static std::unordered_map<const void *, PrepRecord> g_hot_of;
+static void hot_record(const void *prepared, int H, bool gather = false, int B = 0, int n_touch_slots = 0) {
   std::lock_guard<std::mutex> lk(g_hot_mu);
-  if (H > 0) g_hot_of[prepared] = H;
+  if (H > 0 || gather) g_hot_of[prepared] = PrepRecord{H, gather, B, n_touch_slots};
   else g_hot_of.erase(prepared);
 }
 static int hot_recorded(const void *prepared) {
   std::lock_guard<std::mutex> lk(g_hot_mu);
   const auto it = g_hot_of.find(prepared);
-  return it == g_hot_of.end() ? 0 : it->second;
+  return it == g_hot_of.end() ? 0 : it->second.H;
+}
+static bool gather_recorded(const void *prepared, int B, int n_touch_slots) {
+  std::lock_guard<std::mutex> lk(g_hot_mu);
+  const auto it = g_hot_of.find(prepared);
+  return it != g_hot_of.end() && it->second.gather && it->second.B == B && it->second.n_touch_slots == n_touch_slots;
 }
 
 struct HotBufs { float *part; uint32_t *any; float *bpart; };
@@ -679,6 +762,8 @@
   constexpr int gpb = kBlock / G;
   const dim3 groups((bt.B + gpb - 1) / gpb);
   const bool adagrad = opt.kind == DRX_OPT_ADAGRAD;
+  constexpr int NT = kFwdThreads >= G ? kFwdThreads : G, fpb = NT / G;
+  const dim3 fgroups((bt.B + fpb - 1) / fpb);
   switch (form) {
   case ForwardForm::ColumnShard:
     hipLaunchKernelGGL((k_kshard_rest<G, J>), groups, dim3(kBlock), 0, st, P, opt, hist, bt, scale, qthr, loss_kind, S, ks_h, ks_dot);
@@ -695,8 +780,13 @@
                        loss_kind, S);
     break;
   case ForwardForm::PerGroup:
-    hipLaunchKernelGGL((adagrad ? k_sampled_fwd_bwd<G, J, DRX_OPT_ADAGRAD> : k_sampled_fwd_bwd<G, J>), groups, dim3(kBlock), 0, st, P, opt, hist,
-                       bt, scale, qthr, loss_kind, S);
+    if (S.rec) {
+      if constexpr (kPreparedGatherBuilt<G, J>)
+        hipLaunchKernelGGL((adagrad ? k_sampled_fwd_bwd<G, J, DRX_OPT_ADAGRAD, NT, true> : k_sampled_fwd_bwd<G, J, -1, NT, true>), fgroups,
+                           dim3(NT), 0, st, P, opt, hist, bt, scale, qthr, loss_kind, S);
+    } else
+      hipLaunchKernelGGL((adagrad ? k_sampled_fwd_bwd<G, J, DRX_OPT_ADAGRAD, NT> : k_sampled_fwd_bwd<G, J, -1, NT>), fgroups, dim3(NT), 0, st, P,
+                         opt, hist, bt, scale, qthr, loss_kind, S);
     break;
   }
 }
@@ -773,7 +863,7 @@
   PrepBufs R{};
   if (prepared) {
     Carver cp(const_cast<void *>(prepared), prepared_bytes);
-    R = prep_layout(cp, *p, bt->B, bt->n_touch_slots, H);
+    R = prep_layout(cp, *p, bt->B, bt->n_touch_slots, H, gather_recorded(prepared, bt->B, bt->n_touch_slots));
     if (!cp.ok()) return DRX_ESCRATCH;
   } else {
     R = prep_layout(cv, *p, bt->B, bt->n_touch_slots, H);
@@ -799,6 +889,10 @@
   S.n_items = share ? R.n_du : nullptr;
   ReduceForm form = reduce_form(opt->kind, bt->B, S.T, *p);
   const ForwardForm fwd = forward_form(ks_h != nullptr, share, bt->B, bt->n_touch_slots);
+  const bool pg = prepared && R.gather && fwd == ForwardForm::PerGroup &&
+                  dispatch_geom(p->ld, [](auto g) -> int { return kPreparedGatherBuilt<decltype(g)::G, decltype(g)::J> ? 1 : 0; }) != 0;
+  S.rec = pg ? R.rec : nullptr;
+  S.gl = pg ? R.gl : nullptr;
   if (H > 0 && !hot_head_fits(form, p->ld, share, ks_h != nullptr)) return DRX_EINVAL;
   if (given) {
     if (share || (given->form == 1 && (H > 0 || form == ReduceForm::PlannedLong))) return DRX_EINVAL;
@@ -842,7 +936,7 @@
 size_t drx_cdae_prep_bytes(const DrxCdaeParams *p, int32_t B, int32_t n_touch_slots) {
   if (!p || B < 1 || n_touch_slots < 0) return 0;
   Carver c(nullptr, 0);
-  (void)prep_layout(c, *p, B, n_touch_slots);
+  (void)prep_layout(c, *p, B, n_touch_slots, 0, true);
   return align_up(c.off, 256) + 256;
 }
 
@@ -853,11 +947,17 @@
   rc = check_batch(hist, bt);
   if (rc || !prepared || !bt->iid || !bt->keep_off) return DRX_EINVAL;
   Carver cp(prepared, prepared_bytes);
-  PrepBufs R = prep_layout(cp, *p, bt->B, bt->n_touch_slots);
-  if (!cp.ok()) return DRX_ESCRATCH;
+  PrepBufs R = prep_layout(cp, *p, bt->B, bt->n_touch_slots, 0, true);
+  if (!cp.ok()) {
+    Carver cq(prepared, prepared_bytes);
+    R = prep_layout(cq, *p, bt->B, bt->n_touch_slots);
+    if (!cq.ok()) return DRX_ESCRATCH;
+  }
   hot_record(prepared, 0);
-  rc = prepare_impl(p, hist, bt, R, (hipStream_t)stream, true);
-  if (rc) return rc;
+  bool gather = false;
+  rc = prepare_impl(p, hist, bt, R, (hipStream_t)stream, true, TouchPresence{nullptr, WireGeo{1, 0, 1}}, nullptr, nullptr, &gather);
+  if (rc) return rc;
+  hot_record(prepared, 0, gather, bt->B, bt->n_touch_slots);
   if (p->ld <= 16) order_by_degree(bt, R, (hipStream_t)stream, true);
   DRX_LAUNCH_CHECK();
   return DRX_OK;
@@ -945,7 +1045,7 @@
 size_t drx_cdae_prep_bytes_hot(const DrxCdaeParams *p, int32_t B, int32_t n_touch_slots, int32_t H) {
   if (!p || B < 1 || n_touch_slots < 0 || hot_rows(p, H) < 0) return 0;
   Carver c(nullptr, 0);
-  (void)prep_layout(c, *p, B, n_touch_slots, H);
+  (void)prep_layout(c, *p, B, n_touch_slots, H, true);
   return align_up(c.off, 256) + 256;
 }
 
@@ -965,12 +1065,17 @@
   rc = check_batch(hist, bt);
   if (rc || !prepared || !bt->iid || !bt->keep_off || !hot_ok(p, hot)) return DRX_EINVAL;
   Carver cp(prepared, prepared_bytes);
-  PrepBufs R = prep_layout(cp, *p, bt->B, bt->n_touch_slots, hot->H);
-  if (!cp.ok()) return DRX_ESCRATCH;
+  PrepBufs R = prep_layout(cp, *p, bt->B, bt->n_touch_slots, hot->H, true);
+  if (!cp.ok()) {
+    Carver cq(prepared, prepared_bytes);
+    R = prep_layout(cq, *p, bt->B, bt->n_touch_slots, hot->H);
+    if (!cq.ok()) return DRX_ESCRATCH;
+  }
   hot_record(prepared, 0);
-  rc = prepare_impl(p, hist, bt, R, (hipStream_t)stream, true, TouchPresence{nullptr, WireGeo{1, 0, 1}}, hot->slot, hot->item);
-  if (rc) return rc;
-  hot_record(prepared, hot->H);
+  bool gather = false;
+  rc = prepare_impl(p, hist, bt, R, (hipStream_t)stream, true, TouchPresence{nullptr, WireGeo{1, 0, 1}}, hot->slot, hot->item, &gather);
+  if (rc) return rc;
+  hot_record(prepared, hot->H, gather, bt->B, bt->n_touch_slots);
   if (p->ld <= 16) order_by_degree(bt, R, (hipStream_t)stream, true);
   DRX_LAUNCH_CHECK();
   return DRX_OK;
@@ -1034,6 +1139,22 @@
   return DRX_OK;
 }
 
+int drx_debug_prep_gather(const DrxCdaeParams *p, int32_t B, int32_t n_touch_slots, int32_t H, const void *prepared, size_t prepared_bytes,
+                          int32_t *rec_out, int32_t *n_out, int32_t *gl_out, void *stream) {
+  int rc = check_params(p);
+  if (rc) return rc;
+  if (B < 1 || n_touch_slots < 0 || hot_rows(p, H) < 0 || !prepared || !rec_out || !n_out || !gl_out) return DRX_EINVAL;
+  if (!gather_recorded(prepared, B, n_touch_slots) || hot_recorded(prepared) != H) return DRX_EINVAL;
+  Carver cp(const_cast<void *>(prepared), prepared_bytes);
+  const PrepBufs R = prep_layout(cp, *p, B, n_touch_slots, H, true);
+  if (!cp.ok()) return DRX_ESCRATCH;
+  hipStream_t st = (hipStream_t)stream;
+  DRX_HIP(hipMemcpyAsync(rec_out, R.rec, (size_t)B * 8 * sizeof(int32_t), hipMemcpyDeviceToDevice, st));
+  DRX_HIP(hipMemcpyAsync(n_out, R.gn, (size_t)B * sizeof(int32_t), hipMemcpyDeviceToDevice, st));
+  if (n_touch_slots > 0) DRX_HIP(hipMemcpyAsync(gl_out, R.gl, (size_t)n_touch_slots * sizeof(int32_t), hipMemcpyDeviceToDevice, st));
+  return DRX_OK;
+}
+
 int drx_debug_cdae_reduce(const DrxCdaeParams *p, const DrxOptim *opt, const DrxHistory *hist, const DrxBatch *bt, const DrxHotHead *hot,
                           const void *prepared, size_t prepared_bytes, const float *dz1_in, const float *g2_in, const float *dz2_in,
                           int32_t form, void *scratch, size_t scratch_bytes, void *stream) {
diff --git a/drecpy_amd/csrc/drx_prep.hpp b/drecpy_amd/csrc/drx_prep.hpp
--- a/drecpy_amd/csrc/drx_prep.hpp
+++ b/drecpy_amd/csrc/drx_prep.hpp
@@ -44,10 +44,25 @@
 static inline size_t hot_table_lds_bytes(int H) { return H > 0 && DRX_HOT_LDS_LOOKUP ? ((size_t)6 << hot_table_bits(H)) : 0; }
 __device__ __forceinline__ uint32_t hot_table_home(int item, int tbits) { return ((uint32_t)item * 2654435761u) >> (32 - tbits); }
 
+struct GatherList {
+  int32_t *gl, *n;
+  __device__ __forceinline__ void put(int ko0, int &nk, int lane, bool kf, int item) const {
+    const uint32_t m = (uint32_t)group_ballot<16>(kf);
+    if (kf) gl[ko0 + nk + __popc(m & ((1u << lane) - 1u))] = item;
+    nk += __popc(m);
+  }
+};
+struct SlotRecords {
+  int4 *rec;
+  const int32_t *uid, *iid;
+  const float *y;
+  const int32_t *n;
+};
+
 static __global__ __launch_bounds__(kBlock) void k_sparse_touches(int n_items, DrxHistory H, DrxBatch bt, uint32_t qthr, uint32_t *keys,
                                                            uint32_t *vals, int T, uint8_t *solo, uint32_t *zero_a,
                                                            int n_zero_a, uint32_t *zero_b, int n_zero_b, uint32_t *zero_c, int n_zero_c,
-                                                           TouchPresence pres, HotMark hot) {
+                                                           TouchPresence pres, HotMark hot, GatherList gat) {
   constexpr int G = 16;
   const int lane = threadIdx.x % G;
   const int b = blockIdx.x * (kBlock / G) + threadIdx.x / G;
@@ -80,10 +95,15 @@
   const int64_t s = H.indptr[u], e = H.indptr[u + 1];
   const int base = bt.keep_off[b] + 2 * b;
   const uint8_t *kp = bt.keep ? bt.keep + bt.keep_off[b] : nullptr;
-  for (int64_t j = s + lane; j < e; j += G) {
+  int nk = 0;
+  for (int64_t j0 = s; j0 < e; j0 += G) {
+    const int64_t j = j0 + lane;
+    bool kf = false;
+    int item = 0;
+    if (j < e) {
     const uint32_t jj = (uint32_t)(j - s);
-    const bool kf = kp ? (kp[jj] != 0) : (hash_u32(bt.mask_seed, (uint32_t)b, jj) >= qthr);
-    const int item = H.indices[j];
+    kf = kp ? (kp[jj] != 0) : (hash_u32(bt.mask_seed, (uint32_t)b, jj) >= qthr);
+    item = H.indices[j];
     int hs = -1;
     if (hot.slot && kf) {
       if (DRX_HOT_LDS_LOOKUP) {
@@ -98,7 +118,10 @@
     vals[base + jj] = (uint32_t)b;
     if (hs >= 0) atomicOr(&hm[hs], 1u << (b & 15));
     if (pres.present && kf) pres.present[pres.wire(item, 0)] = 1;
-  }
+    }
+    if (gat.gl) gat.put(bt.keep_off[b], nk, lane, kf, item);
+  }
+  if (gat.gl && lane == 0) gat.n[b] = nk;
   if (lane == 0) {
     const int deg = (int)(e - s);
     keys[base + deg] = (uint32_t)(n_items + bt.iid[b]);       vals[base + deg] = (uint32_t)b;
@@ -132,7 +155,8 @@
 static __global__ __launch_bounds__(kBlock) void k_sparse_touches_rounds(int n_items, DrxHistory H, DrxBatch bt, uint32_t qthr, uint32_t *keys,
                                                                   uint32_t *vals, int T, uint8_t *solo, uint32_t *zero_a,
                                                                   int n_zero_a, uint32_t *zero_b, int n_zero_b, uint32_t *zero_c,
-                                                                  int n_zero_c, TouchPresence pres, HotMark hot, uint32_t *part) {
+                                                                  int n_zero_c, TouchPresence pres, HotMark hot, uint32_t *part,
+                                                                  GatherList gat) {
   constexpr int G = 16, SPR = kBlock / G;
   const int lane = threadIdx.x % G, grp = threadIdx.x / G;
   const int B = bt.B, n_rounds = (B + SPR - 1) / SPR, stride = (int)gridDim.x;
@@ -197,8 +221,11 @@
         for (int j = ko1 + 2 * B + lane; j < T; j += G) { keys[j] = DRX_KEY_NONE; vals[j] = 0; }
       const int base = ko0 + 2 * b;
       const uint8_t *kp = bt.keep ? bt.keep + ko0 : nullptr;
-      auto touch = [&](uint32_t jj, int item) {
-        const bool kf = kp ? (kp[jj] != 0) : (hash_u32(bt.mask_seed, (uint32_t)b, jj) >= qthr);
+      int nk = 0;
+      auto touch = [&](bool valid, uint32_t jj, int item) {
+        bool kf = false;
+        if (valid) {
+        kf = kp ? (kp[jj] != 0) : (hash_u32(bt.mask_seed, (uint32_t)b, jj) >= qthr);
         int hs = -1;
         if (hot.slot && kf) {
           if (DRX_HOT_LDS_LOOKUP) {
@@ -215,11 +242,17 @@
         if (part && listed) atomicAdd(&dh[(((uint32_t)item & 255u) << 3) + rep], 1u);
         if (hs >= 0) atomicOr(&hm[hs], 1u << (b & 15));
         if (pres.present && kf) pres.present[pres.wire(item, 0)] = 1;
+        }
+        if (gat.gl) gat.put(ko0, nk, lane, kf, item);
       };
 #pragma unroll
       for (int k = 0; k < kPre; ++k)
-        if (s + lane + k * G < e) touch((uint32_t)(lane + k * G), it[k]);
-      for (int64_t j = s + lane + kPre * G; j < e; j += G) touch((uint32_t)(j - s), H.indices[j]);
+        if (s + k * G < e) touch(s + lane + k * G < e, (uint32_t)(lane + k * G), it[k]);
+      for (int64_t j0 = s + kPre * G; j0 < e; j0 += G) {
+        const int64_t j = j0 + lane;
+        touch(j < e, (uint32_t)(j - s), j < e ? H.indices[j] : 0);
+      }
+      if (gat.gl && lane == 0) gat.n[b] = nk;
       if (lane == 0) {
         const int deg = (int)(e - s);
         const uint32_t k_out = (uint32_t)(n_items + c.iid), k_usr = (uint32_t)(2 * n_items) + (uint32_t)u;
@@ -270,7 +303,8 @@
 
 template <int NT>
 __device__ __forceinline__ void degree_scatter_body(const int32_t *__restrict__ keep_off, int B, unsigned int *__restrict__ work,
-                                                    int32_t *__restrict__ order, int block_id, unsigned int *lds ) {
+                                                    int32_t *__restrict__ order, int block_id, unsigned int *lds ,
+                                                    const SlotRecords &sr = SlotRecords{nullptr, nullptr, nullptr, nullptr, nullptr}) {
   unsigned int *start = lds, *cnt = lds + 256, *base = lds + 512;
   for (int i = threadIdx.x; i < 256; i += NT) cnt[i] = 0;
   if (threadIdx.x < 64) {
@@ -296,7 +330,14 @@
   __syncthreads();
   for (int i = threadIdx.x; i < 256; i += NT) base[i] = cnt[i] ? atomicAdd(&work[256 + i], cnt[i]) : 0u;
   __syncthreads();
-  if (valid) order[start[d] + base[d] + at + __popcll(m & ((1ull << lane) - 1ull))] = b;
+  if (valid) {
+    const unsigned int slot = start[d] + base[d] + at + __popcll(m & ((1ull << lane) - 1ull));
+    order[slot] = b;
+    if (sr.rec) {
+      sr.rec[2 * (size_t)slot] = make_int4(b, sr.uid[b], sr.iid[b], __float_as_int(sr.y[b]));
+      sr.rec[2 * (size_t)slot + 1] = make_int4(keep_off[b], sr.n[b], 0, 0);
+    }
+  }
 }
 
 static __global__ __launch_bounds__(1024) void k_degree_scatter(const int32_t *__restrict__ keep_off, int B, unsigned int *__restrict__ work,
@@ -322,11 +363,11 @@
 static __global__ __launch_bounds__(256) void k_plan_and_mark(uint32_t *keys_s, const uint32_t *__restrict__ vals_s, int T, int n_chunks, int cpb,
                                                        SpanPlan P, uint32_t n_items, int B, uint8_t *solo_v, uint8_t *solo_o,
                                                        int order_blocks, const int32_t *keep_off, unsigned int *order_work,
-                                                       int32_t *order) {
+                                                       int32_t *order, SlotRecords sr) {
   const int plan_blocks = (int)gridDim.x - order_blocks;
   if ((int)blockIdx.x >= plan_blocks) {
     __shared__ unsigned int lds[768];
-    degree_scatter_body<256>(keep_off, B, order_work, order, (int)blockIdx.x - plan_blocks, lds);
+    degree_scatter_body<256>(keep_off, B, order_work, order, (int)blockIdx.x - plan_blocks, lds, sr);
     return;
   }
   const int tid = blockIdx.x * blockDim.x + threadIdx.x;
@@ -435,6 +476,9 @@
   int H, Bw;
   uint32_t *partials;
   int partial_rows;
+  bool gather;
+  int32_t *gn, *gl;
+  int4 *rec;
 };
 
 static inline bool long_segments(int T, const DrxCdaeParams &P) { return (int64_t)T > 8 * ((int64_t)2 * P.n_items + P.n_users); }
@@ -483,7 +527,7 @@
   return events ? hipEventRecord((hipEvent_t)events[i], st) : hipSuccess;
 }
 
-static PrepBufs prep_layout(Carver &cv, const DrxCdaeParams &P, int B, int n_touch_slots, int H = 0) {
+static PrepBufs prep_layout(Carver &cv, const DrxCdaeParams &P, int B, int n_touch_slots, int H = 0, bool gather = false) {
   PrepBufs R{};
   R.T = n_touch_slots + 2 * B;
   R.bits = bits_for((uint64_t)2 * P.n_items + P.n_users + 1);
@@ -520,6 +564,10 @@
   R.hmask = H > 0 ? cv.take<uint32_t>((size_t)H * R.Bw) : nullptr;
   R.partial_rows = DRX_PREP_ROUNDS && sort_first_digit_bits(R.bits) == 8 ? touch_grid(B) : 0;
   R.partials = R.partial_rows > 0 ? cv.take<uint32_t>((size_t)R.partial_rows * kPartialWords) : nullptr;
+  R.gather = gather;
+  R.gn = gather ? cv.take<int32_t>((size_t)B) : nullptr;
+  R.gl = gather ? cv.take<int32_t>((size_t)n_touch_slots + 1) : nullptr;
+  R.rec = gather ? cv.take<int4>((size_t)2 * B) : nullptr;
   return R;
 }
 
@@ -806,27 +854,29 @@
 }
 
 static void launch_touches(const DrxCdaeParams *p, const DrxHistory *hist, const DrxBatch *bt, const PrepBufs &R, hipStream_t st,
-                           TouchPresence pres, const int16_t *hot_slot, const int32_t *hot_item) {
+                           TouchPresence pres, const int16_t *hot_slot, const int32_t *hot_item, bool with_gather = false) {
   const int gpb = kBlock / 16;
   (void)gpb;
   uint32_t *sort_zero = nullptr;
   size_t sort_zero_words = 0;
   sort_pairs_zero_region(R.sort_temp, (size_t)R.T, R.bits, &sort_zero, &sort_zero_words);
   const HotMark hm{R.H > 0 ? hot_slot : nullptr, R.hmask, R.H, R.Bw, hot_item, hot_table_bits(R.H)};
+  const GatherList gat{with_gather ? R.gl : nullptr, with_gather ? R.gn : nullptr};
 #if DRX_PREP_ROUNDS
   hipLaunchKernelGGL(k_sparse_touches_rounds, dim3(touch_grid(bt->B)), dim3(kBlock), hot_table_lds_bytes(R.H), st, p->n_items, *hist, *bt,
                      q_threshold(bt->q), R.keys, R.vals, R.T, R.solo_v, R.plan.cnt, plan_zero_words(R), R.order_work, 512,
-                     sort_zero, (int)sort_zero_words, pres, hm, R.partials);
+                     sort_zero, (int)sort_zero_words, pres, hm, R.partials, gat);
 #else
   hipLaunchKernelGGL(k_sparse_touches, dim3((bt->B + gpb - 1) / gpb), dim3(kBlock), hot_table_lds_bytes(R.H), st, p->n_items, *hist, *bt,
                      q_threshold(bt->q), R.keys, R.vals, R.T, R.solo_v, R.plan.cnt, plan_zero_words(R), R.order_work, 512,
-                     sort_zero, (int)sort_zero_words, pres, hm);
+                     sort_zero, (int)sort_zero_words, pres, hm, gat);
 #endif
 }
 
 static int prepare_impl(const DrxCdaeParams *p, const DrxHistory *hist, const DrxBatch *bt, const PrepBufs &R, hipStream_t st,
                         bool with_marks = false, TouchPresence pres = TouchPresence{nullptr, WireGeo{1, 0, 1}},
-                        const int16_t *hot_slot = nullptr, const int32_t *hot_item = nullptr) {
+                        const int16_t *hot_slot = nullptr, const int32_t *hot_item = nullptr, bool *gather_out = nullptr) {
+  if (gather_out) *gather_out = false;
   if (R.H > 0 && (!hot_slot || !hot_item || !hot_list_fits(R.T, *p, pres.present != nullptr))) return DRX_EINVAL;
   if (hist->t_rank && hist->t_users && hist->t_pos && hist->t_items && !pres.present && long_segments(R.T, *p)) {
     const int32_t *row_end = nullptr;
@@ -840,7 +890,7 @@
         const int blocks = std::max(2048, (R.n_chunks + 255) / 256);
         hipLaunchKernelGGL(k_plan_and_mark, dim3(blocks), dim3(256), 0, st, R.keys_s, R.vals_s, R.T, R.n_chunks,
                            kSegBlock / pick_geom(p->ld).G, Rb.plan, (uint32_t)p->n_items, bt->B, R.solo_v, R.solo_o, 0, bt->keep_off,
-                           R.order_work, R.order);
+                           R.order_work, R.order, SlotRecords{nullptr, nullptr, nullptr, nullptr, nullptr});
         if (R.plan.xrank) hipLaunchKernelGGL(k_place_blocks, dim3(256), dim3(256), 0, st, Rb.plan, R.n_chunks);
         return DRX_OK;
       }
@@ -848,8 +898,9 @@
     }
     if (rc != kTpFallback) return rc;
   }
-  launch_touches(p, hist, bt, R, st, pres, hot_slot, hot_item);
   const bool fused_order = with_marks && p->ld > 16;
+  const bool with_gather = fused_order && R.gather && R.gl && bt->y;
+  launch_touches(p, hist, bt, R, st, pres, hot_slot, hot_item, with_gather);
   const SortRider rider{fused_order ? bt->keep_off : nullptr, bt->B, R.order_work, R.partials, R.partial_rows};
   const int rc = sort_pairs_ex(R.sort_temp, R.sort_bytes, R.keys, R.keys_s, R.vals, R.vals_s, (size_t)R.T, R.bits, true, st, true, rider);
   if (rc) return rc;
@@ -858,8 +909,10 @@
     const int order_blocks = (bt->B + 255) / 256;
     hipLaunchKernelGGL(k_plan_and_mark, dim3(blocks + order_blocks), dim3(256), 0, st, R.keys_s, R.vals_s, R.T, R.n_chunks,
                        kSegBlock / pick_geom(p->ld).G, R.plan, (uint32_t)p->n_items, bt->B, R.solo_v, R.solo_o,
-                       order_blocks, bt->keep_off, R.order_work, R.order);
+                       order_blocks, bt->keep_off, R.order_work, R.order,
+                       SlotRecords{with_gather ? R.rec : nullptr, bt->uid, bt->iid, bt->y, R.gn});
     if (R.plan.xrank) hipLaunchKernelGGL(k_place_blocks, dim3(256), dim3(256), 0, st, R.plan, R.n_chunks);
+    if (gather_out) *gather_out = with_gather;
     return DRX_OK;
   }
   return plan_spans(p, bt, R, st, true);
diff --git a/drecpy_amd/engine.py b/drecpy_amd/engine.py
--- a/drecpy_amd/engine.py
+++ b/drecpy_amd/engine.py
@@ -428,7 +428,7 @@
             check(lib().drx_cdae_sparse_prepare(C.byref(self._params), C.byref(self._hist), C.byref(bt), ptr(out), out.numel(),
                                                 stream_ptr(self.device)), 'drx_cdae_sparse_prepare')
         out._drx_hot = H
-        if H and not getattr(out, '_drx_forget', None):
+        if not getattr(out, '_drx_forget', None):
             out._drx_forget = weakref.finalize(out, _forget_prepared, out.data_ptr())
         return out
 
diff --git a/include/drx.h b/include/drx.h
--- a/include/drx.h
+++ b/include/drx.h
@@ -143,6 +143,9 @@
 int drx_debug_prep_result(const DrxCdaeParams *p, int32_t B, int32_t n_touch_slots, int32_t H, const void *prepared, size_t prepared_bytes,
                           uint32_t *keys_s_out, uint32_t *vals_s_out, uint8_t *solo_v_out, uint8_t *solo_o_out, int32_t *order_out,
                           void *stream);
+
+int drx_debug_prep_gather(const DrxCdaeParams *p, int32_t B, int32_t n_touch_slots, int32_t H, const void *prepared, size_t prepared_bytes,
+                          int32_t *rec_out, int32_t *n_out, int32_t *gl_out, void *stream);
 
 int drx_debug_cdae_reduce(const DrxCdaeParams *p, const DrxOptim *opt, const DrxHistory *hist, const DrxBatch *bt, const DrxHotHead *hot,
                           const void *prepared, size_t prepared_bytes, const float *dz1_in, const float *g2_in, const float *dz2_in,
```

Result: faster. 225.6 million samples/s, median of 6 (+1.2%).
